# XiSHEN0220/RANSAC-Flow

Hardware: NVIDIA H100
Metric: image-pairs/sec at 480x640, nbIter=1k RANSAC (higher is better)
Workload: dtype f32-grade: fp16 hi/lo split operands and activations (22 significand bits), 3 wgmma MMAs per MAC, fp32 accumulate; fp16-split correlation; fp32/fp64 RANSAC

## Files before the change

include/ransacflow_b200.h:

```cpp
#ifndef RANSACFLOW_B200_H
#define RANSACFLOW_B200_H

#include <stddef.h>
#include <stdint.h>

#ifdef __cplusplus
extern "C" {
#endif

#define RF_MAX_IMGS 16

#define RF_RANSAC_OK 0
#define RF_RANSAC_NONE 1
#define RF_RANSAC_NO_MODEL 2
#define RF_RANSAC_TOO_FEW 3

int rf_version(void);
const char* rf_source_digest(void);
const char* rf_last_error_string(void);
uint64_t rf_launch_count(void);

size_t rf_corr_mutual_nn_workspace(int NA, int NB, int C, int precision);
int rf_corr_mutual_nn_launches(int precision);
int rf_corr_mutual_nn(const float* featA, int NA, const float* featB, int NB, int C,
                      int64_t* idx1_out, int64_t* idx2_out, int* count_out,
                      void* ws, size_t ws_bytes, int precision, void* stream);

size_t rf_corr_mutual_nn_presplit_workspace(int NA, int NB);
int rf_corr_mutual_nn_presplit(const void* A_hi, const void* A_lo, int NA, const void* B_hi, const void* B_lo, int NB, int C,
                               int64_t* idx1_out, int64_t* idx2_out, int* count_out, void* ws, size_t ws_bytes, void* stream);

#define RF_SAMPLES_INDEX 0
#define RF_SAMPLES_MOD 1
#define RF_SAMPLES_PHILOX64 2
size_t rf_ransac_workspace(int nbIter);
int rf_ransac_homography(const float* match1, const float* match2, int M, const int* M_dev,
                         const int64_t* samples, int sample_mode, int nbIter, float tolerance, int chunk,
                         float* H_out, int64_t* nbInlier_out, uint8_t* mask_out, int* status_out,
                         void* ws, size_t ws_bytes, void* stream);
int rf_homography_dlt(const float* X, const float* Y, int N, float* H_out, void* stream);
int rf_prediction(const float* match1, const float* match2, int M, const float* H, int N, float* err_out, void* stream);
int rf_build_matches(const int64_t* idx1, const int64_t* idx2, const int* count_in,
                     const float* W1, const float* H1, const float* W2, const float* H2,
                     const uint8_t* valid16, float* match1_out, float* match2_out,
                     int64_t* idx2_kept_out, int* count_out, int capacity, void* stream);

#define RF_ENGINE_FP32 0
#define RF_ENGINE_TF32 1
#define RF_ENGINE_F16 2
#define RF_ENGINE_F16_OUT32 3
#define RF_ENGINE_SPLIT 4
#define RF_ENGINE_SPLIT_OUT32 5
int rf_conv2d_nhwc(const float* x, int nimg, const int* hw_host, int Cin,
                   const float* w, const float* w_tc, const float* bias, const float* residual,
                   int Cout, int R, int S, int stride, int pad, int relu, int engine,
                   float* y, void* stream);
int rf_conv1x1_dual_split(const void* x1, const void* x2, int nimg, const int* hw1_host, const int* hw2_host, int Cin1, int Cin2,
                          int stride2, const void* w_split, const float* bias, int Cout, int relu, void* y, void* stream);
#define RF_OP_CONV 0
#define RF_OP_MAXPOOL 1
#define RF_OP_BLUR 2
#define RF_OP_IM2COL 3
#define RF_OP_POOLBLUR 4
#define RF_OP_STEM7 5
#define RF_OP_CONV_DUAL 6
#define RF_MAX_SLOTS 32
typedef struct rf_layer {
    int op;
    int src, dst, res;
    int Cin, Cout, k, stride, pad, relu;
    const float* w;
    const float* w_tc;
    const float* bias;
    const void* w_f16;
    int flags;
    int src2, Cin2, stride2;
} rf_layer_t;
#define RF_LAYER_OUT_F32 1
#define RF_LAYER_TF32 2
int rf_run_layers(const rf_layer_t* layers_host, int n, void* const* slots_host, int nimg, const int* hw_host,
                  int engine, void* stream);
int rf_maxpool2d_nhwc(const float* x, int nimg, const int* hw_host, int C, int k, int stride, int pad,
                      float* y, void* stream);
int rf_blur_downsample_nhwc(const float* x, int nimg, const int* hw_host, int C, int stride, float* y, void* stream);
int rf_l2norm_nhwc(const float* x, long long P, int C, const uint8_t* mask, float* y, void* stream);
int rf_l2norm_split_nhwc(const void* x_split, long long P, int C, const uint8_t* mask, float* y, void* y_hi, void* y_lo, void* stream);
int rf_l2norm_f16_nhwc(const void* x_f16, long long P, int C, const uint8_t* mask, float* y, void* stream);
int rf_corr_neigh_nhwc(const float* x, const float* y, int N, int h, int w, int C, int k, int ldo, int round_tf32_out,
                       float* out, void* stream);
int rf_corr_neigh_pair_nhwc(const float* x, const float* y, int N, int h, int w, int C, int k, int ldo, int round_tf32_out,
                            float* out_xy, float* out_yx, void* stream);
int rf_corr_neigh_pair_split(const float* x, const float* y, int N, int h, int w, int C, int k, int ldo, void* out12_split, void* both_split,
                             void* stream);
int rf_softmax_flow(const float* logits, int N, int h, int w, int k, float* flow_nchw, void* stream);
int rf_sigmoid(const float* x, long long n, float* y, void* stream);
int rf_preproc_u8(const uint8_t* img, long long npix, int normalize, float* out_nhwc, void* stream);
int rf_resample_u8(const uint8_t* in, int in_h, int in_w, int channels, int horizontal,
                   const int* bounds, const int* kk, int ksize, int out_size, uint8_t* out, void* stream);
int rf_lanczos_coeffs_host(int in_size, int out_size, int* bounds_host, int* kk_host, int kk_capacity, int* ksize_out);

int rf_warp_grid(const float* H, int N, int h, int w, float* grid_out, void* stream);
int rf_grid_sample(const float* in, int N, int C, int Hin, int Win, const long long* in_s_host,
                   const float* grid, int Hout, int Wout, int align_corners,
                   float* out, const long long* out_s_host, void* stream);
int rf_upsample_bilinear(const float* in, int NC, int h, int w, int H, int W, float* out, void* stream);
int rf_compose_fine(const float* flowDown8, const float* match12, const float* match21, int h8, int w8,
                    const float* coarse, int H, int W, int clamp, int align_corners,
                    float* flow12_out, float* match_out, float* flowUp_out, void* stream);
int rf_compose_fine_ex(const float* flowDown8, const float* match12, const float* match21, int h8, int w8,
                       const float* coarse, int Hc, int Wc, int H, int W, int clamp, int align_corners,
                       float* flow12_out, float* match_out, float* flowUp_out, void* stream);
size_t rf_remove_small_cc_workspace(int H, int W);
int rf_remove_small_cc(float* match, int N, int H, int W, float match_th, double cc_th, void* ws, size_t ws_bytes, void* stream);

size_t rf_fill_nearest_matched_workspace(int H, int W);
int rf_fill_nearest_matched(const float* flow, const uint8_t* matched, int H, int W, float* flow_out, int* index_out,
                            void* ws, size_t ws_bytes, void* stream);

#ifdef __cplusplus
}
#endif
#endif
```

ransac-flow_b200/csrc/common.cuh:

```cuda
#pragma once
#include <cuda_runtime.h>
#include <stdint.h>
#include <stdio.h>
#include <atomic>

#include "../../include/ransacflow_b200.h"

namespace rf {

extern thread_local char g_err[512];
extern std::atomic<uint64_t> g_launches;

inline int fail(const char* what, cudaError_t e, const char* file, int line) {
    snprintf(g_err, sizeof(g_err), "%s: %s (%s:%d)", what, cudaGetErrorString(e), file, line);
    return 1;
}
inline int fail_msg(const char* msg) {
    snprintf(g_err, sizeof(g_err), "%s", msg);
    return 2;
}

#define RF_CUDA(expr)                                                   \
    do {                                                                \
        cudaError_t _e = (expr);                                        \
        if (_e != cudaSuccess) return rf::fail(#expr, _e, __FILE__, __LINE__); \
    } while (0)

#define RF_LAUNCHED()                                                   \
    do {                                                                \
        rf::g_launches.fetch_add(1, std::memory_order_relaxed);         \
        cudaError_t _e = cudaGetLastError();                            \
        if (_e != cudaSuccess) return rf::fail("kernel launch", _e, __FILE__, __LINE__); \
    } while (0)

#define RF_REQUIRE(cond, msg)                                           \
    do {                                                                \
        if (!(cond)) return rf::fail_msg(msg " [" #cond "]");           \
    } while (0)

inline cudaStream_t as_stream(void* s) { return reinterpret_cast<cudaStream_t>(s); }

inline int current_device() {
    int dev = 0;
    cudaGetDevice(&dev);
    return (dev >= 0 && dev < 64) ? dev : 0;
}

inline int num_sms() {
    static int n[64] = {0};
    const int dev = current_device();
    if (n[dev] == 0) {
        cudaDeviceGetAttribute(&n[dev], cudaDevAttrMultiProcessorCount, dev);
        if (n[dev] <= 0) n[dev] = 132;
    }
    return n[dev];
}

struct ImgSet {
    int n;
    int H[RF_MAX_IMGS], W[RF_MAX_IMGS];
    int Ho[RF_MAX_IMGS], Wo[RF_MAX_IMGS];
    long long in_pix[RF_MAX_IMGS + 1];
    long long out_pix[RF_MAX_IMGS + 1];
};

inline int make_imgset(ImgSet& s, int nimg, const int* hw, int k, int stride, int pad) {
    if (nimg < 1 || nimg > RF_MAX_IMGS) return 1;
    s.n = nimg;
    s.in_pix[0] = 0;
    s.out_pix[0] = 0;
    for (int i = 0; i < nimg; ++i) {
        s.H[i] = hw[2 * i];
        s.W[i] = hw[2 * i + 1];
        s.Ho[i] = (s.H[i] + 2 * pad - k) / stride + 1;
        s.Wo[i] = (s.W[i] + 2 * pad - k) / stride + 1;
        if (s.Ho[i] < 1 || s.Wo[i] < 1) return 1;
        s.in_pix[i + 1] = s.in_pix[i] + (long long)s.H[i] * s.W[i];
        s.out_pix[i + 1] = s.out_pix[i] + (long long)s.Ho[i] * s.Wo[i];
    }
    for (int i = nimg; i < RF_MAX_IMGS; ++i) {
        s.H[i] = s.W[i] = s.Ho[i] = s.Wo[i] = 0;
        s.in_pix[i + 1] = s.in_pix[nimg];
        s.out_pix[i + 1] = s.out_pix[nimg];
    }
    return 0;
}

struct ConvParams {
    const float* x;
    const float* w;
    const float* bias;
    const float* residual;
    float* y;
    int Cin, Cout, R, S, stride, pad, relu;
    int round_out;
    long long Mtot;
    int K;
};

__device__ __forceinline__ int find_img(const ImgSet& s, long long p) {
    int i = 0;
#pragma unroll
    for (int j = 1; j < RF_MAX_IMGS; ++j) i += (j < s.n && p >= s.out_pix[j]) ? 1 : 0;
    return i;
}

__device__ __forceinline__ uint32_t f2ord(float f) {
    uint32_t u = __float_as_uint(f);
    return (u & 0x80000000u) ? ~u : (u | 0x80000000u);
}
__device__ __forceinline__ float round_tf32(float x) {
    uint32_t u;
    asm("cvt.rna.tf32.f32 %0, %1;" : "=r"(u) : "f"(x));
    return __uint_as_float(u);
}
__device__ __forceinline__ float ord2f(uint32_t u) {
    return __uint_as_float((u & 0x80000000u) ? (u & 0x7fffffffu) : ~u);
}
__device__ __forceinline__ unsigned long long pack_key(float v, uint32_t idx) {
    return ((unsigned long long)f2ord(v) << 32) | (unsigned long long)(0xFFFFFFFFu - idx);
}
__device__ __forceinline__ uint32_t key_index(unsigned long long k) { return 0xFFFFFFFFu - (uint32_t)(k & 0xFFFFFFFFull); }
__device__ __forceinline__ float key_value(unsigned long long k) { return ord2f((uint32_t)(k >> 32)); }

}
```

ransac-flow_b200/csrc/elementwise.cu:

```cuda
#include <cuda_fp16.h>

#include <type_traits>

#include "common.cuh"

namespace rf {

__global__ void maxpool_kernel(const __grid_constant__ ImgSet set, const float* __restrict__ x, float* __restrict__ y,
                               int C, int k, int stride, int pad) {
    const int c4n = C >> 2;
    long long t = (long long)blockIdx.x * blockDim.x + threadIdx.x;
    long long total = set.out_pix[set.n] * c4n;
    if (t >= total) return;
    long long pm = t / c4n;
    int c4 = (int)(t - pm * c4n);
    int im = find_img(set, pm);
    int local = (int)(pm - set.out_pix[im]);
    int oy = local / set.Wo[im], ox = local - oy * set.Wo[im];
    const int H = set.H[im], W = set.W[im];
    float4 m = make_float4(-INFINITY, -INFINITY, -INFINITY, -INFINITY);
    for (int r = 0; r < k; ++r) {
        int iy = oy * stride - pad + r;
        if (iy < 0 || iy >= H) continue;
        for (int s = 0; s < k; ++s) {
            int ix = ox * stride - pad + s;
            if (ix < 0 || ix >= W) continue;
            float4 v = __ldg(reinterpret_cast<const float4*>(x + (set.in_pix[im] + (long long)iy * W + ix) * C) + c4);
            m.x = fmaxf(m.x, v.x); m.y = fmaxf(m.y, v.y); m.z = fmaxf(m.z, v.z); m.w = fmaxf(m.w, v.w);
        }
    }
    reinterpret_cast<float4*>(y + pm * C)[c4] = m;
}

__global__ void maxpool_f16_kernel(const __grid_constant__ ImgSet set, const __half* __restrict__ x, __half* __restrict__ y,
                                   int C, int k, int stride, int pad) {
    const int c8n = C >> 3;
    long long t = (long long)blockIdx.x * blockDim.x + threadIdx.x;
    long long total = set.out_pix[set.n] * c8n;
    if (t >= total) return;
    long long pm = t / c8n;
    int c8 = (int)(t - pm * c8n);
    int im = find_img(set, pm);
    int local = (int)(pm - set.out_pix[im]);
    int oy = local / set.Wo[im], ox = local - oy * set.Wo[im];
    const int H = set.H[im], W = set.W[im];
    const __half2 ninf = __float2half2_rn(-INFINITY);
    __half2 m[4] = {ninf, ninf, ninf, ninf};
    for (int r = 0; r < k; ++r) {
        int iy = oy * stride - pad + r;
        if (iy < 0 || iy >= H) continue;
        for (int s = 0; s < k; ++s) {
            int ix = ox * stride - pad + s;
            if (ix < 0 || ix >= W) continue;
            const uint4 v = __ldg(reinterpret_cast<const uint4*>(x + (set.in_pix[im] + (long long)iy * W + ix) * C) + c8);
            const __half2* h = reinterpret_cast<const __half2*>(&v);
#pragma unroll
            for (int e = 0; e < 4; ++e) m[e] = __hmax2(m[e], h[e]);
        }
    }
    uint4 o;
    __half2* ho = reinterpret_cast<__half2*>(&o);
#pragma unroll
    for (int e = 0; e < 4; ++e) ho[e] = m[e];
    reinterpret_cast<uint4*>(y + pm * C)[c8] = o;
}

template <int KC, int CC, int KPADC>
__global__ void im2col_kernel(const __grid_constant__ ImgSet set, const float* __restrict__ x, float* __restrict__ y,
                              int C_, int k_, int stride, int pad, int Kpad_, int round_out) {
    const int C = CC ? CC : C_, k = KC ? KC : k_, Kpad = KPADC ? KPADC : Kpad_;
    const int im = blockIdx.y;
    const int q4 = Kpad >> 2;
    const int Wo = set.Wo[im], H = set.H[im], W = set.W[im];
    const unsigned idx = blockIdx.x * blockDim.x + threadIdx.x;
    const unsigned total = (unsigned)(set.Ho[im] * Wo) * (unsigned)q4;
    if (idx >= total) return;
    const unsigned local = idx / (unsigned)q4;
    const int e0 = (int)(idx - local * (unsigned)q4) * 4;
    const int oy = (int)(local / (unsigned)Wo), ox = (int)(local - (unsigned)oy * (unsigned)Wo);
    const int kkc = k * k * C, kc = k * C;
    const float* src = x + set.in_pix[im] * C;
    float v[4];
#pragma unroll
    for (int j = 0; j < 4; ++j) {
        const int e = e0 + j;
        float t = 0.f;
        if (e < kkc) {
            const int r = e / kc, rem = e - r * kc;
            const int iy = oy * stride - pad + r;
            const int ixc = (ox * stride - pad) * C + rem;
            if (iy >= 0 && iy < H && ixc >= 0 && ixc < W * C) t = __ldg(src + (long long)iy * W * C + ixc);
            if (round_out) t = round_tf32(t);
        }
        v[j] = t;
    }
    reinterpret_cast<float4*>(y + (set.out_pix[im] + local) * Kpad)[e0 >> 2] = make_float4(v[0], v[1], v[2], v[3]);
}

__device__ __forceinline__ int reflect1(int i, int n) { return i < 0 ? -i : (i >= n ? 2 * n - 2 - i : i); }

template <typename T> struct Vec16;
template <> struct Vec16<float> {
    typedef float elem;
    static constexpr int N = 4;
    static __device__ __forceinline__ void load(const float* p, long long, float (&v)[4]) {
        const float4 t = __ldg(reinterpret_cast<const float4*>(p));
        v[0] = t.x; v[1] = t.y; v[2] = t.z; v[3] = t.w;
    }
    static __device__ __forceinline__ void store(float* p, long long, const float (&v)[4], int round_out) {
        float4 t = make_float4(v[0], v[1], v[2], v[3]);
        if (round_out) { t.x = round_tf32(t.x); t.y = round_tf32(t.y); t.z = round_tf32(t.z); t.w = round_tf32(t.w); }
        *reinterpret_cast<float4*>(p) = t;
    }
};
template <> struct Vec16<__half> {
    typedef __half elem;
    static constexpr int N = 8;
    static __device__ __forceinline__ void load(const __half* p, long long, float (&v)[8]) {
        const uint4 t = __ldg(reinterpret_cast<const uint4*>(p));
        const __half2* h = reinterpret_cast<const __half2*>(&t);
#pragma unroll
        for (int e = 0; e < 4; ++e) { const float2 f = __half22float2(h[e]); v[2 * e] = f.x; v[2 * e + 1] = f.y; }
    }
    static __device__ __forceinline__ void store(__half* p, long long, const float (&v)[8], int) {
        uint4 t;
        __half2* h = reinterpret_cast<__half2*>(&t);
#pragma unroll
        for (int e = 0; e < 4; ++e) h[e] = __floats2half2_rn(v[2 * e], v[2 * e + 1]);
        *reinterpret_cast<uint4*>(p) = t;
    }
};
struct SplitH {};
__device__ __forceinline__ void split_store8(__half* p, long long plane, const float (&v)[8]) {
    uint4 th, tl;
    __half2* h = reinterpret_cast<__half2*>(&th);
    __half2* l = reinterpret_cast<__half2*>(&tl);
#pragma unroll
    for (int e = 0; e < 4; ++e) {
        const float a = fminf(fmaxf(v[2 * e], -65504.f), 65504.f), b = fminf(fmaxf(v[2 * e + 1], -65504.f), 65504.f);
        h[e] = __floats2half2_rn(a, b);
        const float2 f = __half22float2(h[e]);
        l[e] = __floats2half2_rn((a - f.x) * 2048.f, (b - f.y) * 2048.f);
    }
    *reinterpret_cast<uint4*>(p) = th;
    *reinterpret_cast<uint4*>(p + plane) = tl;
}
__device__ __forceinline__ void split_load8(const __half* p, long long plane, float (&v)[8]) {
    const uint4 th = __ldg(reinterpret_cast<const uint4*>(p)), tl = __ldg(reinterpret_cast<const uint4*>(p + plane));
    const __half2* h = reinterpret_cast<const __half2*>(&th);
    const __half2* l = reinterpret_cast<const __half2*>(&tl);
#pragma unroll
    for (int e = 0; e < 4; ++e) {
        const float2 fh = __half22float2(h[e]), fl = __half22float2(l[e]);
        v[2 * e] = fmaf(fl.x, 0.00048828125f, fh.x);
        v[2 * e + 1] = fmaf(fl.y, 0.00048828125f, fh.y);
    }
}
template <> struct Vec16<SplitH> {
    typedef __half elem;
    static constexpr int N = 8;
    static __device__ __forceinline__ void load(const __half* p, long long plane, float (&v)[8]) { split_load8(p, plane, v); }
    static __device__ __forceinline__ void store(__half* p, long long plane, const float (&v)[8], int) { split_store8(p, plane, v); }
};

template <typename T>
__global__ void blur_kernel(const __grid_constant__ ImgSet set, const typename Vec16<T>::elem* __restrict__ x, typename Vec16<T>::elem* __restrict__ y,
                            int C, int stride, int round_out, long long pin = 0, long long pout = 0) {
    constexpr int VN = Vec16<T>::N;
    const int cvn = C / VN;
    long long t = (long long)blockIdx.x * blockDim.x + threadIdx.x;
    long long total = set.out_pix[set.n] * cvn;
    if (t >= total) return;
    long long pm = t / cvn;
    int cv = (int)(t - pm * cvn);
    int im = find_img(set, pm);
    int local = (int)(pm - set.out_pix[im]);
    int oy = local / set.Wo[im], ox = local - oy * set.Wo[im];
    const int H = set.H[im], W = set.W[im];
    float acc[VN];
#pragma unroll
    for (int e = 0; e < VN; ++e) acc[e] = 0.f;
#pragma unroll
    for (int r = 0; r < 3; ++r) {
        int iy = reflect1(oy * stride - 1 + r, H);
#pragma unroll
        for (int s = 0; s < 3; ++s) {
            int ix = reflect1(ox * stride - 1 + s, W);
            float wgt = ((r == 1) ? 2.f : 1.f) * ((s == 1) ? 2.f : 1.f) * 0.0625f;
            float v[VN];
            Vec16<T>::load(x + (set.in_pix[im] + (long long)iy * W + ix) * C + cv * VN, pin, v);
#pragma unroll
            for (int e = 0; e < VN; ++e) acc[e] = fmaf(wgt, v[e], acc[e]);
        }
    }
    Vec16<T>::store(y + pm * C + cv * VN, pout, acc, round_out);
}

template <typename T>
__global__ void poolblur_kernel(const __grid_constant__ ImgSet set, const typename Vec16<T>::elem* __restrict__ x, typename Vec16<T>::elem* __restrict__ y,
                                int C, int round_out, long long pin = 0, long long pout = 0) {
    constexpr int VN = Vec16<T>::N;
    const int cvn = C / VN;
    long long t = (long long)blockIdx.x * blockDim.x + threadIdx.x;
    long long total = set.out_pix[set.n] * cvn;
    if (t >= total) return;
    long long pm = t / cvn;
    int cv = (int)(t - pm * cvn);
    int im = find_img(set, pm);
    int local = (int)(pm - set.out_pix[im]);
    int oy = local / set.Wo[im], ox = local - oy * set.Wo[im];
    const int H = set.H[im], W = set.W[im];
    const int Hp = H - 1, Wp = W - 1;
    const typename Vec16<T>::elem* base = x + set.in_pix[im] * C + cv * VN;
    float acc[VN];
#pragma unroll
    for (int e = 0; e < VN; ++e) acc[e] = 0.f;
#pragma unroll
    for (int r = 0; r < 3; ++r) {
        const int py = reflect1(oy * 2 - 1 + r, Hp);
#pragma unroll
        for (int s = 0; s < 3; ++s) {
            const int px = reflect1(ox * 2 - 1 + s, Wp);
            const float wgt = ((r == 1) ? 2.f : 1.f) * ((s == 1) ? 2.f : 1.f) * 0.0625f;
            float a[VN], b[VN], c[VN], d[VN];
            Vec16<T>::load(base + ((long long)py * W + px) * C, pin, a);
            Vec16<T>::load(base + ((long long)py * W + px + 1) * C, pin, b);
            Vec16<T>::load(base + ((long long)(py + 1) * W + px) * C, pin, c);
            Vec16<T>::load(base + ((long long)(py + 1) * W + px + 1) * C, pin, d);
#pragma unroll
            for (int e = 0; e < VN; ++e) acc[e] = fmaf(wgt, fmaxf(fmaxf(a[e], b[e]), fmaxf(c[e], d[e])), acc[e]);
        }
    }
    Vec16<T>::store(y + pm * C + cv * VN, pout, acc, round_out);
}

__global__ void maxpool_split_kernel(const __grid_constant__ ImgSet set, const __half* __restrict__ x, __half* __restrict__ y,
                                     int C, int k, int stride, int pad, long long pin, long long pout) {
    const int c8n = C >> 3;
    long long t = (long long)blockIdx.x * blockDim.x + threadIdx.x;
    long long total = set.out_pix[set.n] * c8n;
    if (t >= total) return;
    long long pm = t / c8n;
    int c8 = (int)(t - pm * c8n);
    int im = find_img(set, pm);
    int local = (int)(pm - set.out_pix[im]);
    int oy = local / set.Wo[im], ox = local - oy * set.Wo[im];
    const int H = set.H[im], W = set.W[im];
    float m[8];
#pragma unroll
    for (int e = 0; e < 8; ++e) m[e] = -INFINITY;
    for (int r = 0; r < k; ++r) {
        int iy = oy * stride - pad + r;
        if (iy < 0 || iy >= H) continue;
        for (int s = 0; s < k; ++s) {
            int ix = ox * stride - pad + s;
            if (ix < 0 || ix >= W) continue;
            float v[8];
            split_load8(x + (set.in_pix[im] + (long long)iy * W + ix) * C + c8 * 8, pin, v);
#pragma unroll
            for (int e = 0; e < 8; ++e) m[e] = fmaxf(m[e], v[e]);
        }
    }
    split_store8(y + pm * C + c8 * 8, pout, m);
}

__global__ void l2norm_kernel(const float* __restrict__ x, long long P, int C, const unsigned char* __restrict__ mask, float* __restrict__ y) {
    long long pix = ((long long)blockIdx.x * blockDim.x + threadIdx.x) >> 5;
    int lane = threadIdx.x & 31;
    if (pix >= P) return;
    const float4* src = reinterpret_cast<const float4*>(x + pix * C);
    float4* dst = reinterpret_cast<float4*>(y + pix * C);
    const int c4n = C >> 2;
    if (mask != nullptr && mask[pix] == 0) {
        for (int c = lane; c < c4n; c += 32) dst[c] = make_float4(0, 0, 0, 0);
        return;
    }
    float ss = 0.f;
    for (int c = lane; c < c4n; c += 32) {
        float4 v = __ldg(src + c);
        ss = fmaf(v.x, v.x, ss); ss = fmaf(v.y, v.y, ss); ss = fmaf(v.z, v.z, ss); ss = fmaf(v.w, v.w, ss);
    }
#pragma unroll
    for (int d = 16; d >= 1; d >>= 1) ss += __shfl_xor_sync(0xffffffffu, ss, d);
    float denom = fmaxf(sqrtf(ss), 1e-12f);
    for (int c = lane; c < c4n; c += 32) {
        float4 v = __ldg(src + c);
        dst[c] = make_float4(__fdiv_rn(v.x, denom), __fdiv_rn(v.y, denom), __fdiv_rn(v.z, denom), __fdiv_rn(v.w, denom));
    }
}

__global__ void l2norm_f16_kernel(const __half* __restrict__ x, long long P, int C, const unsigned char* __restrict__ mask, float* __restrict__ y) {
    long long pix = ((long long)blockIdx.x * blockDim.x + threadIdx.x) >> 5;
    int lane = threadIdx.x & 31;
    if (pix >= P) return;
    const uint4* src = reinterpret_cast<const uint4*>(x + pix * C);
    float4* dst = reinterpret_cast<float4*>(y + pix * C);
    const int c8n = C >> 3;
    if (mask != nullptr && mask[pix] == 0) {
        for (int c = lane; c < 2 * c8n; c += 32) dst[c] = make_float4(0, 0, 0, 0);
        return;
    }
    float ss = 0.f;
    for (int c = lane; c < c8n; c += 32) {
        const uint4 v = __ldg(src + c);
        const __half2* h = reinterpret_cast<const __half2*>(&v);
#pragma unroll
        for (int e = 0; e < 4; ++e) { const float2 f = __half22float2(h[e]); ss = fmaf(f.x, f.x, ss); ss = fmaf(f.y, f.y, ss); }
    }
#pragma unroll
    for (int d = 16; d >= 1; d >>= 1) ss += __shfl_xor_sync(0xffffffffu, ss, d);
    float denom = fmaxf(sqrtf(ss), 1e-12f);
    for (int c = lane; c < c8n; c += 32) {
        const uint4 v = __ldg(src + c);
        const __half2* h = reinterpret_cast<const __half2*>(&v);
        const float2 f0 = __half22float2(h[0]), f1 = __half22float2(h[1]), f2 = __half22float2(h[2]), f3 = __half22float2(h[3]);
        dst[2 * c] = make_float4(__fdiv_rn(f0.x, denom), __fdiv_rn(f0.y, denom), __fdiv_rn(f1.x, denom), __fdiv_rn(f1.y, denom));
        dst[2 * c + 1] = make_float4(__fdiv_rn(f2.x, denom), __fdiv_rn(f2.y, denom), __fdiv_rn(f3.x, denom), __fdiv_rn(f3.y, denom));
    }
}

__global__ void l2norm_split_kernel(const __half* __restrict__ x, long long plane, long long P, int C, const unsigned char* __restrict__ mask,
                                    float* __restrict__ y, __half* __restrict__ yhi, __half* __restrict__ ylo) {
    long long pix = ((long long)blockIdx.x * blockDim.x + threadIdx.x) >> 5;
    int lane = threadIdx.x & 31;
    if (pix >= P) return;
    const __half* src = x + pix * C;
    float4* dst = reinterpret_cast<float4*>(y + pix * C);
    const int c8n = C >> 3;
    if (mask != nullptr && mask[pix] == 0) {
        if (y != nullptr)
            for (int c = lane; c < 2 * c8n; c += 32) dst[c] = make_float4(0, 0, 0, 0);
        if (yhi != nullptr)
            for (int c = lane; c < c8n; c += 32) {
                reinterpret_cast<uint4*>(yhi + pix * C)[c] = make_uint4(0, 0, 0, 0);
                reinterpret_cast<uint4*>(ylo + pix * C)[c] = make_uint4(0, 0, 0, 0);
            }
        return;
    }
    float ss = 0.f;
    for (int c = lane; c < c8n; c += 32) {
        float v[8];
        split_load8(src + c * 8, plane, v);
#pragma unroll
        for (int e = 0; e < 8; ++e) ss = fmaf(v[e], v[e], ss);
    }
#pragma unroll
    for (int d = 16; d >= 1; d >>= 1) ss += __shfl_xor_sync(0xffffffffu, ss, d);
    float denom = fmaxf(sqrtf(ss), 1e-12f);
    for (int c = lane; c < c8n; c += 32) {
        float v[8];
        split_load8(src + c * 8, plane, v);
#pragma unroll
        for (int e = 0; e < 8; ++e) v[e] = __fdiv_rn(v[e], denom);
        if (y != nullptr) {
            dst[2 * c] = make_float4(v[0], v[1], v[2], v[3]);
            dst[2 * c + 1] = make_float4(v[4], v[5], v[6], v[7]);
        }
        if (yhi != nullptr) split_store8(yhi + pix * C + c * 8, (ylo - yhi), v);
    }
}

__device__ __forceinline__ void corr_store(float* out, long long idx, float v, int round_out, long long plane) {
    if (round_out == 3) {
        const float a = fminf(fmaxf(v, -65504.f), 65504.f);
        const __half h = __float2half_rn(a);
        reinterpret_cast<__half*>(out)[idx] = h;
        reinterpret_cast<__half*>(out)[idx + plane] = __float2half_rn((a - __half2float(h)) * 2048.f);
    } else if (round_out == 2) {
        reinterpret_cast<__half*>(out)[idx] = __float2half_rn(v);
    } else {
        out[idx] = round_out ? round_tf32(v) : v;
    }
}

__global__ void corr_neigh_kernel(const float* __restrict__ x, const float* __restrict__ y, int N, int h, int w, int C, int k, int ldo, int round_out,
                                  float* __restrict__ out, float* __restrict__ out2) {
    long long pix = ((long long)blockIdx.x * blockDim.x + threadIdx.x) >> 5;
    int lane = threadIdx.x & 31;
    long long P = (long long)N * h * w;
    if (pix >= P) return;
    int n = (int)(pix / ((long long)h * w));
    int rem = (int)(pix - (long long)n * h * w);
    int r = rem / w, c = rem - r * w;
    const int pad = k / 2, c4n = C >> 2;
    const bool split = round_out == 3;
    const long long plane1 = P * ldo, plane2 = 2 * P * ldo;
    const float4* xs = reinterpret_cast<const float4*>(x + pix * C);
    float4 xv[8];
#pragma unroll
    for (int q = 0; q < 8; ++q) xv[q] = (lane + 32 * q < c4n) ? __ldg(xs + lane + 32 * q) : make_float4(0, 0, 0, 0);
    for (int i = 0; i < k; ++i) {
        int yr = r + i - pad;
        for (int j = 0; j < k; ++j) {
            int yc = c + j - pad;
            float acc = 0.f;
            if (yr >= 0 && yr < h && yc >= 0 && yc < w) {
                const float4* ys = reinterpret_cast<const float4*>(y + (((long long)n * h + yr) * w + yc) * C);
#pragma unroll
                for (int q = 0; q < 8; ++q)
                    if (lane + 32 * q < c4n) {
                        float4 v = __ldg(ys + lane + 32 * q);
                        acc = fmaf(xv[q].x, v.x, acc); acc = fmaf(xv[q].y, v.y, acc);
                        acc = fmaf(xv[q].z, v.z, acc); acc = fmaf(xv[q].w, v.w, acc);
                    }
            }
#pragma unroll
            for (int d = 16; d >= 1; d >>= 1) acc += __shfl_xor_sync(0xffffffffu, acc, d);
            if (lane == 0) {
                corr_store(out, pix * ldo + i * k + j, acc, round_out, plane1);
                if (out2 != nullptr) {
                    if (split) corr_store(out2, pix * ldo + i * k + j, acc, 3, plane2);
                    const bool inside = yr >= 0 && yr < h && yc >= 0 && yc < w;
                    const long long q = inside ? (((long long)n * h + yr) * w + yc) : pix;
                    const int e = inside ? (k - 1 - i) * k + (k - 1 - j) : i * k + j;
                    if (split) corr_store(out2, (P + q) * ldo + e, acc, 3, plane2);
                    else corr_store(out2, q * ldo + e, acc, round_out, 0);
                }
            }
        }
    }
    for (int cz = k * k + lane; cz < ldo; cz += 32) {
        corr_store(out, pix * ldo + cz, 0.f, round_out, plane1);
        if (out2 != nullptr) {
            if (split) { corr_store(out2, pix * ldo + cz, 0.f, 3, plane2); corr_store(out2, (P + pix) * ldo + cz, 0.f, 3, plane2); }
            else corr_store(out2, pix * ldo + cz, 0.f, round_out, 0);
        }
    }
}

__global__ void __launch_bounds__(256)
corr_neigh7_kernel(const float* __restrict__ x, const float* __restrict__ y, int N, int h, int w, int C, int ldo, int round_out,
                   float* __restrict__ out, float* __restrict__ out2) {
    constexpr int K = 7, KK = 49, PAD = 3;
    const long long pix = ((long long)blockIdx.x * blockDim.x + threadIdx.x) >> 5;
    const int lane = threadIdx.x & 31;
    const long long P = (long long)N * h * w;
    if (pix >= P) return;
    const int n = (int)(pix / ((long long)h * w));
    const int rem = (int)(pix - (long long)n * h * w);
    const int r = rem / w, c = rem - r * w;
    const int c4n = C >> 2;
    const bool split = round_out == 3;
    const long long plane1 = P * ldo, plane2 = 2 * P * ldo;
    const float4* xs = reinterpret_cast<const float4*>(x + pix * C);
    float4 xv[8];
#pragma unroll
    for (int q = 0; q < 8; ++q) xv[q] = (lane + 32 * q < c4n) ? __ldg(xs + lane + 32 * q) : make_float4(0, 0, 0, 0);
    float a[64];
#pragma unroll
    for (int t = 0; t < 64; ++t) a[t] = 0.f;
#pragma unroll
    for (int i = 0; i < K; ++i) {
        const int yr = r + i - PAD;
#pragma unroll
        for (int j = 0; j < K; ++j) {
            const int yc = c + j - PAD;
            if (yr >= 0 && yr < h && yc >= 0 && yc < w) {
                const float4* ys = reinterpret_cast<const float4*>(y + (((long long)n * h + yr) * w + yc) * C);
                float acc = 0.f;
#pragma unroll
                for (int q = 0; q < 8; ++q)
                    if (lane + 32 * q < c4n) {
                        const float4 v = __ldg(ys + lane + 32 * q);
                        acc = fmaf(xv[q].x, v.x, acc); acc = fmaf(xv[q].y, v.y, acc);
                        acc = fmaf(xv[q].z, v.z, acc); acc = fmaf(xv[q].w, v.w, acc);
                    }
                a[i * K + j] = acc;
            }
        }
    }
#pragma unroll
    for (int s = 16, nv = 32; s >= 1; s >>= 1, nv >>= 1) {
        const bool up = (lane & s) != 0;
#pragma unroll
        for (int v = 0; v < nv; ++v) {
            const float send = up ? a[v] : a[v + nv];
            const float keep = up ? a[v + nv] : a[v];
            a[v] = keep + __shfl_xor_sync(0xffffffffu, send, s);
        }
    }
#pragma unroll
    for (int u = 0; u < 2; ++u) {
        const int t = 2 * lane + u;
        if (t >= ldo) continue;
        const float v = a[u];
        corr_store(out, pix * ldo + t, v, round_out, plane1);
        if (out2 != nullptr) {
            if (split) corr_store(out2, pix * ldo + t, v, 3, plane2);
            if (t < KK) {
                const int i = t / K, j = t - i * K;
                const int yr = r + i - PAD, yc = c + j - PAD;
                const bool inside = yr >= 0 && yr < h && yc >= 0 && yc < w;
                const long long q = inside ? (((long long)n * h + yr) * w + yc) : pix;
                const int e = inside ? (KK - 1 - t) : t;
                if (split) corr_store(out2, (P + q) * ldo + e, v, 3, plane2);
                else corr_store(out2, q * ldo + e, v, round_out, 0);
            } else {
                if (split) corr_store(out2, (P + pix) * ldo + t, 0.f, 3, plane2);
                else corr_store(out2, pix * ldo + t, 0.f, round_out, 0);
            }
        }
    }
    for (int t = 64 + lane; t < ldo; t += 32) {
        corr_store(out, pix * ldo + t, 0.f, round_out, plane1);
        if (out2 != nullptr) {
            if (split) { corr_store(out2, pix * ldo + t, 0.f, 3, plane2); corr_store(out2, (P + pix) * ldo + t, 0.f, 3, plane2); }
            else corr_store(out2, pix * ldo + t, 0.f, round_out, 0);
        }
    }
}

__global__ void softmax_flow_kernel(const float* __restrict__ logits, int N, int h, int w, int k, float* __restrict__ flow) {
    long long pix = (long long)blockIdx.x * blockDim.x + threadIdx.x;
    long long hw = (long long)h * w;
    if (pix >= N * hw) return;
    const int kk = k * k, pad = k / 2;
    const float* l = logits + pix * kk;
    float m = -INFINITY;
    for (int q = 0; q < kk; ++q) m = fmaxf(m, __ldg(l + q));
    float sum = 0.f, sx = 0.f, sy = 0.f;
    for (int q = 0; q < kk; ++q) {
        float e = expf(__ldg(l + q) - m);
        sum += e;
        sx = fmaf(e, (float)(q % k - pad), sx);
        sy = fmaf(e, (float)(q / k - pad), sy);
    }
    int n = (int)(pix / hw);
    long long rem = pix - n * hw;
    flow[(n * 2 + 0) * hw + rem] = (sx / sum) / (float)w * 2.f;
    flow[(n * 2 + 1) * hw + rem] = (sy / sum) / (float)h * 2.f;
}

__global__ void sigmoid_kernel(const float* __restrict__ x, long long n, float* __restrict__ y) {
    long long i = (long long)blockIdx.x * blockDim.x + threadIdx.x;
    if (i < n) y[i] = 1.f / (1.f + expf(-x[i]));
}

__global__ void preproc_kernel(const unsigned char* __restrict__ img, long long n, int normalize, float* __restrict__ out) {
    long long i = (long long)blockIdx.x * blockDim.x + threadIdx.x;
    if (i >= n) return;
    int c = (int)(i % 3);
    float v = __fdiv_rn((float)img[i], 255.f);
    if (normalize) {
        const float mean = (c == 0) ? 0.485f : (c == 1 ? 0.456f : 0.406f);
        const float sd = (c == 0) ? 0.229f : (c == 1 ? 0.224f : 0.225f);
        v = __fdiv_rn(__fsub_rn(v, mean), sd);
    }
    out[i] = v;
}

__device__ __forceinline__ float preproc_one(unsigned int byte, int c, int normalize) {
    float v = __fdiv_rn((float)byte, 255.f);
    if (normalize) {
        const float mean = (c == 0) ? 0.485f : (c == 1 ? 0.456f : 0.406f);
        const float sd = (c == 0) ? 0.229f : (c == 1 ? 0.224f : 0.225f);
        v = __fdiv_rn(__fsub_rn(v, mean), sd);
    }
    return v;
}
__global__ void preproc_vec_kernel(const unsigned int* __restrict__ img, long long ngroups, int normalize, float4* __restrict__ out) {
    long long g = (long long)blockIdx.x * blockDim.x + threadIdx.x;
    if (g >= ngroups) return;
    const unsigned int w0 = __ldg(img + 3 * g), w1 = __ldg(img + 3 * g + 1), w2 = __ldg(img + 3 * g + 2);
    out[3 * g] = make_float4(preproc_one(w0 & 255u, 0, normalize), preproc_one((w0 >> 8) & 255u, 1, normalize),
                             preproc_one((w0 >> 16) & 255u, 2, normalize), preproc_one(w0 >> 24, 0, normalize));
    out[3 * g + 1] = make_float4(preproc_one(w1 & 255u, 1, normalize), preproc_one((w1 >> 8) & 255u, 2, normalize),
                                 preproc_one((w1 >> 16) & 255u, 0, normalize), preproc_one(w1 >> 24, 1, normalize));
    out[3 * g + 2] = make_float4(preproc_one(w2 & 255u, 2, normalize), preproc_one((w2 >> 8) & 255u, 0, normalize),
                                 preproc_one((w2 >> 16) & 255u, 1, normalize), preproc_one(w2 >> 24, 2, normalize));
}

#define RF_PRECISION_BITS 22
__device__ __forceinline__ unsigned char clip8(int ss) {
    int v = ss >> RF_PRECISION_BITS;
    return (unsigned char)(v < 0 ? 0 : (v > 255 ? 255 : v));
}
__global__ void resample_h_kernel(const unsigned char* __restrict__ in, int in_h, int in_w, int ch, const int* __restrict__ bounds,
                                  const int* __restrict__ kk, int ksize, int out_w, unsigned char* __restrict__ out) {
    long long t = (long long)blockIdx.x * blockDim.x + threadIdx.x;
    if (t >= (long long)in_h * out_w) return;
    const int ox = (int)(t % out_w), oy = (int)(t / out_w);
    const int lo = bounds[2 * ox], cnt = bounds[2 * ox + 1];
    const int* k = kk + (long long)ox * ksize;
    const unsigned char* row = in + ((long long)oy * in_w + lo) * ch;
    if (ch == 3) {
        int s0 = 1 << (RF_PRECISION_BITS - 1), s1 = s0, s2 = s0;
        for (int x = 0; x < cnt; ++x) {
            const int kx = __ldg(k + x);
            s0 += (int)row[3 * x] * kx; s1 += (int)row[3 * x + 1] * kx; s2 += (int)row[3 * x + 2] * kx;
        }
        unsigned char* o = out + t * 3;
        o[0] = clip8(s0); o[1] = clip8(s1); o[2] = clip8(s2);
    } else {
        for (int c = 0; c < ch; ++c) {
            int ss = 1 << (RF_PRECISION_BITS - 1);
            for (int x = 0; x < cnt; ++x) ss += (int)row[(long long)x * ch + c] * __ldg(k + x);
            out[t * ch + c] = clip8(ss);
        }
    }
}
__global__ void resample_v_kernel(const unsigned char* __restrict__ in, int in_h, int row_bytes, const int* __restrict__ bounds,
                                  const int* __restrict__ kk, int ksize, int out_h, unsigned char* __restrict__ out) {
    const int q = row_bytes >> 2;
    long long t = (long long)blockIdx.x * blockDim.x + threadIdx.x;
    if (t >= (long long)out_h * q) return;
    const int xq = (int)(t % q), oy = (int)(t / q);
    const int lo = bounds[2 * oy], cnt = bounds[2 * oy + 1];
    const int* k = kk + (long long)oy * ksize;
    const unsigned int* col = reinterpret_cast<const unsigned int*>(in + (long long)lo * row_bytes) + xq;
    int s0 = 1 << (RF_PRECISION_BITS - 1), s1 = s0, s2 = s0, s3 = s0;
    for (int y = 0; y < cnt; ++y) {
        const unsigned int v = __ldg(col + (long long)y * q);
        const int ky = __ldg(k + y);
        s0 += (int)(v & 0xFF) * ky; s1 += (int)((v >> 8) & 0xFF) * ky; s2 += (int)((v >> 16) & 0xFF) * ky; s3 += (int)(v >> 24) * ky;
    }
    reinterpret_cast<unsigned int*>(out)[t] = (unsigned)clip8(s0) | ((unsigned)clip8(s1) << 8) | ((unsigned)clip8(s2) << 16) | ((unsigned)clip8(s3) << 24);
}
__global__ void resample_u8_kernel(const unsigned char* __restrict__ in, int in_h, int in_w, int ch, int horizontal,
                                   const int* __restrict__ bounds, const int* __restrict__ kk, int ksize, int out_size,
                                   unsigned char* __restrict__ out) {
    const int out_h = horizontal ? in_h : out_size, out_w = horizontal ? out_size : in_w;
    long long t = (long long)blockIdx.x * blockDim.x + threadIdx.x;
    long long total = (long long)out_h * out_w * ch;
    if (t >= total) return;
    int c = (int)(t % ch);
    long long pq = t / ch;
    int ox = (int)(pq % out_w), oy = (int)(pq / out_w);
    int o = horizontal ? ox : oy;
    int lo = bounds[2 * o], cnt = bounds[2 * o + 1];
    const int* k = kk + (long long)o * ksize;
    int ss = 1 << (RF_PRECISION_BITS - 1);
    if (horizontal) {
        const unsigned char* row = in + ((long long)oy * in_w) * ch + c;
        for (int x = 0; x < cnt; ++x) ss += (int)row[(long long)(x + lo) * ch] * k[x];
    } else {
        const unsigned char* col = in + (long long)ox * ch + c;
        for (int y = 0; y < cnt; ++y) ss += (int)col[(long long)(y + lo) * in_w * ch] * k[y];
    }
    out[t] = clip8(ss);
}

__device__ __forceinline__ float lin11(int i, int n) {
    if (n == 1) return -1.f;
    float step = 2.f / (float)(n - 1);
    return (i < n / 2) ? (-1.f + step * (float)i) : (1.f - step * (float)(n - 1 - i));
}

__global__ void warp_grid_kernel(const float* __restrict__ Hm, int N, int h, int w, float* __restrict__ grid) {
    long long t = (long long)blockIdx.x * blockDim.x + threadIdx.x;
    long long hw = (long long)h * w;
    if (t >= N * hw) return;
    int n = (int)(t / hw);
    int rem = (int)(t - n * hw);
    int r = rem / w, c = rem - r * w;
    const float* H = Hm + n * 9;
    float x = lin11(c, w), y = lin11(r, h);
    float px = __fadd_rn(__fadd_rn(__fmul_rn(H[0], x), __fmul_rn(H[1], y)), H[2]);
    float py = __fadd_rn(__fadd_rn(__fmul_rn(H[3], x), __fmul_rn(H[4], y)), H[5]);
    float pz = __fadd_rn(__fadd_rn(__fmul_rn(H[6], x), __fmul_rn(H[7], y)), H[8]);
    reinterpret_cast<float2*>(grid)[t] = make_float2(__fdiv_rn(px, pz), __fdiv_rn(py, pz));
}

__device__ __forceinline__ float unnormalize(float coord, int size, int align_corners) {
    return align_corners ? ((coord + 1.f) / 2.f) * (float)(size - 1) : ((coord + 1.f) * (float)size - 1.f) / 2.f;
}

__device__ __forceinline__ float in_int_range(float c) {
    return fabsf(c) < 2147483648.f ? c : -100.f;
}

struct Strides4 { long long n, c, h, w; };

__global__ void grid_sample_kernel(const float* __restrict__ in, int N, int C, int Hin, int Win, Strides4 is,
                                   const float* __restrict__ grid, int Hout, int Wout, int align_corners,
                                   float* __restrict__ out, Strides4 os) {
    long long t = (long long)blockIdx.x * blockDim.x + threadIdx.x;
    long long hw = (long long)Hout * Wout;
    if (t >= N * hw) return;
    int n = (int)(t / hw);
    int rem = (int)(t - n * hw);
    int r = rem / Wout, c = rem - r * Wout;
    float2 g = __ldg(reinterpret_cast<const float2*>(grid) + t);
    float ix = in_int_range(unnormalize(g.x, Win, align_corners)), iy = in_int_range(unnormalize(g.y, Hin, align_corners));
    float fx = floorf(ix), fy = floorf(iy);
    int x0 = (int)fx, y0 = (int)fy, x1 = x0 + 1, y1 = y0 + 1;
    float nw = (fx + 1.f - ix) * (fy + 1.f - iy), ne = (ix - fx) * (fy + 1.f - iy);
    float sw = (fx + 1.f - ix) * (iy - fy), se = (ix - fx) * (iy - fy);
    bool vx0 = x0 >= 0 && x0 < Win, vx1 = x1 >= 0 && x1 < Win, vy0 = y0 >= 0 && y0 < Hin, vy1 = y1 >= 0 && y1 < Hin;
    const float* base = in + n * is.n;
    float* ob = out + n * os.n + r * os.h + c * os.w;
    for (int ch = 0; ch < C; ++ch) {
        const float* p = base + ch * is.c;
        float acc = 0.f;
        if (vy0 && vx0) acc += __ldg(p + y0 * is.h + x0 * is.w) * nw;
        if (vy0 && vx1) acc += __ldg(p + y0 * is.h + x1 * is.w) * ne;
        if (vy1 && vx0) acc += __ldg(p + y1 * is.h + x0 * is.w) * sw;
        if (vy1 && vx1) acc += __ldg(p + y1 * is.h + x1 * is.w) * se;
        ob[ch * os.c] = acc;
    }
}

__device__ __forceinline__ void up_coord(int dst, int in_size, int out_size, int& i0, int& i1, float& l0, float& l1) {
    float scale = (float)in_size / (float)out_size;
    float src = scale * ((float)dst + 0.5f) - 0.5f;
    if (src < 0.f) src = 0.f;
    i0 = (int)src;
    i1 = i0 + ((i0 < in_size - 1) ? 1 : 0);
    l1 = src - (float)i0;
    l0 = 1.f - l1;
}
__device__ __forceinline__ float up_sample(const float* __restrict__ p, int h, int w, int H, int W, int Y, int X) {
    int y0, y1, x0, x1;
    float ly0, ly1, lx0, lx1;
    up_coord(Y, h, H, y0, y1, ly0, ly1);
    up_coord(X, w, W, x0, x1, lx0, lx1);
    return ly0 * (lx0 * __ldg(p + y0 * w + x0) + lx1 * __ldg(p + y0 * w + x1)) +
           ly1 * (lx0 * __ldg(p + y1 * w + x0) + lx1 * __ldg(p + y1 * w + x1));
}

__global__ void upsample_kernel(const float* __restrict__ in, int NC, int h, int w, int H, int W, float* __restrict__ out) {
    long long t = (long long)blockIdx.x * blockDim.x + threadIdx.x;
    long long HW = (long long)H * W;
    if (t >= NC * HW) return;
    int nc = (int)(t / HW);
    int rem = (int)(t - nc * HW);
    int Y = rem / W, X = rem - Y * W;
    out[t] = up_sample(in + (long long)nc * h * w, h, w, H, W, Y, X);
}

__global__ void compose_fine_kernel(const float* __restrict__ flow8, const float* __restrict__ m12, const float* __restrict__ m21,
                                    int h8, int w8, const float* __restrict__ coarse, int Hc, int Wc, int H, int W, int clamp, int align_corners,
                                    float* __restrict__ flow12, float* __restrict__ match, float* __restrict__ flowUp_out) {
    long long t = (long long)blockIdx.x * blockDim.x + threadIdx.x;
    if (t >= (long long)H * W) return;
    int Y = (int)(t / W), X = (int)(t - (long long)Y * W);
    float fx = up_sample(flow8, h8, w8, H, W, Y, X) + lin11(X, W);
    float fy = up_sample(flow8 + h8 * w8, h8, w8, H, W, Y, X) + lin11(Y, H);
    if (clamp) {
        fx = fminf(fmaxf(fx, -1.f), 1.f);
        fy = fminf(fmaxf(fy, -1.f), 1.f);
    }
    if (flowUp_out) reinterpret_cast<float2*>(flowUp_out)[t] = make_float2(fx, fy);
    const float2* cg = reinterpret_cast<const float2*>(coarse);
    float ox = 0.f, oy = 0.f, mm = 0.f;
    {
        float ix = unnormalize(fx, Wc, align_corners), iy = unnormalize(fy, Hc, align_corners);
        float flx = floorf(ix), fly = floorf(iy);
        int x0 = (int)flx, y0 = (int)fly, x1 = x0 + 1, y1 = y0 + 1;
        float nw = (flx + 1.f - ix) * (fly + 1.f - iy), ne = (ix - flx) * (fly + 1.f - iy);
        float sw = (flx + 1.f - ix) * (iy - fly), se = (ix - flx) * (iy - fly);
        bool vx0 = x0 >= 0 && x0 < Wc, vx1 = x1 >= 0 && x1 < Wc, vy0 = y0 >= 0 && y0 < Hc, vy1 = y1 >= 0 && y1 < Hc;
        if (vy0 && vx0) { float2 v = __ldg(cg + (long long)y0 * Wc + x0); ox += v.x * nw; oy += v.y * nw; }
        if (vy0 && vx1) { float2 v = __ldg(cg + (long long)y0 * Wc + x1); ox += v.x * ne; oy += v.y * ne; }
        if (vy1 && vx0) { float2 v = __ldg(cg + (long long)y1 * Wc + x0); ox += v.x * sw; oy += v.y * sw; }
        if (vy1 && vx1) { float2 v = __ldg(cg + (long long)y1 * Wc + x1); ox += v.x * se; oy += v.y * se; }
    }
    if (m21) {
        float ix = unnormalize(fx, W, align_corners), iy = unnormalize(fy, H, align_corners);
        float flx = floorf(ix), fly = floorf(iy);
        int x0 = (int)flx, y0 = (int)fly, x1 = x0 + 1, y1 = y0 + 1;
        float nw = (flx + 1.f - ix) * (fly + 1.f - iy), ne = (ix - flx) * (fly + 1.f - iy);
        float sw = (flx + 1.f - ix) * (iy - fly), se = (ix - flx) * (iy - fly);
        bool vx0 = x0 >= 0 && x0 < W, vx1 = x1 >= 0 && x1 < W, vy0 = y0 >= 0 && y0 < H, vy1 = y1 >= 0 && y1 < H;
        if (vy0 && vx0) mm += up_sample(m21, h8, w8, H, W, y0, x0) * nw;
        if (vy0 && vx1) mm += up_sample(m21, h8, w8, H, W, y0, x1) * ne;
        if (vy1 && vx0) mm += up_sample(m21, h8, w8, H, W, y1, x0) * sw;
        if (vy1 && vx1) mm += up_sample(m21, h8, w8, H, W, y1, x1) * se;
    }
    reinterpret_cast<float2*>(flow12)[t] = make_float2(ox, oy);
    if (match) {
        float m = up_sample(m12, h8, w8, H, W, Y, X);
        if (m21) m *= mm;
        float inside = ((ox >= -1.f && ox <= 1.f) ? 1.f : 0.f) * ((oy >= -1.f && oy <= 1.f) ? 1.f : 0.f);
        match[t] = m * inside;
    }
}

__device__ __forceinline__ int cc_find(const int* L, int i) {
    int p = L[i];
    while (p != i) { i = p; p = L[i]; }
    return i;
}
__device__ __forceinline__ void cc_union(int* L, int a, int b) {
    bool done = false;
    while (!done) {
        a = cc_find(L, a);
        b = cc_find(L, b);
        if (a < b) { int old = atomicMin(&L[b], a); done = (old == b); b = old; }
        else if (b < a) { int old = atomicMin(&L[a], b); done = (old == a); a = old; }
        else done = true;
    }
}
__global__ void cc_init_kernel(const float* __restrict__ match, float th, int n, int* __restrict__ L, int* __restrict__ cnt) {
    int i = blockIdx.x * blockDim.x + threadIdx.x;
    if (i >= n) return;
    L[i] = (match[i] > th) ? i : -1;
    cnt[i] = 0;
}
__global__ void cc_merge_kernel(int* __restrict__ L, int H, int W) {
    int i = blockIdx.x * blockDim.x + threadIdx.x;
    if (i >= H * W || L[i] < 0) return;
    const int y = i / W, x = i - y * W;
    if (x > 0 && L[i - 1] >= 0) cc_union(L, i, i - 1);
    if (y > 0) {
        if (L[i - W] >= 0) cc_union(L, i, i - W);
        if (x > 0 && L[i - W - 1] >= 0) cc_union(L, i, i - W - 1);
        if (x + 1 < W && L[i - W + 1] >= 0) cc_union(L, i, i - W + 1);
    }
}
__global__ void cc_flatten_count_kernel(int* __restrict__ L, int n, int* __restrict__ cnt) {
    int i = blockIdx.x * blockDim.x + threadIdx.x;
    if (i >= n || L[i] < 0) return;
    const int r = cc_find(L, i);
    atomicAdd(&cnt[r], 1);
}
__global__ void cc_filter_kernel(float* __restrict__ match, const int* __restrict__ L, const int* __restrict__ cnt, int n, double cc_th) {
    int i = blockIdx.x * blockDim.x + threadIdx.x;
    if (i >= n || L[i] < 0) return;
    const int r = cc_find(L, i);
    if ((double)cnt[r] / (double)n <= cc_th) match[i] = 0.f;
}

__global__ void edt_cols_kernel(const unsigned char* __restrict__ matched, int H, int W, int* __restrict__ gy) {
    const int x = blockIdx.x * blockDim.x + threadIdx.x;
    if (x >= W) return;
    int last = -1;
    for (int y = 0; y < H; ++y) {
        if (matched[(long long)y * W + x]) last = y;
        gy[(long long)y * W + x] = last;
    }
    last = -1;
    for (int y = H - 1; y >= 0; --y) {
        if (matched[(long long)y * W + x]) last = y;
        const int a = gy[(long long)y * W + x];
        int pick = a;
        if (a < 0) pick = last;
        else if (last >= 0 && (last - y) < (y - a)) pick = last;
        gy[(long long)y * W + x] = pick;
    }
}
__global__ void edt_rows_fill_kernel(const int* __restrict__ gy, int H, int W, int* __restrict__ v, double* __restrict__ z,
                                     const float2* __restrict__ flow, float2* __restrict__ out, int* __restrict__ idx_out) {
    const int y = blockIdx.x * blockDim.x + threadIdx.x;
    if (y >= H) return;
    const int* g = gy + (long long)y * W;
    int* vv = v + (long long)y * W;
    double* zz = z + (long long)y * (W + 1);
    int k = -1;
    for (int q = 0; q < W; ++q) {
        if (g[q] < 0) continue;
        const long long dq = (long long)(y - g[q]) * (y - g[q]);
        double sx = -1e300;
        while (k >= 0) {
            const int p = vv[k];
            const long long dp = (long long)(y - g[p]) * (y - g[p]);
            sx = (double)((dq + (long long)q * q) - (dp + (long long)p * p)) / (double)(2 * (q - p));
            if (sx <= zz[k]) --k; else break;
        }
        if (k < 0) sx = -1e300;
        ++k;
        vv[k] = q;
        zz[k] = sx;
    }
    if (k < 0) {
        for (int x = 0; x < W; ++x) { out[(long long)y * W + x] = flow[(long long)y * W + x]; if (idx_out) { idx_out[2 * ((long long)y * W + x)] = y; idx_out[2 * ((long long)y * W + x) + 1] = x; } }
        return;
    }
    const int kmax = k;
    k = 0;
    for (int x = 0; x < W; ++x) {
        while (k < kmax && zz[k + 1] < (double)x) ++k;
        const int xs = vv[k], ys = g[xs];
        out[(long long)y * W + x] = flow[(long long)ys * W + xs];
        if (idx_out) { idx_out[2 * ((long long)y * W + x)] = ys; idx_out[2 * ((long long)y * W + x) + 1] = xs; }
    }
}

}

using namespace rf;

static inline unsigned blocks_for(long long n, int threads) { return (unsigned)((n + threads - 1) / threads); }

static int launch_corr_neigh(const float* x, const float* y, int N, int h, int w, int C, int k, int ldo, int round_out, float* out,
                             float* out2, void* stream) {
    const long long P = (long long)N * h * w;
    if (P == 0) return 0;
    if (k == 7) corr_neigh7_kernel<<<blocks_for(P * 32, 256), 256, 0, as_stream(stream)>>>(x, y, N, h, w, C, ldo, round_out, out, out2);
    else corr_neigh_kernel<<<blocks_for(P * 32, 256), 256, 0, as_stream(stream)>>>(x, y, N, h, w, C, k, ldo, round_out, out, out2);
    RF_LAUNCHED();
    return 0;
}

extern "C" int rf_maxpool2d_nhwc(const float* x, int nimg, const int* hw_host, int C, int k, int stride, int pad, float* y, void* stream) {
    RF_REQUIRE((C % 4) == 0 && k >= 1 && stride >= 1, "rf_maxpool2d_nhwc: C must be a multiple of 4");
    ImgSet set;
    RF_REQUIRE(make_imgset(set, nimg, hw_host, k, stride, pad) == 0, "rf_maxpool2d_nhwc: bad image set");
    long long total = set.out_pix[nimg] * (C / 4);
    maxpool_kernel<<<blocks_for(total, 256), 256, 0, as_stream(stream)>>>(set, x, y, C, k, stride, pad);
    RF_LAUNCHED();
    return 0;
}

int rf_blur_downsample_impl(const float* x, int nimg, const int* hw_host, int C, int stride, int round_out, float* y, void* stream) {
    RF_REQUIRE((C % 4) == 0 && stride >= 1, "rf_blur_downsample_nhwc: C must be a multiple of 4");
    ImgSet set;
    RF_REQUIRE(make_imgset(set, nimg, hw_host, 3, stride, 1) == 0, "rf_blur_downsample_nhwc: bad image set");
    for (int i = 0; i < nimg; ++i) RF_REQUIRE(set.H[i] >= 2 && set.W[i] >= 2, "rf_blur_downsample_nhwc: reflect padding needs H, W >= 2");
    long long total = set.out_pix[nimg] * (C / 4);
    blur_kernel<float><<<blocks_for(total, 256), 256, 0, as_stream(stream)>>>(set, x, y, C, stride, round_out);
    RF_LAUNCHED();
    return 0;
}

int rf_poolblur_impl(const float* x, int nimg, const int* hw_host, int C, int round_out, float* y, void* stream) {
    RF_REQUIRE((C % 4) == 0, "rf_poolblur: C must be a multiple of 4");
    ImgSet set;
    RF_REQUIRE(make_imgset(set, nimg, hw_host, 4, 2, 1) == 0, "rf_poolblur: bad image set");
    for (int i = 0; i < nimg; ++i) RF_REQUIRE(set.H[i] >= 3 && set.W[i] >= 3, "rf_poolblur: needs H, W >= 3");
    long long total = set.out_pix[nimg] * (C / 4);
    poolblur_kernel<float><<<blocks_for(total, 256), 256, 0, as_stream(stream)>>>(set, x, y, C, round_out);
    RF_LAUNCHED();
    return 0;
}

extern "C" int rf_blur_downsample_nhwc(const float* x, int nimg, const int* hw_host, int C, int stride, float* y, void* stream) {
    return rf_blur_downsample_impl(x, nimg, hw_host, C, stride, 0, y, stream);
}

template <typename T> struct OutElem { typedef T type; };
template <> struct OutElem<SplitH> { typedef __half type; };

template <int K, int C, int KPAD, int STRIDE, int PAD, int TPX, typename OutT = float>
__global__ void __launch_bounds__(256)
im2col_smem_kernel(const __grid_constant__ ImgSet set, const float* __restrict__ x, typename OutElem<OutT>::type* __restrict__ y, int round_out,
                   long long plane = 0) {
    constexpr int INW = ((TPX - 1) * STRIDE + K) * C;
    constexpr int Q4 = KPAD / 4;
    __shared__ float sIn[K][INW + 1];
    const int im = blockIdx.z, oy = blockIdx.y, ox0 = blockIdx.x * TPX;
    const int Wo = set.Wo[im];
    if (oy >= set.Ho[im] || ox0 >= Wo) return;
    const int H = set.H[im], WC = set.W[im] * C;
    const float* src = x + set.in_pix[im] * C;
    const int col0 = (ox0 * STRIDE - PAD) * C;
    constexpr int NLD = (K * INW + 255) / 256;
    float stage[NLD];
#pragma unroll
    for (int i = 0; i < NLD; ++i) {
        const int idx = threadIdx.x + i * 256;
        const int r = idx / INW, j = idx - r * INW;
        const int iy = oy * STRIDE - PAD + r, col = col0 + j;
        stage[i] = (idx < K * INW && iy >= 0 && iy < H && col >= 0 && col < WC) ? __ldg(src + (long long)iy * WC + col) : 0.f;
    }
#pragma unroll
    for (int i = 0; i < NLD; ++i) {
        const int idx = threadIdx.x + i * 256;
        const int r = idx / INW, j = idx - r * INW;
        if (idx < K * INW) sIn[r][j] = round_out ? round_tf32(stage[i]) : stage[i];
    }
    __syncthreads();
    const int npx = min(TPX, Wo - ox0);
    if constexpr (std::is_same<OutT, SplitH>::value) {
        constexpr int Q8 = KPAD / 8;
        __half* dsts = y + (set.out_pix[im] + (long long)oy * Wo + ox0) * KPAD;
        for (int f = threadIdx.x; f < npx * Q8; f += 256) {
            const int px = f / Q8, e0 = (f - px * Q8) * 8;
            float v[8];
#pragma unroll
            for (int j = 0; j < 8; ++j) {
                const int e = e0 + j;
                v[j] = (e < K * K * C) ? sIn[e / (K * C)][px * STRIDE * C + e % (K * C)] : 0.f;
            }
            split_store8(dsts + (long long)f * 8, plane, v);
        }
        return;
    } else if constexpr (sizeof(OutT) == 2) {
        constexpr int Q8 = KPAD / 8;
        uint4* dst8 = reinterpret_cast<uint4*>(y + (set.out_pix[im] + (long long)oy * Wo + ox0) * KPAD);
        for (int f = threadIdx.x; f < npx * Q8; f += 256) {
            const int px = f / Q8, e0 = (f - px * Q8) * 8;
            float v[8];
#pragma unroll
            for (int j = 0; j < 8; ++j) {
                const int e = e0 + j;
                v[j] = (e < K * K * C) ? sIn[e / (K * C)][px * STRIDE * C + e % (K * C)] : 0.f;
            }
            uint4 o;
            __half2* ho = reinterpret_cast<__half2*>(&o);
#pragma unroll
            for (int j = 0; j < 4; ++j) ho[j] = __floats2half2_rn(v[2 * j], v[2 * j + 1]);
            dst8[f] = o;
        }
        return;
    }
    float4* dst = reinterpret_cast<float4*>(y + (set.out_pix[im] + (long long)oy * Wo + ox0) * KPAD);
    for (int f = threadIdx.x; f < npx * Q4; f += 256) {
        const int px = f / Q4, e0 = (f - px * Q4) * 4;
        float v[4];
#pragma unroll
        for (int j = 0; j < 4; ++j) {
            const int e = e0 + j;
            v[j] = (e < K * K * C) ? sIn[e / (K * C)][px * STRIDE * C + e % (K * C)] : 0.f;
        }
        dst[f] = make_float4(v[0], v[1], v[2], v[3]);
    }
}

int rf_im2col_impl(const float* x, int nimg, const int* hw_host, int C, int k, int stride, int pad, int Kpad, int round_out,
                   float* y, void* stream) {
    RF_REQUIRE(Kpad >= k * k * C && C >= 1, "rf_im2col: Kpad too small");
    ImgSet set;
    RF_REQUIRE(make_imgset(set, nimg, hw_host, k, stride, pad) == 0, "rf_im2col: bad image set");
    RF_REQUIRE((Kpad & 3) == 0, "rf_im2col: Kpad must be a multiple of 4");
    long long maxq = 0;
    for (int i = 0; i < nimg; ++i) {
        long long q = (long long)set.Ho[i] * set.Wo[i] * (Kpad / 4);
        RF_REQUIRE(q < (1ll << 31), "rf_im2col: image too large for 32-bit indexing");
        if (q > maxq) maxq = q;
    }
    int maxHo = 0, maxWo = 0;
    for (int i = 0; i < nimg; ++i) { maxHo = set.Ho[i] > maxHo ? set.Ho[i] : maxHo; maxWo = set.Wo[i] > maxWo ? set.Wo[i] : maxWo; }
    if (k == 7 && C == 3 && Kpad == 160 && stride == 2 && pad == 3) {
        im2col_smem_kernel<7, 3, 160, 2, 3, 64><<<dim3((maxWo + 63) / 64, maxHo, nimg), 256, 0, as_stream(stream)>>>(set, x, y, round_out);
        RF_LAUNCHED();
        return 0;
    }
    if (k == 3 && C == 3 && Kpad == 32 && stride == 1 && pad == 1) {
        im2col_smem_kernel<3, 3, 32, 1, 1, 128><<<dim3((maxWo + 127) / 128, maxHo, nimg), 256, 0, as_stream(stream)>>>(set, x, y, round_out);
        RF_LAUNCHED();
        return 0;
    }
    dim3 grid(blocks_for(maxq, 256), nimg);
    if (k == 7 && C == 3 && Kpad == 160) im2col_kernel<7, 3, 160><<<grid, 256, 0, as_stream(stream)>>>(set, x, y, C, k, stride, pad, Kpad, round_out);
    else if (k == 3 && C == 3 && Kpad == 32) im2col_kernel<3, 3, 32><<<grid, 256, 0, as_stream(stream)>>>(set, x, y, C, k, stride, pad, Kpad, round_out);
    else im2col_kernel<0, 0, 0><<<grid, 256, 0, as_stream(stream)>>>(set, x, y, C, k, stride, pad, Kpad, round_out);
    RF_LAUNCHED();
    return 0;
}

int rf_im2col_f16_impl(const float* x, int nimg, const int* hw_host, int C, int k, int stride, int pad, int Kpad, void* y_f16, void* stream) {
    const bool resnet = (k == 7 && C == 3 && Kpad == 192 && stride == 2 && pad == 3);
    const bool fe = (k == 3 && C == 3 && Kpad == 64 && stride == 1 && pad == 1);
    RF_REQUIRE(resnet || fe, "rf_im2col (engine 2): only the ResNet-50 stem (7x7/2, Kpad 192) and the FeatureExtractor stem (3x3/1, Kpad 64)");
    ImgSet set;
    RF_REQUIRE(make_imgset(set, nimg, hw_host, k, stride, pad) == 0, "rf_im2col: bad image set");
    int maxHo = 0, maxWo = 0;
    for (int i = 0; i < nimg; ++i) { maxHo = set.Ho[i] > maxHo ? set.Ho[i] : maxHo; maxWo = set.Wo[i] > maxWo ? set.Wo[i] : maxWo; }
    if (fe) {
        im2col_smem_kernel<3, 3, 64, 1, 1, 128, __half><<<dim3((maxWo + 127) / 128, maxHo, nimg), 256, 0, as_stream(stream)>>>(
            set, x, static_cast<__half*>(y_f16), 0);
        RF_LAUNCHED();
        return 0;
    }
    im2col_smem_kernel<7, 3, 192, 2, 3, 64, __half><<<dim3((maxWo + 63) / 64, maxHo, nimg), 256, 0, as_stream(stream)>>>(
        set, x, static_cast<__half*>(y_f16), 0);
    RF_LAUNCHED();
    return 0;
}

int rf_blur_f16_impl(const void* x_f16, int nimg, const int* hw_host, int C, int stride, void* y_f16, void* stream) {
    RF_REQUIRE((C % 8) == 0 && stride >= 1, "rf_blur (engine 2): C must be a multiple of 8");
    ImgSet set;
    RF_REQUIRE(make_imgset(set, nimg, hw_host, 3, stride, 1) == 0, "rf_blur: bad image set");
    for (int i = 0; i < nimg; ++i) RF_REQUIRE(set.H[i] >= 2 && set.W[i] >= 2, "rf_blur: reflect padding needs H, W >= 2");
    long long total = set.out_pix[nimg] * (C / 8);
    blur_kernel<__half><<<blocks_for(total, 256), 256, 0, as_stream(stream)>>>(set, static_cast<const __half*>(x_f16), static_cast<__half*>(y_f16), C, stride, 0);
    RF_LAUNCHED();
    return 0;
}

int rf_poolblur_f16_impl(const void* x_f16, int nimg, const int* hw_host, int C, void* y_f16, void* stream) {
    RF_REQUIRE((C % 8) == 0, "rf_poolblur (engine 2): C must be a multiple of 8");
    ImgSet set;
    RF_REQUIRE(make_imgset(set, nimg, hw_host, 4, 2, 1) == 0, "rf_poolblur: bad image set");
    for (int i = 0; i < nimg; ++i) RF_REQUIRE(set.H[i] >= 3 && set.W[i] >= 3, "rf_poolblur: needs H, W >= 3");
    long long total = set.out_pix[nimg] * (C / 8);
    poolblur_kernel<__half><<<blocks_for(total, 256), 256, 0, as_stream(stream)>>>(set, static_cast<const __half*>(x_f16), static_cast<__half*>(y_f16), C, 0);
    RF_LAUNCHED();
    return 0;
}

int rf_maxpool_f16_impl(const void* x_f16, int nimg, const int* hw_host, int C, int k, int stride, int pad, void* y_f16, void* stream) {
    RF_REQUIRE((C % 8) == 0 && k >= 1 && stride >= 1, "rf_maxpool (engine 2): C must be a multiple of 8");
    ImgSet set;
    RF_REQUIRE(make_imgset(set, nimg, hw_host, k, stride, pad) == 0, "rf_maxpool: bad image set");
    long long total = set.out_pix[nimg] * (C / 8);
    maxpool_f16_kernel<<<blocks_for(total, 256), 256, 0, as_stream(stream)>>>(set, static_cast<const __half*>(x_f16), static_cast<__half*>(y_f16), C, k, stride, pad);
    RF_LAUNCHED();
    return 0;
}

extern "C" int rf_l2norm_f16_nhwc(const void* x_f16, long long P, int C, const uint8_t* mask, float* y, void* stream) {
    RF_REQUIRE((C % 8) == 0 && P >= 0, "rf_l2norm_f16_nhwc: C must be a multiple of 8");
    RF_REQUIRE(((uintptr_t)x_f16 % 16) == 0 && ((uintptr_t)y % 16) == 0, "rf_l2norm_f16_nhwc: pointers must be 16-byte aligned");
    if (P == 0) return 0;
    l2norm_f16_kernel<<<blocks_for(P * 32, 256), 256, 0, as_stream(stream)>>>(static_cast<const __half*>(x_f16), P, C, mask, y);
    RF_LAUNCHED();
    return 0;
}

int rf_blur_split_impl(const void* x, int nimg, const int* hw_host, int C, int stride, void* y, void* stream) {
    RF_REQUIRE((C % 8) == 0 && stride >= 1, "rf_blur (engine 4): C must be a multiple of 8");
    ImgSet set;
    RF_REQUIRE(make_imgset(set, nimg, hw_host, 3, stride, 1) == 0, "rf_blur: bad image set");
    for (int i = 0; i < nimg; ++i) RF_REQUIRE(set.H[i] >= 2 && set.W[i] >= 2, "rf_blur: reflect padding needs H, W >= 2");
    long long total = set.out_pix[nimg] * (C / 8);
    blur_kernel<SplitH><<<blocks_for(total, 256), 256, 0, as_stream(stream)>>>(set, static_cast<const __half*>(x), static_cast<__half*>(y), C, stride, 0,
                                                                              set.in_pix[nimg] * C, set.out_pix[nimg] * C);
    RF_LAUNCHED();
    return 0;
}

int rf_poolblur_split_impl(const void* x, int nimg, const int* hw_host, int C, void* y, void* stream) {
    RF_REQUIRE((C % 8) == 0, "rf_poolblur (engine 4): C must be a multiple of 8");
    ImgSet set;
    RF_REQUIRE(make_imgset(set, nimg, hw_host, 4, 2, 1) == 0, "rf_poolblur: bad image set");
    for (int i = 0; i < nimg; ++i) RF_REQUIRE(set.H[i] >= 3 && set.W[i] >= 3, "rf_poolblur: needs H, W >= 3");
    long long total = set.out_pix[nimg] * (C / 8);
    poolblur_kernel<SplitH><<<blocks_for(total, 256), 256, 0, as_stream(stream)>>>(set, static_cast<const __half*>(x), static_cast<__half*>(y), C, 0,
                                                                                  set.in_pix[nimg] * C, set.out_pix[nimg] * C);
    RF_LAUNCHED();
    return 0;
}

int rf_maxpool_split_impl(const void* x, int nimg, const int* hw_host, int C, int k, int stride, int pad, void* y, void* stream) {
    RF_REQUIRE((C % 8) == 0 && k >= 1 && stride >= 1, "rf_maxpool (engine 4): C must be a multiple of 8");
    ImgSet set;
    RF_REQUIRE(make_imgset(set, nimg, hw_host, k, stride, pad) == 0, "rf_maxpool: bad image set");
    long long total = set.out_pix[nimg] * (C / 8);
    maxpool_split_kernel<<<blocks_for(total, 256), 256, 0, as_stream(stream)>>>(set, static_cast<const __half*>(x), static_cast<__half*>(y), C, k, stride, pad,
                                                                               set.in_pix[nimg] * C, set.out_pix[nimg] * C);
    RF_LAUNCHED();
    return 0;
}

int rf_im2col_split_impl(const float* x, int nimg, const int* hw_host, int C, int k, int stride, int pad, int Kpad, void* y, void* stream) {
    RF_REQUIRE(k == 3 && C == 3 && Kpad == 64 && stride == 1 && pad == 1, "rf_im2col (engine 4): only the FeatureExtractor stem (3x3/1, Kpad 64)");
    ImgSet set;
    RF_REQUIRE(make_imgset(set, nimg, hw_host, k, stride, pad) == 0, "rf_im2col: bad image set");
    int maxHo = 0, maxWo = 0;
    for (int i = 0; i < nimg; ++i) { maxHo = set.Ho[i] > maxHo ? set.Ho[i] : maxHo; maxWo = set.Wo[i] > maxWo ? set.Wo[i] : maxWo; }
    im2col_smem_kernel<3, 3, 64, 1, 1, 128, SplitH><<<dim3((maxWo + 127) / 128, maxHo, nimg), 256, 0, as_stream(stream)>>>(
        set, x, static_cast<__half*>(y), 0, set.out_pix[nimg] * 64);
    RF_LAUNCHED();
    return 0;
}

extern "C" int rf_l2norm_split_nhwc(const void* x_split, long long P, int C, const uint8_t* mask, float* y, void* y_hi, void* y_lo, void* stream) {
    RF_REQUIRE((C % 8) == 0 && P >= 0, "rf_l2norm_split_nhwc: C must be a multiple of 8");
    RF_REQUIRE(((uintptr_t)x_split % 16) == 0 && ((uintptr_t)y % 16) == 0 && ((uintptr_t)y_hi % 16) == 0 && ((uintptr_t)y_lo % 16) == 0,
               "rf_l2norm_split_nhwc: pointers must be 16-byte aligned");
    RF_REQUIRE((y_hi == nullptr) == (y_lo == nullptr), "rf_l2norm_split_nhwc: y_hi and y_lo go together");
    RF_REQUIRE(y != nullptr || y_hi != nullptr, "rf_l2norm_split_nhwc: no output");
    if (P == 0) return 0;
    l2norm_split_kernel<<<blocks_for(P * 32, 256), 256, 0, as_stream(stream)>>>(static_cast<const __half*>(x_split), P * C, P, C, mask, y,
                                                                               static_cast<__half*>(y_hi), static_cast<__half*>(y_lo));
    RF_LAUNCHED();
    return 0;
}

extern "C" int rf_corr_neigh_pair_split(const float* x, const float* y, int N, int h, int w, int C, int k, int ldo, void* out12_split, void* both_split,
                                        void* stream) {
    RF_REQUIRE((C % 4) == 0 && C <= 1024 && (k % 2) == 1 && ldo >= k * k, "rf_corr_neigh_pair_split: need C % 4 == 0, C <= 1024, odd k, ldo >= k*k");
    RF_REQUIRE(out12_split != nullptr && out12_split != both_split, "rf_corr_neigh_pair_split: outputs");
    return launch_corr_neigh(x, y, N, h, w, C, k, ldo, 3, static_cast<float*>(out12_split), static_cast<float*>(both_split), stream);
}

extern "C" int rf_l2norm_nhwc(const float* x, long long P, int C, const uint8_t* mask, float* y, void* stream) {
    RF_REQUIRE((C % 4) == 0 && P >= 0, "rf_l2norm_nhwc: C must be a multiple of 4");
    if (P == 0) return 0;
    l2norm_kernel<<<blocks_for(P * 32, 256), 256, 0, as_stream(stream)>>>(x, P, C, mask, y);
    RF_LAUNCHED();
    return 0;
}

extern "C" int rf_corr_neigh_nhwc(const float* x, const float* y, int N, int h, int w, int C, int k, int ldo, int round_tf32_out, float* out, void* stream) {
    RF_REQUIRE((C % 4) == 0 && C <= 1024 && (k % 2) == 1 && ldo >= k * k, "rf_corr_neigh_nhwc: need C % 4 == 0, C <= 1024, odd k, ldo >= k*k");
    return launch_corr_neigh(x, y, N, h, w, C, k, ldo, round_tf32_out, out, nullptr, stream);
}

extern "C" int rf_corr_neigh_pair_nhwc(const float* x, const float* y, int N, int h, int w, int C, int k, int ldo, int round_tf32_out,
                                       float* out_xy, float* out_yx, void* stream) {
    RF_REQUIRE((C % 4) == 0 && C <= 1024 && (k % 2) == 1 && ldo >= k * k, "rf_corr_neigh_pair_nhwc: need C % 4 == 0, C <= 1024, odd k, ldo >= k*k");
    RF_REQUIRE(out_xy != nullptr && out_yx != nullptr && out_xy != out_yx, "rf_corr_neigh_pair_nhwc: two distinct outputs");
    return launch_corr_neigh(x, y, N, h, w, C, k, ldo, round_tf32_out, out_xy, out_yx, stream);
}

extern "C" int rf_softmax_flow(const float* logits, int N, int h, int w, int k, float* flow_nchw, void* stream) {
    long long P = (long long)N * h * w;
    if (P == 0) return 0;
    softmax_flow_kernel<<<blocks_for(P, 128), 128, 0, as_stream(stream)>>>(logits, N, h, w, k, flow_nchw);
    RF_LAUNCHED();
    return 0;
}

extern "C" int rf_sigmoid(const float* x, long long n, float* y, void* stream) {
    if (n <= 0) return 0;
    sigmoid_kernel<<<blocks_for(n, 256), 256, 0, as_stream(stream)>>>(x, n, y);
    RF_LAUNCHED();
    return 0;
}

extern "C" int rf_preproc_u8(const uint8_t* img, long long npix, int normalize, float* out_nhwc, void* stream) {
    if (npix <= 0) return 0;
    const long long n = npix * 3;
    if (((uintptr_t)img & 3) == 0 && ((uintptr_t)out_nhwc & 15) == 0 && n >= 12) {
        const long long groups = n / 12, tail = n - groups * 12;
        preproc_vec_kernel<<<blocks_for(groups, 256), 256, 0, as_stream(stream)>>>(reinterpret_cast<const unsigned int*>(img), groups, normalize,
                                                                                   reinterpret_cast<float4*>(out_nhwc));
        RF_LAUNCHED();
        if (tail > 0) {
            preproc_kernel<<<1, 32, 0, as_stream(stream)>>>(img + groups * 12, tail, normalize, out_nhwc + groups * 12);
            RF_LAUNCHED();
        }
        return 0;
    }
    preproc_kernel<<<blocks_for(n, 256), 256, 0, as_stream(stream)>>>(img, n, normalize, out_nhwc);
    RF_LAUNCHED();
    return 0;
}

extern "C" int rf_resample_u8(const uint8_t* in, int in_h, int in_w, int channels, int horizontal,
                              const int* bounds, const int* kk, int ksize, int out_size, uint8_t* out, void* stream) {
    long long total = (long long)(horizontal ? in_h : out_size) * (horizontal ? out_size : in_w) * channels;
    if (total <= 0) return 0;
    if (horizontal) {
        resample_h_kernel<<<blocks_for((long long)in_h * out_size, 256), 256, 0, as_stream(stream)>>>(in, in_h, in_w, channels, bounds, kk, ksize, out_size, out);
        RF_LAUNCHED();
        return 0;
    }
    const long long row_bytes = (long long)in_w * channels;
    if ((row_bytes & 3) == 0 && ((uintptr_t)in & 3) == 0 && ((uintptr_t)out & 3) == 0) {
        resample_v_kernel<<<blocks_for((long long)out_size * (row_bytes >> 2), 256), 256, 0, as_stream(stream)>>>(in, in_h, (int)row_bytes, bounds, kk, ksize, out_size, out);
        RF_LAUNCHED();
        return 0;
    }
    resample_u8_kernel<<<blocks_for(total, 256), 256, 0, as_stream(stream)>>>(in, in_h, in_w, channels, horizontal, bounds, kk, ksize, out_size, out);
    RF_LAUNCHED();
    return 0;
}

static double rf_sinc(double x) {
    if (x == 0.0) return 1.0;
    x = x * 3.14159265358979323846;
    return sin(x) / x;
}
static double rf_lanczos(double x) {
    if (-3.0 <= x && x < 3.0) return rf_sinc(x) * rf_sinc(x / 3);
    return 0.0;
}
extern "C" int rf_lanczos_coeffs_host(int in_size, int out_size, int* bounds_host, int* kk_host, int kk_capacity, int* ksize_out) {
    RF_REQUIRE(in_size > 0 && out_size > 0, "rf_lanczos_coeffs_host: bad sizes");
    double scale, filterscale;
    filterscale = scale = (double)in_size / out_size;
    if (filterscale < 1.0) filterscale = 1.0;
    double support = 3.0 * filterscale;
    int ksize = (int)ceil(support) * 2 + 1;
    *ksize_out = ksize;
    if (kk_host == nullptr) return 0;
    RF_REQUIRE((long long)ksize * out_size <= kk_capacity, "rf_lanczos_coeffs_host: kk buffer too small");
    double* k = new double[ksize];
    for (int xx = 0; xx < out_size; xx++) {
        double center = 0 + (xx + 0.5) * scale;
        double ww = 0.0;
        double ss = 1.0 / filterscale;
        int xmin = (int)(center - support + 0.5);
        if (xmin < 0) xmin = 0;
        int xmax = (int)(center + support + 0.5);
        if (xmax > in_size) xmax = in_size;
        xmax -= xmin;
        int x;
        for (x = 0; x < xmax; x++) {
            double w = rf_lanczos((x + xmin - center + 0.5) * ss);
            k[x] = w;
            ww += w;
        }
        for (x = 0; x < xmax; x++)
            if (ww != 0.0) k[x] /= ww;
        for (; x < ksize; x++) k[x] = 0;
        bounds_host[xx * 2 + 0] = xmin;
        bounds_host[xx * 2 + 1] = xmax;
        for (x = 0; x < ksize; x++) {
            if (k[x] < 0) kk_host[xx * ksize + x] = (int)(-0.5 + k[x] * (1 << RF_PRECISION_BITS));
            else kk_host[xx * ksize + x] = (int)(0.5 + k[x] * (1 << RF_PRECISION_BITS));
        }
    }
    delete[] k;
    return 0;
}

extern "C" int rf_warp_grid(const float* H, int N, int h, int w, float* grid_out, void* stream) {
    long long total = (long long)N * h * w;
    if (total <= 0) return 0;
    warp_grid_kernel<<<blocks_for(total, 256), 256, 0, as_stream(stream)>>>(H, N, h, w, grid_out);
    RF_LAUNCHED();
    return 0;
}

extern "C" int rf_grid_sample(const float* in, int N, int C, int Hin, int Win, const long long* in_s_host,
                              const float* grid, int Hout, int Wout, int align_corners,
                              float* out, const long long* out_s_host, void* stream) {
    long long total = (long long)N * Hout * Wout;
    if (total <= 0) return 0;
    Strides4 is{in_s_host[0], in_s_host[1], in_s_host[2], in_s_host[3]};
    Strides4 os{out_s_host[0], out_s_host[1], out_s_host[2], out_s_host[3]};
    grid_sample_kernel<<<blocks_for(total, 256), 256, 0, as_stream(stream)>>>(in, N, C, Hin, Win, is, grid, Hout, Wout, align_corners, out, os);
    RF_LAUNCHED();
    return 0;
}

extern "C" int rf_upsample_bilinear(const float* in, int NC, int h, int w, int H, int W, float* out, void* stream) {
    long long total = (long long)NC * H * W;
    if (total <= 0) return 0;
    upsample_kernel<<<blocks_for(total, 256), 256, 0, as_stream(stream)>>>(in, NC, h, w, H, W, out);
    RF_LAUNCHED();
    return 0;
}

extern "C" int rf_compose_fine(const float* flowDown8, const float* match12, const float* match21, int h8, int w8,
                               const float* coarse, int H, int W, int clamp, int align_corners,
                               float* flow12_out, float* match_out, float* flowUp_out, void* stream) {
    long long total = (long long)H * W;
    if (total <= 0) return 0;
    RF_REQUIRE(match_out == nullptr || match12 != nullptr, "rf_compose_fine: match_out needs match12");
    compose_fine_kernel<<<blocks_for(total, 256), 256, 0, as_stream(stream)>>>(flowDown8, match12, match21, h8, w8, coarse, H, W, H, W, clamp,
                                                                              align_corners, flow12_out, match_out, flowUp_out);
    RF_LAUNCHED();
    return 0;
}

extern "C" int rf_compose_fine_ex(const float* flowDown8, const float* match12, const float* match21, int h8, int w8,
                                  const float* coarse, int Hc, int Wc, int H, int W, int clamp, int align_corners,
                                  float* flow12_out, float* match_out, float* flowUp_out, void* stream) {
    long long total = (long long)H * W;
    if (total <= 0) return 0;
    RF_REQUIRE(Hc >= 1 && Wc >= 1, "rf_compose_fine_ex: empty coarse grid");
    RF_REQUIRE(match_out == nullptr || match12 != nullptr, "rf_compose_fine_ex: match_out needs match12");
    compose_fine_kernel<<<blocks_for(total, 256), 256, 0, as_stream(stream)>>>(flowDown8, match12, match21, h8, w8, coarse, Hc, Wc, H, W, clamp,
                                                                              align_corners, flow12_out, match_out, flowUp_out);
    RF_LAUNCHED();
    return 0;
}

extern "C" size_t rf_remove_small_cc_workspace(int H, int W) { return 2ull * (size_t)(H > 0 ? H : 0) * (size_t)(W > 0 ? W : 0) * sizeof(int) + 256; }

extern "C" int rf_remove_small_cc(float* match, int N, int H, int W, float match_th, double cc_th, void* ws, size_t ws_bytes, void* stream) {
    if (cc_th == 0.0 || N <= 0 || H <= 0 || W <= 0) return 0;
    RF_REQUIRE((long long)H * W < (1ll << 31), "rf_remove_small_cc: image too large");
    RF_REQUIRE(ws != nullptr && ws_bytes >= rf_remove_small_cc_workspace(H, W), "rf_remove_small_cc: workspace too small");
    const int n = H * W;
    int* L = reinterpret_cast<int*>((reinterpret_cast<uintptr_t>(ws) + 255) & ~(uintptr_t)255);
    int* cnt = L + n;
    cudaStream_t st = as_stream(stream);
    for (int j = 0; j < N; ++j) {
        float* m = match + (long long)j * n;
        cc_init_kernel<<<blocks_for(n, 256), 256, 0, st>>>(m, match_th, n, L, cnt);
        RF_LAUNCHED();
        cc_merge_kernel<<<blocks_for(n, 256), 256, 0, st>>>(L, H, W);
        RF_LAUNCHED();
        cc_flatten_count_kernel<<<blocks_for(n, 256), 256, 0, st>>>(L, n, cnt);
        RF_LAUNCHED();
        cc_filter_kernel<<<blocks_for(n, 256), 256, 0, st>>>(m, L, cnt, n, cc_th);
        RF_LAUNCHED();
    }
    return 0;
}

extern "C" size_t rf_fill_nearest_matched_workspace(int H, int W) {
    const size_t h = H > 0 ? H : 0, w = W > 0 ? W : 0;
    return 2 * h * w * sizeof(int) + h * (w + 1) * sizeof(double) + 512;
}

extern "C" int rf_fill_nearest_matched(const float* flow, const uint8_t* matched, int H, int W, float* flow_out, int* index_out,
                                       void* ws, size_t ws_bytes, void* stream) {
    if (H <= 0 || W <= 0) return 0;
    RF_REQUIRE(flow != flow_out, "rf_fill_nearest_matched: in-place is not supported");
    RF_REQUIRE(ws != nullptr && ws_bytes >= rf_fill_nearest_matched_workspace(H, W), "rf_fill_nearest_matched: workspace too small");
    const size_t n = (size_t)H * W;
    double* z = reinterpret_cast<double*>((reinterpret_cast<uintptr_t>(ws) + 255) & ~(uintptr_t)255);
    int* gy = reinterpret_cast<int*>(z + (size_t)H * (W + 1));
    int* v = gy + n;
    cudaStream_t st = as_stream(stream);
    edt_cols_kernel<<<blocks_for(W, 64), 64, 0, st>>>(matched, H, W, gy);
    RF_LAUNCHED();
    edt_rows_fill_kernel<<<blocks_for(H, 32), 32, 0, st>>>(gy, H, W, v, z, reinterpret_cast<const float2*>(flow),
                                                          reinterpret_cast<float2*>(flow_out), index_out);
    RF_LAUNCHED();
    return 0;
}
```

ransac-flow_b200/csrc/gemm_tc.cu:

```cuda
#include <cuda.h>
#include <cuda_fp16.h>

#include <mutex>
#include <unordered_map>

#include "common.cuh"
#include "tc_common.cuh"

namespace rf {

constexpr int K_TF32 = 0, K_F16 = 1, K_SPLIT = 2, K_TF32X3 = 3;
constexpr int MODE_CONV = 0, MODE_CORR = 1;
constexpr int O_F32 = 0, O_F16 = 1, O_SPLIT = 2;
constexpr int WG_THREADS = 288;

struct alignas(64) WgParams {
    CUtensorMap mapA[RF_MAX_IMGS];
    CUtensorMap mapA2[RF_MAX_IMGS];
    CUtensorMap mapY[RF_MAX_IMGS];
    CUtensorMap mapR[RF_MAX_IMGS];
    CUtensorMap mapB;
    CUtensorMap mapBlo;
    int nimg;
    int tiles, ntiles;
    int tile_start[RF_MAX_IMGS + 1];
    int tiles_x[RF_MAX_IMGS];
    int tw[RF_MAX_IMGS];
    int Ho[RF_MAX_IMGS], Wo[RF_MAX_IMGS];
    long long out_pix[RF_MAX_IMGS + 1];
    int R, S, pad, stride, Cin, Cout, relu, round_out;
    int kc1, stride2;
    long long plane;
    const float* bias;
    const void* residual;
    void* y;
    unsigned long long* rowbest;
    unsigned long long* colbest;
    int NA, NB;
};
static_assert(sizeof(WgParams) <= 32764, "kernel parameter space (CUDA 12.1+ large kernel parameters)");

template <int KIND, int BN, int MODE>
struct WgCfg {
    static constexpr int NPL = (KIND == K_SPLIT || KIND == K_TF32X3) ? 2 : 1;
    static constexpr int A_BYTES = NPL * TC_A_BYTES;
    static constexpr int B_PLANE = BN * 128;
    static constexpr int STAGE_BYTES = A_BYTES + NPL * B_PLANE;
    static constexpr bool ONE_CTA = MODE == MODE_CORR || NPL * BN >= 256;
    static constexpr int BUDGET = ONE_CTA ? 200 * 1024 : 100 * 1024;
    static constexpr int STAGES = BUDGET / STAGE_BYTES > 6 ? 6 : BUDGET / STAGE_BYTES;
    static constexpr int CTAS_PER_SM = ONE_CTA ? 1 : 2;
    static constexpr int SMEM_BYTES = STAGES * STAGE_BYTES + 1024  + 256 ;
    static_assert(STAGES >= 2 && SMEM_BYTES <= 227 * 1024, "shared memory");
};

__device__ __forceinline__ __half2 pack_sat(float a, float b) {
    uint32_t r;
    asm("cvt.rn.satfinite.f16x2.f32 %0, %1, %2;" : "=r"(r) : "f"(b), "f"(a));
    return *reinterpret_cast<__half2*>(&r);
}
__device__ __forceinline__ void split2(float a, float b, __half2& hi, __half2& lo) {
    hi = pack_sat(a, b);
    const float2 f = __half22float2(hi);
    lo = pack_sat((a - f.x) * 2048.f, (b - f.y) * 2048.f);
}

template <int KIND, int BN, int NACC>
__device__ __forceinline__ void mma_block(float (&acc)[NACC][BN / 2], uint32_t sa, uint32_t sb) {
    constexpr bool TF32 = KIND == K_TF32 || KIND == K_TF32X3;
#pragma unroll
    for (int k = 0; k < 4; ++k) {
        const uint64_t ah = wg_desc(sa + 32 * k), bh = wg_desc(sb + 32 * k);
        if constexpr (KIND == K_SPLIT || KIND == K_TF32X3) {
            const uint64_t al = wg_desc(sa + TC_A_BYTES + 32 * k), bl = wg_desc(sb + BN * 128 + 32 * k);
            float (&x)[BN / 2] = acc[NACC - 1];
            wgmma<TF32, BN>(x, al, bh);
            wgmma<TF32, BN>(x, ah, bl);
            wgmma<TF32, BN>(acc[0], ah, bh);
        } else {
            wgmma<TF32, BN>(acc[0], ah, bh);
        }
    }
}

template <int KIND, int BN, int MODE, int OUT>
__global__ void __launch_bounds__(WG_THREADS, WgCfg<KIND, BN, MODE>::CTAS_PER_SM)
wg_kernel(const __grid_constant__ WgParams p) {
    using Cfg = WgCfg<KIND, BN, MODE>;
    constexpr int STAGES = Cfg::STAGES;
    constexpr int BK = (KIND == K_TF32 || KIND == K_TF32X3) ? TC_BK : TC_BK_F16;
    constexpr int NACC = KIND == K_SPLIT ? 2 : 1;
    constexpr bool SLOT = MODE == MODE_CONV && OUT != O_F32;
    constexpr int BOX_BYTES = (OUT == O_SPLIT ? 2 : 1) * 128 * 128;
    static_assert(!SLOT || (BN / 64) * BOX_BYTES <= Cfg::STAGE_BYTES, "the output tile fits one stage");
    extern __shared__ uint8_t smem_raw[];
    uint8_t* smem = smem_raw + ((1024u - (smem_u32(smem_raw) & 1023u)) & 1023u);
    uint64_t* full = reinterpret_cast<uint64_t*>(smem + STAGES * Cfg::STAGE_BYTES);
    uint64_t* empty = full + STAGES;
    const int warp = threadIdx.x >> 5, lane = threadIdx.x & 31;
    const int kc = p.Cin / BK;
    const int KI = p.R * p.S * kc;

    const int t_first = MODE == MODE_CORR ? 0 : (int)blockIdx.x;
    const int t_step = MODE == MODE_CORR ? 1 : (int)gridDim.x;
    const int t_end = MODE == MODE_CORR ? 1 : p.ntiles;
    struct Tile { int img, tw, ox0, oy0, n0; };
    auto decode = [&](int t) {
        const int mtile = MODE == MODE_CORR ? (int)blockIdx.y : t % p.tiles;
        const int ntile = MODE == MODE_CORR ? (int)blockIdx.x : t / p.tiles;
        Tile T;
        T.img = 0;
#pragma unroll
        for (int j = 1; j < RF_MAX_IMGS; ++j) T.img += (j < p.nimg && mtile >= p.tile_start[j]) ? 1 : 0;
        const int tloc = mtile - p.tile_start[T.img];
        T.tw = p.tw[T.img];
        const int tyi = tloc / p.tiles_x[T.img], txi = tloc - tyi * p.tiles_x[T.img];
        T.ox0 = txi * T.tw;
        T.oy0 = tyi * (128 / T.tw);
        T.n0 = ntile * BN;
        return T;
    };
    auto boxes = [&](const Tile& T) { return BN == 64 || T.n0 + 64 >= p.Cout ? 1 : 2; };

    if (threadIdx.x == 0) {
        for (int s = 0; s < STAGES; ++s) { mbar_init(&full[s], 1); mbar_init(&empty[s], 256); }
        fence_barrier_init();
    }
    __syncthreads();

    if (warp == 8) {
        if (lane == 0) {
            tma_prefetch_desc(&p.mapB);
            uint32_t prefetched = 0;
            int st = 0;
            uint32_t ph = 0;
            for (int t = t_first; t < t_end; t += t_step) {
                const Tile T = decode(t);
                if (!((prefetched >> T.img) & 1u)) {
                    prefetched |= 1u << T.img;
                    tma_prefetch_desc(&p.mapA[T.img]);
                    if constexpr (SLOT) {
                        tma_prefetch_desc(&p.mapY[T.img]);
                        if (p.residual) tma_prefetch_desc(&p.mapR[T.img]);
                    }
                }
                for (int it = 0; it < KI; ++it) {
                    mbar_wait(&empty[st], ph ^ 1);
                    uint8_t* sa = smem + st * Cfg::STAGE_BYTES;
                    uint8_t* sb = sa + Cfg::A_BYTES;
                    mbar_expect_tx(&full[st], Cfg::STAGE_BYTES);
                    if constexpr (MODE == MODE_CORR) {
                        const int c0 = it * BK;
                        tma_load_3d(sa, &p.mapA[0], &full[st], c0, T.ox0, 0);
                        tma_load_3d(sa + TC_A_BYTES, &p.mapA2[0], &full[st], c0, T.ox0, 0);
                        tma_load_2d(sb, &p.mapB, &full[st], c0, T.n0);
                        tma_load_2d(sb + Cfg::B_PLANE, &p.mapBlo, &full[st], c0, T.n0);
                    } else {
                        const int tap = it / kc, cc = it - tap * kc;
                        const int r = tap / p.S, s = tap - r * p.S;
                        const int c0 = cc * BK, x = T.ox0 * p.stride + s - p.pad, y = T.oy0 * p.stride + r - p.pad;
                        const int kcol = tap * p.Cin + c0;
                        if constexpr (KIND == K_SPLIT) {
                            if (cc < p.kc1) tma_load_4d(sa, &p.mapA[T.img], &full[st], c0, x, y, 0);
                            else tma_load_4d(sa, &p.mapA2[T.img], &full[st], (cc - p.kc1) * BK, T.ox0 * p.stride2, T.oy0 * p.stride2, 0);
                            tma_load_3d(sb, &p.mapB, &full[st], kcol, T.n0, 0);
                        } else {
                            tma_load_3d(sa, &p.mapA[T.img], &full[st], c0, x, y);
                            tma_load_2d(sb, &p.mapB, &full[st], kcol, T.n0);
                        }
                    }
                    if (++st == STAGES) { st = 0; ph ^= 1; }
                }
                if constexpr (SLOT) {
                    mbar_wait(&empty[st], ph ^ 1);
                    if (p.residual) {
                        const int nb = boxes(T);
                        uint8_t* slot = smem + st * Cfg::STAGE_BYTES;
                        mbar_expect_tx(&full[st], nb * BOX_BYTES);
                        for (int b = 0; b < nb; ++b) {
                            if constexpr (OUT == O_SPLIT) tma_load_4d(slot + b * BOX_BYTES, &p.mapR[T.img], &full[st], T.n0 + 64 * b, T.ox0, T.oy0, 0);
                            else tma_load_3d(slot + b * BOX_BYTES, &p.mapR[T.img], &full[st], T.n0 + 64 * b, T.ox0, T.oy0);
                        }
                    } else {
                        mbar_arrive(&full[st]);
                    }
                    if (++st == STAGES) { st = 0; ph ^= 1; }
                }
            }
        }
        return;
    }

    const int g = warp >> 2;
    const int rbase = 64 * g + 16 * (warp & 3) + (lane >> 2);
    const int cbase = 2 * (lane & 3);
    auto before = [](int s) { return s == 0 ? STAGES - 1 : s - 1; };
    int st = 0;
    uint32_t ph = 0;
    bool stored = false;
    for (int t = t_first; t < t_end; t += t_step) {
        const Tile T = decode(t);
        float acc[NACC][BN / 2];
#pragma unroll
        for (int a = 0; a < NACC; ++a)
#pragma unroll
            for (int i = 0; i < BN / 2; ++i) acc[a][i] = 0.f;
        for (int it = 0; it < KI; ++it) {
            mbar_wait(&full[st], ph);
            const uint32_t sa = smem_u32(smem + st * Cfg::STAGE_BYTES);
            wg_fence();
            mma_block<KIND, BN, NACC>(acc, sa + g * (64 * 128), sa + Cfg::A_BYTES);
            wg_commit();
            wg_wait<1>();
            if (it > 0) {
                mbar_arrive(&empty[before(st)]);
            } else if (SLOT && stored) {
                if (threadIdx.x == 0) bulk_wait_read();
                mbar_arrive(&empty[before(st)]);
            }
            if (++st == STAGES) { st = 0; ph ^= 1; }
        }
        wg_wait<0>();
#pragma unroll
        for (int a = 0; a < NACC; ++a) wg_fence_regs(acc[a]);
        mbar_arrive(&empty[before(st)]);

        auto value = [&](int i) -> float {
            if constexpr (KIND == K_SPLIT) return fmaf(acc[1][i], 0.00048828125f, acc[0][i]);
            else return acc[0][i];
        };

        if constexpr (SLOT) {
            mbar_wait(&full[st], ph);
            uint8_t* slot = smem + st * Cfg::STAGE_BYTES;
#pragma unroll
            for (int h = 0; h < 2; ++h) {
                const int m = rbase + 8 * h;
#pragma unroll
                for (int j = 0; j < BN / 8; ++j) {
                    const int c = 8 * j + cbase, n = T.n0 + c;
                    if (n >= p.Cout) continue;
                    float v0 = value(4 * j + 2 * h), v1 = value(4 * j + 2 * h + 1);
                    if (p.bias) { v0 += __ldg(p.bias + n); v1 += __ldg(p.bias + n + 1); }
                    uint8_t* e = slot + (c >> 6) * BOX_BYTES + m * 128 + ((((c & 63) >> 3) ^ (m & 7)) << 4) + (c & 7) * 2;
                    if (p.residual) {
                        if constexpr (OUT == O_F16) {
                            const float2 r = __half22float2(*reinterpret_cast<const __half2*>(e));
                            v0 += r.x; v1 += r.y;
                        } else {
                            const float2 rh = __half22float2(*reinterpret_cast<const __half2*>(e));
                            const float2 rl = __half22float2(*reinterpret_cast<const __half2*>(e + 128 * 128));
                            v0 += fmaf(rl.x, 0.00048828125f, rh.x); v1 += fmaf(rl.y, 0.00048828125f, rh.y);
                        }
                    }
                    if (p.relu) { v0 = fmaxf(v0, 0.f); v1 = fmaxf(v1, 0.f); }
                    if constexpr (OUT == O_F16) {
                        *reinterpret_cast<__half2*>(e) = pack_sat(v0, v1);
                    } else {
                        __half2 hi, lo;
                        split2(v0, v1, hi, lo);
                        *reinterpret_cast<__half2*>(e) = hi;
                        *reinterpret_cast<__half2*>(e + 128 * 128) = lo;
                    }
                }
            }
            fence_proxy_async();
            asm volatile("bar.sync 1, 256;" ::: "memory");
            if (threadIdx.x == 0) {
                const int nb = boxes(T);
                for (int b = 0; b < nb; ++b) {
                    if constexpr (OUT == O_SPLIT) tma_store_4d(&p.mapY[T.img], slot + b * BOX_BYTES, T.n0 + 64 * b, T.ox0, T.oy0, 0);
                    else tma_store_3d(&p.mapY[T.img], slot + b * BOX_BYTES, T.n0 + 64 * b, T.ox0, T.oy0);
                }
                bulk_commit();
            }
            stored = true;
            if (++st == STAGES) { st = 0; ph ^= 1; }
        } else if constexpr (MODE == MODE_CONV) {
            const int img = T.img, tw = T.tw;
#pragma unroll
            for (int h = 0; h < 2; ++h) {
                const int m = rbase + 8 * h;
                const int py = m / tw, px = m - py * tw;
                const int oy = T.oy0 + py, ox = T.ox0 + px;
                if (oy >= p.Ho[img] || ox >= p.Wo[img]) continue;
                const long long pix = p.out_pix[img] + (long long)oy * p.Wo[img] + ox;
#pragma unroll
                for (int j = 0; j < BN / 8; ++j) {
                    const int n = T.n0 + 8 * j + cbase;
                    if (n >= p.Cout) continue;
                    const bool two = n + 1 < p.Cout;
                    float v0 = value(4 * j + 2 * h), v1 = value(4 * j + 2 * h + 1);
                    if (p.bias) { v0 += __ldg(p.bias + n); if (two) v1 += __ldg(p.bias + n + 1); }
                    const long long o = pix * p.Cout + n;
                    if (p.residual) {
                        const float* r = static_cast<const float*>(p.residual) + o;
                        v0 += __ldg(r); if (two) v1 += __ldg(r + 1);
                    }
                    if (p.relu) { v0 = fmaxf(v0, 0.f); v1 = fmaxf(v1, 0.f); }
                    if (p.round_out) { v0 = round_tf32(v0); v1 = round_tf32(v1); }
                    float* y = static_cast<float*>(p.y) + o;
                    if (two && (p.Cout & 1) == 0) *reinterpret_cast<float2*>(y) = make_float2(v0, v1);
                    else { y[0] = v0; if (two) y[1] = v1; }
                }
            }
        } else {
            const int n0 = T.n0;
            unsigned long long* sCol = reinterpret_cast<unsigned long long*>(smem);
            const int row0 = T.ox0 + rbase, row1 = row0 + 8;
            const bool rv0 = row0 < p.NA, rv1 = row1 < p.NA;
            unsigned long long rb0 = 0ull, rb1 = 0ull;
            asm volatile("bar.sync 1, 256;" ::: "memory");
#pragma unroll
            for (int j = 0; j < BN / 8; ++j) {
#pragma unroll
                for (int e = 0; e < 2; ++e) {
                    const int c = 8 * j + cbase + e, col = n0 + c;
                    const bool cv = col < p.NB;
                    const float s0 = value(4 * j + e), s1 = value(4 * j + 2 + e);
                    unsigned long long ck = 0ull;
                    if (cv) {
                        if (rv0) { const unsigned long long k = pack_key(s0, (uint32_t)col); rb0 = k > rb0 ? k : rb0; ck = pack_key(s0, (uint32_t)row0); }
                        if (rv1) { const unsigned long long k = pack_key(s1, (uint32_t)col); rb1 = k > rb1 ? k : rb1;
                                   const unsigned long long k1 = pack_key(s1, (uint32_t)row1); ck = k1 > ck ? k1 : ck; }
                    }
#pragma unroll
                    for (int off = 4; off < 32; off <<= 1) {
                        const unsigned long long o = __shfl_xor_sync(0xffffffffu, ck, off);
                        ck = o > ck ? o : ck;
                    }
                    if (lane < 4) sCol[warp * BN + c] = ck;
                }
            }
#pragma unroll
            for (int off = 1; off < 4; off <<= 1) {
                const unsigned long long o0 = __shfl_xor_sync(0xffffffffu, rb0, off), o1 = __shfl_xor_sync(0xffffffffu, rb1, off);
                rb0 = o0 > rb0 ? o0 : rb0;
                rb1 = o1 > rb1 ? o1 : rb1;
            }
            if ((lane & 3) == 0) {
                if (rv0 && rb0 != 0ull) atomicMax(p.rowbest + row0, rb0);
                if (rv1 && rb1 != 0ull) atomicMax(p.rowbest + row1, rb1);
            }
            asm volatile("bar.sync 1, 256;" ::: "memory");
            for (int c = threadIdx.x; c < BN; c += 256) {
                if (n0 + c >= p.NB) continue;
                unsigned long long cb = 0ull;
#pragma unroll
                for (int w = 0; w < 8; ++w) { const unsigned long long k = sCol[w * BN + c]; cb = k > cb ? k : cb; }
                if (cb != 0ull) atomicMax(p.colbest + n0 + c, cb);
            }
        }
    }
    if constexpr (SLOT)
        if (threadIdx.x == 0) bulk_wait();
}


constexpr int SS_TW = 16, SS_TH = 8, SS_K = 7, SS_C = 3, SS_KK = 147, SS_KB = 3;
constexpr int SS_IN_W = ((SS_TW - 1) * 2 + SS_K) * SS_C;
constexpr int SS_IN_H = (SS_TH - 1) * 2 + SS_K;
constexpr int SS_IN_LD = 112;
constexpr int SS_THREADS = 256;
constexpr int SS_B_PLANE = 64 * 128;
constexpr int SS_OFF_ALO = SS_KB * TC_A_BYTES;
constexpr int SS_OFF_B = 2 * SS_KB * TC_A_BYTES;
constexpr int SS_OFF_IN = SS_OFF_B + SS_KB * 2 * SS_B_PLANE;
constexpr int SS_OFF_BAR = SS_OFF_IN + SS_IN_H * SS_IN_LD * 4;
constexpr int SS_SMEM = SS_OFF_BAR + 64 + 1024;
constexpr int SS_NLD = (SS_IN_H * SS_IN_W + SS_THREADS - 1) / SS_THREADS;
static_assert(SS_SMEM <= 227 * 1024, "stem shared memory");

struct alignas(64) StemParams {
    CUtensorMap mapB;
    int nimg;
    int tile_start[RF_MAX_IMGS + 1];
    int tiles_x[RF_MAX_IMGS];
    int H[RF_MAX_IMGS], W[RF_MAX_IMGS], Ho[RF_MAX_IMGS], Wo[RF_MAX_IMGS];
    long long in_pix[RF_MAX_IMGS], out_pix[RF_MAX_IMGS];
    long long plane;
    const float* x;
    const float* bias;
    __half* y;
};

__device__ __forceinline__ uint32_t stem_pack_split(float v) {
    __half2 hi, lo;
    split2(v, 0.f, hi, lo);
    return (*reinterpret_cast<uint32_t*>(&hi) & 0xFFFFu) | (*reinterpret_cast<uint32_t*>(&lo) << 16);
}

template <int HALF, int kb>
__device__ __forceinline__ void stem_build_half(const uint32_t* __restrict__ base, uint8_t* sA, int m) {
#pragma unroll
    for (int cc = 0; cc < 4; ++cc) {
        const int c8 = HALF * 4 + cc;
        uint4 oh, ol;
        uint32_t* ph = reinterpret_cast<uint32_t*>(&oh);
        uint32_t* pl = reinterpret_cast<uint32_t*>(&ol);
#pragma unroll
        for (int e = 0; e < 4; ++e) {
            const int k0 = kb * 64 + c8 * 8 + 2 * e, k1 = k0 + 1;
            const uint32_t a = k0 < SS_KK ? base[(k0 / 21) * SS_IN_LD + (k0 % 21)] : 0u;
            const uint32_t b = k1 < SS_KK ? base[(k1 / 21) * SS_IN_LD + (k1 % 21)] : 0u;
            ph[e] = __byte_perm(a, b, 0x5410);
            pl[e] = __byte_perm(a, b, 0x7632);
        }
        uint8_t* dst = sA + kb * TC_A_BYTES + m * 128 + ((c8 ^ (m & 7)) << 4);
        *reinterpret_cast<uint4*>(dst) = oh;
        *reinterpret_cast<uint4*>(dst + SS_OFF_ALO) = ol;
    }
}

template <bool SPLIT>
__global__ void __launch_bounds__(SS_THREADS, 1)
stem7_kernel(const __grid_constant__ StemParams p) {
    constexpr int NPL = SPLIT ? 2 : 1;
    extern __shared__ uint8_t smem_raw[];
    uint8_t* smem = smem_raw + ((1024u - (smem_u32(smem_raw) & 1023u)) & 1023u);
    uint8_t* sA = smem;
    uint8_t* sB = smem + SS_OFF_B;
    uint32_t* sIn = reinterpret_cast<uint32_t*>(smem + SS_OFF_IN);
    uint64_t* bar_b = reinterpret_cast<uint64_t*>(smem + SS_OFF_BAR);
    const int t = threadIdx.x, warp = t >> 5, lane = t & 31;

    int img = 0;
#pragma unroll
    for (int j = 1; j < RF_MAX_IMGS; ++j) img += (j < p.nimg && (int)blockIdx.x >= p.tile_start[j]) ? 1 : 0;
    const int tloc = blockIdx.x - p.tile_start[img];
    const int tyi = tloc / p.tiles_x[img], txi = tloc - tyi * p.tiles_x[img];
    const int ox0 = txi * SS_TW, oy0 = tyi * SS_TH;

    if (t == 0) {
        mbar_init(bar_b, 1);
        fence_barrier_init();
    }
    __syncthreads();
    if (t == 0) {
        mbar_expect_tx(bar_b, SS_KB * NPL * SS_B_PLANE);
#pragma unroll
        for (int kb = 0; kb < SS_KB; ++kb) {
            if constexpr (SPLIT) tma_load_3d(sB + kb * 2 * SS_B_PLANE, &p.mapB, bar_b, kb * 64, 0, 0);
            else tma_load_2d(sB + kb * SS_B_PLANE, &p.mapB, bar_b, kb * 64, 0);
        }
    }
    {
        const int H = p.H[img], WC = p.W[img] * SS_C;
        const float* src = p.x + p.in_pix[img] * SS_C;
        const int iy0 = oy0 * 2 - 3, col0 = (ox0 * 2 - 3) * SS_C;
#pragma unroll
        for (int i = 0; i < SS_NLD; ++i) {
            const int idx = t + i * SS_THREADS;
            const int r = idx / SS_IN_W, j = idx - r * SS_IN_W;
            const int iy = iy0 + r, col = col0 + j;
            if (idx < SS_IN_H * SS_IN_W)
                sIn[r * SS_IN_LD + j] = stem_pack_split((iy >= 0 && iy < H && col >= 0 && col < WC) ? __ldg(src + (long long)iy * WC + col) : 0.f);
        }
    }
    __syncthreads();
    {
        const int m = t & 127, py = m >> 4, px = m & 15;
        const uint32_t* base = sIn + (2 * py) * SS_IN_LD + 6 * px;
        if (t < 128) { stem_build_half<0, 0>(base, sA, m); stem_build_half<0, 1>(base, sA, m); stem_build_half<0, 2>(base, sA, m); }
        else { stem_build_half<1, 0>(base, sA, m); stem_build_half<1, 1>(base, sA, m); stem_build_half<1, 2>(base, sA, m); }
    }
    fence_proxy_async();
    __syncthreads();
    mbar_wait(bar_b, 0);

    const int g = warp >> 2;
    constexpr int NACC = SPLIT ? 2 : 1;
    float acc[NACC][32];
#pragma unroll
    for (int a = 0; a < NACC; ++a)
#pragma unroll
        for (int i = 0; i < 32; ++i) acc[a][i] = 0.f;
    wg_fence();
#pragma unroll
    for (int kb = 0; kb < SS_KB; ++kb) {
        const uint32_t a = smem_u32(sA + kb * TC_A_BYTES + g * (64 * 128)), b = smem_u32(sB + kb * NPL * SS_B_PLANE);
#pragma unroll
        for (int k = 0; k < 4; ++k) {
            const uint64_t ah = wg_desc(a + 32 * k), bh = wg_desc(b + 32 * k);
            if constexpr (SPLIT) {
                wgmma<false, 64>(acc[1], wg_desc(a + SS_OFF_ALO + 32 * k), bh);
                wgmma<false, 64>(acc[1], ah, wg_desc(b + SS_B_PLANE + 32 * k));
            }
            wgmma<false, 64>(acc[0], ah, bh);
        }
    }
    wg_commit();
    wg_wait<0>();
#pragma unroll
    for (int a = 0; a < NACC; ++a) wg_fence_regs(acc[a]);

    const int rbase = 64 * g + 16 * (warp & 3) + (lane >> 2), cbase = 2 * (lane & 3);
#pragma unroll
    for (int h = 0; h < 2; ++h) {
        const int m = rbase + 8 * h;
        const int oy = oy0 + (m >> 4), ox = ox0 + (m & 15);
        if (oy >= p.Ho[img] || ox >= p.Wo[img]) continue;
        __half* y = p.y + (p.out_pix[img] + (long long)oy * p.Wo[img] + ox) * 64;
#pragma unroll
        for (int j = 0; j < 8; ++j) {
            const int n = 8 * j + cbase, i = 4 * j + 2 * h;
            float v0 = SPLIT ? fmaf(acc[NACC - 1][i], 0.00048828125f, acc[0][i]) : acc[0][i];
            float v1 = SPLIT ? fmaf(acc[NACC - 1][i + 1], 0.00048828125f, acc[0][i + 1]) : acc[0][i + 1];
            if (p.bias) { v0 += __ldg(p.bias + n); v1 += __ldg(p.bias + n + 1); }
            v0 = fmaxf(v0, 0.f);
            v1 = fmaxf(v1, 0.f);
            if constexpr (SPLIT) {
                __half2 hi, lo;
                split2(v0, v1, hi, lo);
                *reinterpret_cast<__half2*>(y + n) = hi;
                *reinterpret_cast<__half2*>(y + p.plane + n) = lo;
            } else {
                *reinterpret_cast<__half2*>(y + n) = pack_sat(v0, v1);
            }
        }
    }
}


__global__ void split_tf32_kernel(const float4* __restrict__ x, float4* __restrict__ hi, float4* __restrict__ lo, long long n4) {
    long long i = (long long)blockIdx.x * blockDim.x + threadIdx.x;
    if (i >= n4) return;
    float4 v = __ldg(x + i), h, l;
    h.x = __uint_as_float(__float_as_uint(v.x) & 0xFFFFE000u); l.x = v.x - h.x;
    h.y = __uint_as_float(__float_as_uint(v.y) & 0xFFFFE000u); l.y = v.y - h.y;
    h.z = __uint_as_float(__float_as_uint(v.z) & 0xFFFFE000u); l.z = v.z - h.z;
    h.w = __uint_as_float(__float_as_uint(v.w) & 0xFFFFE000u); l.w = v.w - h.w;
    hi[i] = h;
    lo[i] = l;
}

__global__ void split_f16_all_kernel(const float4* __restrict__ A, const float4* __restrict__ B, uint2* __restrict__ Ahi, uint2* __restrict__ Alo,
                                     uint2* __restrict__ Bhi, uint2* __restrict__ Blo, long long na4, long long nb4,
                                     unsigned long long* __restrict__ keys, long long nkeys) {
    const long long i = (long long)blockIdx.x * blockDim.x + threadIdx.x;
    if (i < nkeys) keys[i] = 0ull;
    if (i >= na4 + nb4) return;
    const bool isA = i < na4;
    const long long k = isA ? i : i - na4;
    const float4 v = __ldg((isA ? A : B) + k);
    const __half2 h0 = __floats2half2_rn(v.x, v.y), h1 = __floats2half2_rn(v.z, v.w);
    const float2 f0 = __half22float2(h0), f1 = __half22float2(h1);
    const __half2 l0 = __floats2half2_rn((v.x - f0.x) * 2048.f, (v.y - f0.y) * 2048.f);
    const __half2 l1 = __floats2half2_rn((v.z - f1.x) * 2048.f, (v.w - f1.y) * 2048.f);
    uint2 ho, lo2;
    ho.x = *reinterpret_cast<const uint32_t*>(&h0); ho.y = *reinterpret_cast<const uint32_t*>(&h1);
    lo2.x = *reinterpret_cast<const uint32_t*>(&l0); lo2.y = *reinterpret_cast<const uint32_t*>(&l1);
    (isA ? Ahi : Bhi)[k] = ho;
    (isA ? Alo : Blo)[k] = lo2;
}

typedef CUresult (*EncodeTiledFn)(CUtensorMap*, CUtensorMapDataType, cuuint32_t, void*, const cuuint64_t*, const cuuint64_t*,
                                  const cuuint32_t*, const cuuint32_t*, CUtensorMapInterleave, CUtensorMapSwizzle,
                                  CUtensorMapL2promotion, CUtensorMapFloatOOBfill);

static EncodeTiledFn get_encode() {
    static EncodeTiledFn fn = nullptr;
    if (!fn) {
        void* ptr = nullptr;
        cudaDriverEntryPointQueryResult q;
        if (cudaGetDriverEntryPoint("cuTensorMapEncodeTiled", &ptr, cudaEnableDefault, &q) == cudaSuccess && q == cudaDriverEntryPointSuccess)
            fn = reinterpret_cast<EncodeTiledFn>(ptr);
    }
    return fn;
}

struct MapKey {
    const void* ptr;
    unsigned long long d0, d1, d2, d3, plane;
    unsigned b0, b1, b2, b3, es, esize;
    bool operator==(const MapKey& o) const {
        return ptr == o.ptr && d0 == o.d0 && d1 == o.d1 && d2 == o.d2 && d3 == o.d3 && plane == o.plane && b0 == o.b0 && b1 == o.b1 && b2 == o.b2 &&
               b3 == o.b3 && es == o.es && esize == o.esize;
    }
};
struct MapKeyHash {
    size_t operator()(const MapKey& k) const {
        size_t h = std::hash<const void*>()(k.ptr);
        auto mix = [&](unsigned long long v) { h ^= std::hash<unsigned long long>()(v) + 0x9e3779b97f4a7c15ull + (h << 6) + (h >> 2); };
        mix(k.d0); mix(k.d1); mix(k.d2); mix(k.d3); mix(k.plane); mix(k.b0); mix(k.b1); mix(k.b2); mix(k.b3); mix(k.es); mix(k.esize);
        return h;
    }
};
static std::mutex g_map_mu;
static std::unordered_map<MapKey, CUtensorMap, MapKeyHash> g_maps;

int get_map4(CUtensorMap* out, const void* ptr, unsigned long long d0, unsigned long long d1, unsigned long long d2, unsigned long long d3,
             unsigned long long plane_bytes, unsigned b0, unsigned b1, unsigned b2, unsigned b3, unsigned es_, unsigned esize) {
    MapKey key{ptr, d0, d1, d2, d3, plane_bytes, b0, b1, b2, b3, es_, esize};
    std::lock_guard<std::mutex> g(g_map_mu);
    auto it = g_maps.find(key);
    if (it != g_maps.end()) { *out = it->second; return 0; }
    EncodeTiledFn enc = get_encode();
    if (!enc) return fail_msg("cuTensorMapEncodeTiled is not available from this driver");
    cuuint64_t dims[4] = {d0, d1, d2, d3};
    cuuint64_t strides[3] = {d0 * (unsigned long long)esize, d0 * d1 * (unsigned long long)esize, plane_bytes};
    cuuint32_t box[4] = {b0, b1 * es_, b2 * es_, b3};
    cuuint32_t es[4] = {1, es_, es_, 1};
    int rank = d3 > 0 ? 4 : (d2 > 0 ? 3 : 2);
    CUresult r = enc(out, esize == 2 ? CU_TENSOR_MAP_DATA_TYPE_FLOAT16 : CU_TENSOR_MAP_DATA_TYPE_FLOAT32, rank, const_cast<void*>(ptr), dims, strides, box, es,
                     CU_TENSOR_MAP_INTERLEAVE_NONE, CU_TENSOR_MAP_SWIZZLE_128B, CU_TENSOR_MAP_L2_PROMOTION_L2_256B,
                     CU_TENSOR_MAP_FLOAT_OOB_FILL_NONE);
    if (r != CUDA_SUCCESS) {
        snprintf(g_err, sizeof(g_err), "cuTensorMapEncodeTiled failed with CUresult %d (dims %llu,%llu,%llu,%llu box %u,%u,%u,%u)", (int)r, d0, d1, d2, d3, b0, b1, b2, b3);
        return 3;
    }
    if (g_maps.size() > 8192) g_maps.clear();
    g_maps[key] = *out;
    return 0;
}

int get_map(CUtensorMap* out, const void* ptr, unsigned long long d0, unsigned long long d1, unsigned long long d2,
            unsigned b0, unsigned b1, unsigned b2, unsigned es_, unsigned esize) {
    return get_map4(out, ptr, d0, d1, d2, 0, 0, b0, b1, b2, 0, es_, esize);
}

int pick_tw(int Ho, int Wo) {
    int best = 16;
    long long best_area = -1;
    const int cands[5] = {16, 32, 8, 64, 128};
    for (int i = 0; i < 5; ++i) {
        int tw = cands[i], th = 128 / tw;
        long long area = (long long)((Wo + tw - 1) / tw) * ((Ho + th - 1) / th);
        if (best_area < 0 || area < best_area) { best_area = area; best = tw; }
    }
    return best;
}

template <int KIND, int BN, int MODE, int OUT>
static int launch_wg(const WgParams& p, dim3 grid, cudaStream_t st) {
    using Cfg = WgCfg<KIND, BN, MODE>;
    static bool attr[64] = {false};
    const int dev = current_device();
    if (!attr[dev]) {
        RF_CUDA(cudaFuncSetAttribute(wg_kernel<KIND, BN, MODE, OUT>, cudaFuncAttributeMaxDynamicSharedMemorySize, Cfg::SMEM_BYTES));
        attr[dev] = true;
    }
    wg_kernel<KIND, BN, MODE, OUT><<<grid, WG_THREADS, Cfg::SMEM_BYTES, st>>>(p);
    RF_LAUNCHED();
    return 0;
}

template <int KIND, int BN, int OUT>
static int launch_conv_bn(const WgParams& p, cudaStream_t st) {
    const int resident = WgCfg<KIND, BN, MODE_CONV>::CTAS_PER_SM * num_sms();
    return launch_wg<KIND, BN, MODE_CONV, OUT>(p, dim3(p.ntiles < resident ? p.ntiles : resident), st);
}
template <int KIND, int OUT>
static int launch_conv(const WgParams& p, int BN, cudaStream_t st) {
    return BN == 128 ? launch_conv_bn<KIND, 128, OUT>(p, st) : launch_conv_bn<KIND, 64, OUT>(p, st);
}

struct SplitDual { const void* x2; const int* hw2; int Cin2, stride2; };

static int conv_impl(const ImgSet& set, const ConvParams& cp, const void* w, cudaStream_t st, int kind, bool out32, const SplitDual* dual) {
    WgParams p;
    memset(&p, 0, sizeof(p));
    const bool split = kind == K_SPLIT;
    const unsigned esz = kind == K_TF32 ? 4u : 2u;
    const unsigned bk = kind == K_TF32 ? TC_BK : TC_BK_F16;
    const int BN = cp.Cout > 64 ? 128 : 64;
    const char* xb = reinterpret_cast<const char*>(cp.x);
    const unsigned long long in_plane = (unsigned long long)set.in_pix[set.n] * cp.Cin * 2ull;
    long long in2_pix[RF_MAX_IMGS + 1] = {0};
    if (dual)
        for (int i = 0; i < set.n; ++i) in2_pix[i + 1] = in2_pix[i] + (long long)dual->hw2[2 * i] * dual->hw2[2 * i + 1];
    const unsigned long long in2_plane = dual ? (unsigned long long)in2_pix[set.n] * dual->Cin2 * 2ull : 0ull;
    p.nimg = set.n;
    const bool tma_out = kind != K_TF32 && !out32;
    const unsigned long long out_plane = (unsigned long long)set.out_pix[set.n] * cp.Cout * 2ull;
    const char* yb = reinterpret_cast<const char*>(cp.y);
    const char* rb = reinterpret_cast<const char*>(cp.residual);
    int tiles = 0;
    for (int i = 0; i < set.n; ++i) {
        const int tw = pick_tw(set.Ho[i], set.Wo[i]), th = 128 / tw;
        p.tw[i] = tw;
        p.tiles_x[i] = (set.Wo[i] + tw - 1) / tw;
        p.tile_start[i] = tiles;
        tiles += p.tiles_x[i] * ((set.Ho[i] + th - 1) / th);
        p.Ho[i] = set.Ho[i]; p.Wo[i] = set.Wo[i];
        p.out_pix[i] = set.out_pix[i];
        int rc = split ? get_map4(&p.mapA[i], xb + set.in_pix[i] * cp.Cin * 2, (unsigned long long)cp.Cin, (unsigned long long)set.W[i],
                                  (unsigned long long)set.H[i], 2, in_plane, bk, (unsigned)tw, (unsigned)th, 2, (unsigned)cp.stride, 2)
                       : get_map(&p.mapA[i], xb + set.in_pix[i] * cp.Cin * esz, (unsigned long long)cp.Cin, (unsigned long long)set.W[i],
                                 (unsigned long long)set.H[i], bk, (unsigned)tw, (unsigned)th, (unsigned)cp.stride, esz);
        if (!rc && dual)
            rc = get_map4(&p.mapA2[i], static_cast<const char*>(dual->x2) + in2_pix[i] * dual->Cin2 * 2, (unsigned long long)dual->Cin2,
                          (unsigned long long)dual->hw2[2 * i + 1], (unsigned long long)dual->hw2[2 * i], 2, in2_plane, bk, (unsigned)tw,
                          (unsigned)th, 2, (unsigned)dual->stride2, 2);
        const long long o = set.out_pix[i] * cp.Cout * 2;
        for (int m = 0; m < (cp.residual ? 2 : 1) && tma_out && !rc; ++m) {
            CUtensorMap* map = m == 0 ? &p.mapY[i] : &p.mapR[i];
            const void* base = (m == 0 ? yb : rb) + o;
            rc = split ? get_map4(map, base, (unsigned long long)cp.Cout, (unsigned long long)set.Wo[i], (unsigned long long)set.Ho[i], 2,
                                  out_plane, 64, (unsigned)tw, (unsigned)th, 2, 1, 2)
                       : get_map(map, base, (unsigned long long)cp.Cout, (unsigned long long)set.Wo[i], (unsigned long long)set.Ho[i],
                                 64, (unsigned)tw, (unsigned)th, 1, 2);
        }
        if (rc) return rc;
    }
    RF_REQUIRE(tiles > 0, "rf_conv2d_nhwc: empty output");
    for (int i = set.n; i <= RF_MAX_IMGS; ++i) p.tile_start[i] = tiles;
    p.out_pix[set.n] = set.out_pix[set.n];
    int rc = split ? get_map(&p.mapB, w, (unsigned long long)cp.K, (unsigned long long)cp.Cout, 2, bk, (unsigned)BN, 2, 1, 2)
                   : get_map(&p.mapB, w, (unsigned long long)cp.K, (unsigned long long)cp.Cout, 0, bk, (unsigned)BN, 0, 1, esz);
    if (rc) return rc;
    p.R = cp.R; p.S = cp.S; p.pad = cp.pad; p.stride = cp.stride; p.Cin = cp.Cin; p.Cout = cp.Cout; p.relu = cp.relu; p.round_out = cp.round_out;
    p.kc1 = cp.Cin / (int)bk;
    p.stride2 = 1;
    if (dual) { p.Cin = cp.Cin + dual->Cin2; p.stride2 = dual->stride2; }
    p.plane = (long long)set.out_pix[set.n] * cp.Cout;
    p.bias = cp.bias; p.residual = cp.residual; p.y = cp.y;
    p.tiles = tiles;
    p.ntiles = tiles * ((cp.Cout + BN - 1) / BN);
    if (kind == K_TF32) return launch_conv<K_TF32, O_F32>(p, BN, st);
    if (kind == K_F16) return out32 ? launch_conv<K_F16, O_F32>(p, BN, st) : launch_conv<K_F16, O_F16>(p, BN, st);
    return out32 ? launch_conv<K_SPLIT, O_F32>(p, BN, st) : launch_conv<K_SPLIT, O_SPLIT>(p, BN, st);
}

template <bool SPLIT>
static int stem_impl(const float* x, int nimg, const int* hw_host, const void* w, const float* bias, void* y, void* stream) {
    RF_REQUIRE(x != nullptr && w != nullptr && y != nullptr, "rf_stem7: null pointer");
    RF_REQUIRE(((uintptr_t)y % 16) == 0 && ((uintptr_t)w % 16) == 0, "rf_stem7: pointers must be 16-byte aligned");
    ImgSet set;
    RF_REQUIRE(make_imgset(set, nimg, hw_host, 7, 2, 3) == 0, "rf_stem7: bad image set");
    StemParams p;
    memset(&p, 0, sizeof(p));
    p.nimg = nimg;
    int tiles = 0;
    for (int i = 0; i < nimg; ++i) {
        p.tiles_x[i] = (set.Wo[i] + SS_TW - 1) / SS_TW;
        p.tile_start[i] = tiles;
        tiles += p.tiles_x[i] * ((set.Ho[i] + SS_TH - 1) / SS_TH);
        p.H[i] = set.H[i]; p.W[i] = set.W[i]; p.Ho[i] = set.Ho[i]; p.Wo[i] = set.Wo[i];
        p.in_pix[i] = set.in_pix[i];
        p.out_pix[i] = set.out_pix[i];
    }
    for (int i = nimg; i <= RF_MAX_IMGS; ++i) p.tile_start[i] = tiles;
    int rc = SPLIT ? get_map(&p.mapB, w, 192ull, 64ull, 2, 64, 64, 2, 1, 2) : get_map(&p.mapB, w, 192ull, 64ull, 0, 64, 64, 0, 1, 2);
    if (rc) return rc;
    p.plane = set.out_pix[nimg] * 64;
    p.x = x; p.bias = bias; p.y = static_cast<__half*>(y);
    static bool attr[64] = {false};
    const int dev = current_device();
    if (!attr[dev]) {
        RF_CUDA(cudaFuncSetAttribute(stem7_kernel<SPLIT>, cudaFuncAttributeMaxDynamicSharedMemorySize, SS_SMEM));
        attr[dev] = true;
    }
    stem7_kernel<SPLIT><<<tiles, SS_THREADS, SS_SMEM, as_stream(stream)>>>(p);
    RF_LAUNCHED();
    return 0;
}

}

using namespace rf;

bool rf_conv2d_tc_supported(const ConvParams& p) {
    return (p.stride == 1 || p.stride == 2) && (p.Cin % TC_BK) == 0 && p.Cout >= 1 && p.R == p.S && (p.R == 1 || p.R == 3);
}
bool rf_conv2d_f16_supported(const ConvParams& p) {
    return (p.stride == 1 || p.stride == 2) && (p.Cin % TC_BK_F16) == 0 && p.Cout >= 8 && (p.Cout % 8) == 0 && p.R == p.S && (p.R == 1 || p.R == 3);
}
bool rf_conv2d_split_supported(const ConvParams& p) {
    return (p.stride == 1 || p.stride == 2) && (p.Cin % TC_BK_F16) == 0 && p.Cout >= 1 && p.R == p.S && (p.R == 1 || p.R == 3);
}

int rf_conv2d_tc(const ImgSet& set, const ConvParams& cp, const void* w_tc, cudaStream_t st, bool f16, bool out32) {
    RF_REQUIRE(w_tc != nullptr, "rf_conv2d_nhwc: tensor-core engines need w_tc ([Cout][R*S*Cin])");
    RF_REQUIRE(f16 ? rf_conv2d_f16_supported(cp) : rf_conv2d_tc_supported(cp),
               "rf_conv2d_nhwc: tensor-core engines need stride 1 or 2, 1x1 or 3x3, Cin % 32 == 0 (fp16: Cin % 64 == 0, Cout % 8 == 0)");
    RF_REQUIRE(!out32 || (f16 && cp.R == 3 && cp.stride == 1 && cp.pad == 1 && cp.residual == nullptr),
               "rf_conv2d_nhwc: engine 3 (fp16 operands, fp32 output) covers 3x3 / stride 1 / pad 1 layers without residual");
    RF_REQUIRE(!f16 || (((uintptr_t)cp.x % 16) == 0 && ((uintptr_t)cp.y % 16) == 0 && ((uintptr_t)cp.residual % 16) == 0),
               "rf_conv2d_nhwc: engine 2 needs 16-byte aligned x / y / residual");
    return conv_impl(set, cp, w_tc, st, f16 ? K_F16 : K_TF32, out32, nullptr);
}

int rf_conv2d_split(const ImgSet& set, const ConvParams& cp, const void* w_split, cudaStream_t st, bool out32) {
    RF_REQUIRE(w_split != nullptr, "rf_conv2d_nhwc: engine 4 needs the split weights ([2][Cout][R*S*Cin] fp16)");
    RF_REQUIRE(rf_conv2d_split_supported(cp), "rf_conv2d_nhwc: engine 4 needs stride 1 or 2, 1x1 or 3x3, Cin % 64 == 0");
    RF_REQUIRE(out32 || (cp.Cout % 8) == 0, "rf_conv2d_nhwc: engine 4 needs Cout % 8 == 0 for split outputs");
    RF_REQUIRE(!out32 || cp.residual == nullptr, "rf_conv2d_nhwc: engine 4 fp32 outputs take no residual");
    RF_REQUIRE(((uintptr_t)cp.x % 16) == 0 && ((uintptr_t)cp.y % 16) == 0 && ((uintptr_t)cp.residual % 16) == 0 && ((uintptr_t)w_split % 16) == 0,
               "rf_conv2d_nhwc: engine 4 needs 16-byte aligned pointers");
    return conv_impl(set, cp, w_split, st, K_SPLIT, out32, nullptr);
}

extern "C" int rf_conv1x1_dual_split(const void* x1, const void* x2, int nimg, const int* hw1_host, const int* hw2_host, int Cin1, int Cin2,
                                     int stride2, const void* w_split, const float* bias, int Cout, int relu, void* y, void* stream) {
    RF_REQUIRE(x1 != nullptr && x2 != nullptr && y != nullptr && hw1_host != nullptr && hw2_host != nullptr && w_split != nullptr,
               "rf_conv1x1_dual_split: null pointer");
    RF_REQUIRE(Cin1 >= 1 && Cin2 >= 1 && Cout >= 1, "rf_conv1x1_dual_split: bad channel counts");
    RF_REQUIRE((Cin1 % TC_BK_F16) == 0 && (Cin2 % TC_BK_F16) == 0 && (Cout % 8) == 0 && (stride2 == 1 || stride2 == 2),
               "rf_conv1x1_dual_split: Cin1 % 64 == 0, Cin2 % 64 == 0, Cout % 8 == 0, stride2 1 or 2");
    RF_REQUIRE(((uintptr_t)x1 % 16) == 0 && ((uintptr_t)x2 % 16) == 0 && ((uintptr_t)y % 16) == 0 && ((uintptr_t)w_split % 16) == 0,
               "rf_conv1x1_dual_split: pointers must be 16-byte aligned");
    ImgSet set;
    RF_REQUIRE(make_imgset(set, nimg, hw1_host, 1, 1, 0) == 0, "rf_conv1x1_dual_split: bad image set");
    for (int i = 0; i < nimg; ++i)
        RF_REQUIRE((hw2_host[2 * i] - 1) / stride2 + 1 == set.Ho[i] && (hw2_host[2 * i + 1] - 1) / stride2 + 1 == set.Wo[i],
                   "rf_conv1x1_dual_split: the second input, sampled with stride2, must have the first input's size");
    ConvParams p;
    p.x = static_cast<const float*>(x1); p.w = nullptr; p.bias = bias; p.residual = nullptr; p.y = static_cast<float*>(y);
    p.Cin = Cin1; p.Cout = Cout; p.R = 1; p.S = 1; p.stride = 1; p.pad = 0; p.relu = relu;
    p.round_out = 0;
    p.Mtot = set.out_pix[nimg];
    p.K = Cin1 + Cin2;
    SplitDual dual{x2, hw2_host, Cin2, stride2};
    return conv_impl(set, p, w_split, as_stream(stream), K_SPLIT, false, &dual);
}

int rf_stem7_f16_impl(const float* x, int nimg, const int* hw_host, const void* w_f16, const float* bias, void* y_f16, void* stream) {
    return stem_impl<false>(x, nimg, hw_host, w_f16, bias, y_f16, stream);
}
int rf_stem7_split_impl(const float* x, int nimg, const int* hw_host, const void* w_split, const float* bias, void* y_split, void* stream) {
    return stem_impl<true>(x, nimg, hw_host, w_split, bias, y_split, stream);
}

size_t rf_corr_tc_workspace(int NA, int NB, int C) { return 2ull * ((size_t)NA + NB) * C * sizeof(float) + 1024; }

int rf_corr_argmax_tc(const float* featA, int NA, const float* featB, int NB, int C,
                      unsigned long long* rowbest, unsigned long long* colbest, void* ws, cudaStream_t st, int precision,
                      const void* const* presplit) {
    const bool f16 = precision == 2;
    RF_REQUIRE(presplit == nullptr || f16, "rf_corr_mutual_nn: pre-split operands go with the fp16-split kernel (precision 2)");
    RF_REQUIRE((C % (f16 ? TC_BK_F16 : TC_BK)) == 0, "rf_corr_mutual_nn: precision 1 needs C % 32 == 0, precision 2 C % 64 == 0");
    uintptr_t base = (reinterpret_cast<uintptr_t>(ws) + 255) & ~(uintptr_t)255;
    const size_t esz = f16 ? 2 : 4;
    char* Ahi = reinterpret_cast<char*>(base);
    char* Alo = Ahi + (size_t)NA * C * esz;
    char* Bhi = Alo + (size_t)NA * C * esz;
    char* Blo = Bhi + (size_t)NB * C * esz;
    long long na4 = (long long)NA * C / 4, nb4 = (long long)NB * C / 4;
    if (presplit != nullptr) {
        Ahi = const_cast<char*>(static_cast<const char*>(presplit[0]));
        Alo = const_cast<char*>(static_cast<const char*>(presplit[1]));
        Bhi = const_cast<char*>(static_cast<const char*>(presplit[2]));
        Blo = const_cast<char*>(static_cast<const char*>(presplit[3]));
        for (int i = 0; i < 4; ++i) RF_REQUIRE(presplit[i] != nullptr && ((uintptr_t)presplit[i] % 16) == 0, "rf_corr_mutual_nn_presplit: planes must be 16-byte aligned");
    } else if (f16) {
        RF_REQUIRE(colbest == rowbest + NA, "rf_corr_mutual_nn: arg-max keys must be contiguous");
        const long long nkeys = (long long)NA + NB, n = na4 + nb4 > nkeys ? na4 + nb4 : nkeys;
        split_f16_all_kernel<<<(unsigned)((n + 255) / 256), 256, 0, st>>>((const float4*)featA, (const float4*)featB, (uint2*)Ahi, (uint2*)Alo,
                                                                            (uint2*)Bhi, (uint2*)Blo, na4, nb4, rowbest, nkeys);
        RF_LAUNCHED();
    } else {
        split_tf32_kernel<<<(unsigned)((na4 + 255) / 256), 256, 0, st>>>((const float4*)featA, (float4*)Ahi, (float4*)Alo, na4);
        RF_LAUNCHED();
        split_tf32_kernel<<<(unsigned)((nb4 + 255) / 256), 256, 0, st>>>((const float4*)featB, (float4*)Bhi, (float4*)Blo, nb4);
        RF_LAUNCHED();
    }
    constexpr int BN = 128;
    const unsigned bk = f16 ? TC_BK_F16 : TC_BK, es = (unsigned)esz;
    WgParams p;
    memset(&p, 0, sizeof(p));
    p.nimg = 1;
    p.tw[0] = 128;
    p.tiles_x[0] = (NA + 127) / 128;
    for (int i = 1; i <= RF_MAX_IMGS; ++i) p.tile_start[i] = p.tiles_x[0];
    p.Ho[0] = 1; p.Wo[0] = NA;
    int rc = get_map(&p.mapA[0], Ahi, (unsigned long long)C, (unsigned long long)NA, 1, bk, 128, 1, 1, es);
    if (!rc) rc = get_map(&p.mapA2[0], Alo, (unsigned long long)C, (unsigned long long)NA, 1, bk, 128, 1, 1, es);
    if (!rc) rc = get_map(&p.mapB, Bhi, (unsigned long long)C, (unsigned long long)NB, 0, bk, BN, 0, 1, es);
    if (!rc) rc = get_map(&p.mapBlo, Blo, (unsigned long long)C, (unsigned long long)NB, 0, bk, BN, 0, 1, es);
    if (rc) return rc;
    p.R = 1; p.S = 1; p.pad = 0; p.stride = 1; p.Cin = C; p.Cout = NB;
    p.rowbest = rowbest; p.colbest = colbest; p.NA = NA; p.NB = NB;
    const dim3 grid((NB + BN - 1) / BN, p.tiles_x[0]);
    RF_REQUIRE(grid.y <= 65535u, "rf_corr_mutual_nn: NA > 8388480");
    if (f16) return launch_wg<K_SPLIT, BN, MODE_CORR, 0>(p, grid, st);
    return launch_wg<K_TF32X3, BN, MODE_CORR, 0>(p, grid, st);
}
```

ransac-flow_b200/csrc/runner.cu:

```cuda
#include "common.cuh"

using namespace rf;

int rf_im2col_impl(const float* x, int nimg, const int* hw_host, int C, int k, int stride, int pad, int Kpad, int round_out,
                   float* y, void* stream);
int rf_poolblur_impl(const float* x, int nimg, const int* hw_host, int C, int round_out, float* y, void* stream);
int rf_im2col_f16_impl(const float* x, int nimg, const int* hw_host, int C, int k, int stride, int pad, int Kpad, void* y_f16, void* stream);
int rf_maxpool_f16_impl(const void* x_f16, int nimg, const int* hw_host, int C, int k, int stride, int pad, void* y_f16, void* stream);
int rf_stem7_f16_impl(const float* x, int nimg, const int* hw_host, const void* w_f16, const float* bias, void* y_f16, void* stream);
int rf_blur_f16_impl(const void* x_f16, int nimg, const int* hw_host, int C, int stride, void* y_f16, void* stream);
int rf_poolblur_f16_impl(const void* x_f16, int nimg, const int* hw_host, int C, void* y_f16, void* stream);
int rf_stem7_split_impl(const float* x, int nimg, const int* hw_host, const void* w_split, const float* bias, void* y_split, void* stream);
int rf_blur_split_impl(const void* x, int nimg, const int* hw_host, int C, int stride, void* y, void* stream);
int rf_poolblur_split_impl(const void* x, int nimg, const int* hw_host, int C, void* y, void* stream);
int rf_maxpool_split_impl(const void* x, int nimg, const int* hw_host, int C, int k, int stride, int pad, void* y, void* stream);
int rf_im2col_split_impl(const float* x, int nimg, const int* hw_host, int C, int k, int stride, int pad, int Kpad, void* y, void* stream);
int rf_blur_downsample_impl(const float* x, int nimg, const int* hw_host, int C, int stride, int round_out, float* y, void* stream);

extern "C" int rf_run_layers(const rf_layer_t* L, int n, void* const* slots, int nimg, const int* hw_host, int engine, void* stream) {
    RF_REQUIRE(L != nullptr && n >= 1 && nimg >= 1 && nimg <= RF_MAX_IMGS, "rf_run_layers: bad arguments");
    static thread_local int hw[RF_MAX_SLOTS][2 * RF_MAX_IMGS];
    bool known[RF_MAX_SLOTS] = {false};
    RF_REQUIRE(L[0].src >= 0 && L[0].src < RF_MAX_SLOTS, "rf_run_layers: bad input slot");
    for (int i = 0; i < 2 * nimg; ++i) hw[L[0].src][i] = hw_host[i];
    known[L[0].src] = true;
    for (int li = 0; li < n; ++li) {
        const rf_layer_t& l = L[li];
        RF_REQUIRE(l.src >= 0 && l.src < RF_MAX_SLOTS && l.dst >= 0 && l.dst < RF_MAX_SLOTS && l.res < RF_MAX_SLOTS, "rf_run_layers: slot index out of range");
        RF_REQUIRE(known[l.src], "rf_run_layers: layer reads a slot nothing has written");
        RF_REQUIRE(l.dst != l.src && l.dst != l.res, "rf_run_layers: in-place layers are not supported");
        const int* shw = hw[l.src];
        const float* x = static_cast<const float*>(slots[l.src]);
        float* y = static_cast<float*>(slots[l.dst]);
        int rc = 0;
        int k = l.k, stride = l.stride, pad = l.pad;
        if (engine == RF_ENGINE_SPLIT) {
            if (l.op == RF_OP_CONV) {
                const float* res = l.res >= 0 ? static_cast<const float*>(slots[l.res]) : nullptr;
                rc = rf_conv2d_nhwc(x, nimg, shw, l.Cin, l.w, static_cast<const float*>(l.w_f16), l.bias, res, l.Cout, k, k, stride, pad, l.relu,
                                    (l.flags & RF_LAYER_OUT_F32) ? RF_ENGINE_SPLIT_OUT32 : RF_ENGINE_SPLIT, y, stream);
            } else if (l.op == RF_OP_CONV_DUAL) {
                RF_REQUIRE(l.src2 >= 0 && l.src2 < RF_MAX_SLOTS && known[l.src2] && l.dst != l.src2 && l.res < 0 && k == 1 && stride == 1 && pad == 0,
                           "rf_run_layers: RF_OP_CONV_DUAL needs a written second input slot, k = 1, stride 1, pad 0, no residual");
                rc = rf_conv1x1_dual_split(x, slots[l.src2], nimg, shw, hw[l.src2], l.Cin, l.Cin2, l.stride2, l.w_f16, l.bias, l.Cout, l.relu, y, stream);
            } else if (l.op == RF_OP_MAXPOOL) {
                rc = rf_maxpool_split_impl(x, nimg, shw, l.Cin, k, stride, pad, y, stream);
            } else if (l.op == RF_OP_BLUR) {
                k = 3; pad = 1;
                rc = rf_blur_split_impl(x, nimg, shw, l.Cin, stride, y, stream);
            } else if (l.op == RF_OP_POOLBLUR) {
                k = 4; stride = 2; pad = 1;
                rc = rf_poolblur_split_impl(x, nimg, shw, l.Cin, y, stream);
            } else if (l.op == RF_OP_STEM7) {
                RF_REQUIRE(l.src == L[0].src && l.Cin == 3 && l.Cout == 64 && k == 7 && stride == 2 && pad == 3 && l.relu,
                           "rf_run_layers: RF_OP_STEM7 is the ResNet-50 stem on the fp32 input slot");
                rc = rf_stem7_split_impl(x, nimg, shw, l.w_f16, l.bias, y, stream);
            } else if (l.op == RF_OP_IM2COL) {
                RF_REQUIRE(l.src == L[0].src, "rf_run_layers (engine 4): im2col reads the fp32 input slot");
                rc = rf_im2col_split_impl(x, nimg, shw, l.Cin, k, stride, pad, l.Cout, y, stream);
            } else {
                return fail_msg("rf_run_layers: unknown op");
            }
        } else if (engine == RF_ENGINE_F16) {
            if (l.op == RF_OP_CONV) {
                const float* res = l.res >= 0 ? static_cast<const float*>(slots[l.res]) : nullptr;
                if (l.flags & RF_LAYER_TF32)
                    rc = rf_conv2d_nhwc(x, nimg, shw, l.Cin, l.w, l.w_tc, l.bias, res, l.Cout, k, k, stride, pad, l.relu, RF_ENGINE_TF32, y, stream);
                else
                    rc = rf_conv2d_nhwc(x, nimg, shw, l.Cin, l.w, static_cast<const float*>(l.w_f16), l.bias, res, l.Cout, k, k, stride, pad, l.relu,
                                        (l.flags & RF_LAYER_OUT_F32) ? RF_ENGINE_F16_OUT32 : RF_ENGINE_F16, y, stream);
            } else if (l.op == RF_OP_MAXPOOL) {
                rc = rf_maxpool_f16_impl(x, nimg, shw, l.Cin, k, stride, pad, y, stream);
            } else if (l.op == RF_OP_BLUR) {
                k = 3; pad = 1;
                rc = rf_blur_f16_impl(x, nimg, shw, l.Cin, stride, y, stream);
            } else if (l.op == RF_OP_POOLBLUR) {
                k = 4; stride = 2; pad = 1;
                rc = rf_poolblur_f16_impl(x, nimg, shw, l.Cin, y, stream);
            } else if (l.op == RF_OP_STEM7) {
                RF_REQUIRE(l.src == L[0].src && l.Cin == 3 && l.Cout == 64 && k == 7 && stride == 2 && pad == 3 && l.relu,
                           "rf_run_layers: RF_OP_STEM7 is the ResNet-50 stem on the fp32 input slot");
                rc = rf_stem7_f16_impl(x, nimg, shw, l.w_f16, l.bias, y, stream);
            } else if (l.op == RF_OP_IM2COL) {
                RF_REQUIRE(l.src == L[0].src, "rf_run_layers (engine 2): im2col reads the fp32 input slot");
                rc = rf_im2col_f16_impl(x, nimg, shw, l.Cin, k, stride, pad, l.Cout, y, stream);
            } else {
                return fail_msg("rf_run_layers: unknown op");
            }
        } else if (l.op == RF_OP_CONV) {
            const float* res = l.res >= 0 ? static_cast<const float*>(slots[l.res]) : nullptr;
            rc = rf_conv2d_nhwc(x, nimg, shw, l.Cin, l.w, l.w_tc, l.bias, res, l.Cout, k, k, stride, pad, l.relu, engine, y, stream);
        } else if (l.op == RF_OP_MAXPOOL) {
            rc = rf_maxpool2d_nhwc(x, nimg, shw, l.Cin, k, stride, pad, y, stream);
        } else if (l.op == RF_OP_BLUR) {
            k = 3; pad = 1;
            rc = rf_blur_downsample_impl(x, nimg, shw, l.Cin, stride, engine == 1 ? 1 : 0, y, stream);
        } else if (l.op == RF_OP_POOLBLUR) {
            k = 4; stride = 2; pad = 1;
            rc = rf_poolblur_impl(x, nimg, shw, l.Cin, engine == 1 ? 1 : 0, y, stream);
        } else if (l.op == RF_OP_IM2COL) {
            rc = rf_im2col_impl(x, nimg, shw, l.Cin, k, stride, pad, l.Cout, engine == 1 ? 1 : 0, y, stream);
        } else {
            return fail_msg("rf_run_layers: unknown op");
        }
        if (rc) return rc;
        for (int i = 0; i < nimg; ++i) {
            hw[l.dst][2 * i] = (shw[2 * i] + 2 * pad - k) / stride + 1;
            hw[l.dst][2 * i + 1] = (shw[2 * i + 1] + 2 * pad - k) / stride + 1;
        }
        known[l.dst] = true;
    }
    return 0;
}
```

ransac-flow_b200/program.py:

```python
import ctypes as C

import torch

from ._lib import check, lib, need_cuda, stream

RF_OP_CONV, RF_OP_MAXPOOL, RF_OP_BLUR, RF_OP_IM2COL, RF_OP_POOLBLUR, RF_OP_STEM7, RF_OP_CONV_DUAL = 0, 1, 2, 3, 4, 5, 6
RF_MAX_SLOTS = 32
RF_LAYER_OUT_F32, RF_LAYER_TF32 = 1, 2


class rf_layer_t(C.Structure):
    _fields_ = [("op", C.c_int), ("src", C.c_int), ("dst", C.c_int), ("res", C.c_int),
                ("Cin", C.c_int), ("Cout", C.c_int), ("k", C.c_int), ("stride", C.c_int), ("pad", C.c_int), ("relu", C.c_int),
                ("w", C.c_void_p), ("w_tc", C.c_void_p), ("bias", C.c_void_p), ("w_f16", C.c_void_p), ("flags", C.c_int),
                ("src2", C.c_int), ("Cin2", C.c_int), ("stride2", C.c_int)]


lib.rf_run_layers.restype = C.c_int
lib.rf_run_layers.argtypes = [C.POINTER(rf_layer_t), C.c_int, C.POINTER(C.c_void_p), C.c_int, C.POINTER(C.c_int), C.c_int, C.c_void_p]


class LayerProgram:

    def __init__(self, cin, device=None):
        self.device = device
        self.ops = []
        self.chan = [cin]
        self._keep = []
        self.flags = {}
        self.dual = {}
        self._compiled = {}

    def conv(self, src, fc, relu, res=None, out_f32=False, tf32=False):
        assert self.chan[src] == fc.cin, (self.chan[src], fc.cin)
        self.flags[len(self.ops)] = (RF_LAYER_OUT_F32 if out_f32 else 0) | (RF_LAYER_TF32 if tf32 else 0)
        self.ops.append((RF_OP_CONV, src, -1 if res is None else res, fc.cin, fc.cout, fc.k, fc.stride, fc.pad, int(relu), fc))
        self._keep.append(fc)
        self.chan.append(fc.cout)
        return len(self.chan) - 1

    def conv_dual(self, src, src2, fc, stride2, relu):
        assert fc.k == 1 and self.chan[src] == fc.cin and self.chan[src2] == fc.cin2, (self.chan[src], self.chan[src2], fc.cin, fc.cin2)
        self.dual[len(self.ops)] = (src2, fc.cin2, stride2)
        self.ops.append((RF_OP_CONV_DUAL, src, -1, fc.cin, fc.cout, 1, 1, 0, int(relu), fc))
        self._keep.append(fc)
        self.chan.append(fc.cout)
        self.split_only = True
        return len(self.chan) - 1

    def maxpool(self, src, k, stride, pad):
        c = self.chan[src]
        self.ops.append((RF_OP_MAXPOOL, src, -1, c, c, k, stride, pad, 0, None))
        self.chan.append(c)
        return len(self.chan) - 1

    def poolblur(self, src):
        c = self.chan[src]
        self.ops.append((RF_OP_POOLBLUR, src, -1, c, c, 4, 2, 1, 0, None))
        self.chan.append(c)
        return len(self.chan) - 1

    def im2col(self, src, k, stride, pad, kpad):
        c = self.chan[src]
        assert kpad >= k * k * c
        self.ops.append((RF_OP_IM2COL, src, -1, c, kpad, k, stride, pad, 0, None))
        self.chan.append(kpad)
        return len(self.chan) - 1

    def stem(self, src, weight, bn, stride, pad, kalign=32):
        from .model import FoldedConv
        cout, cin, k, _ = weight.shape
        kpad = (k * k * cin + kalign - 1) // kalign * kalign
        dev = self.device or weight.device
        w = weight.detach().float().cpu().permute(0, 2, 3, 1).reshape(cout, k * k * cin)
        w = torch.nn.functional.pad(w, (0, kpad - k * k * cin)).reshape(cout, kpad, 1, 1)
        x = self.im2col(src, k, stride, pad, kpad)
        return self.conv(x, FoldedConv(w, bn, 1, pad=0, device=dev), relu=True)

    def stem7_fused(self, src, weight, bn):
        from .model import FoldedConv
        cout, cin, k, _ = weight.shape
        assert (cout, cin, k) == (64, 3, 7) and self.chan[src] == 3
        dev = self.device or weight.device
        w = weight.detach().float().cpu().permute(0, 2, 3, 1).reshape(cout, k * k * cin)
        w = torch.nn.functional.pad(w, (0, 192 - k * k * cin)).reshape(cout, 192, 1, 1)
        fc = FoldedConv(w, bn, 1, pad=0, device=dev)
        self.ops.append((RF_OP_STEM7, src, -1, 3, 64, 7, 2, 3, 1, fc))
        self._keep.append(fc)
        self.chan.append(64)
        self.f16_only = True
        return len(self.chan) - 1

    def blur(self, src, stride):
        c = self.chan[src]
        self.ops.append((RF_OP_BLUR, src, -1, c, c, 3, stride, 1, 0, None))
        self.chan.append(c)
        return len(self.chan) - 1

    def _compile(self, hw, device, f16=False, split=False):
        n_t = len(self.chan)
        last_use = [0] * n_t
        for i, o in enumerate(self.ops):
            last_use[o[1]] = i
            if o[2] >= 0:
                last_use[o[2]] = i
            if i in self.dual:
                last_use[self.dual[i][0]] = i
        last_use[n_t - 1] = len(self.ops)
        hws = [list(hw)]
        for o in self.ops:
            k, s, p = o[5], o[6], o[7]
            hws.append([((h + 2 * p - k) // s + 1, (w + 2 * p - k) // s + 1) for h, w in hws[o[1]]])
        esize = [4] * n_t
        if f16:
            esize[0] = 4 if self.ops[0][0] in (RF_OP_IM2COL, RF_OP_STEM7) else 2
            for i, o in enumerate(self.ops):
                fl = self.flags.get(i, 0)
                esize[i + 1] = 4 if fl else 2
                if fl & RF_LAYER_TF32:
                    assert esize[o[1]] == 4, "a TF32 layer under the fp16 engine needs an fp32 input (out_f32 on its producer)"
                elif o[0] not in (RF_OP_IM2COL, RF_OP_STEM7):
                    assert esize[o[1]] == 2 and (o[2] < 0 or esize[o[2]] == 2), "fp16 layer fed by an fp32 tensor"
        elems = [sum(h * w for h, w in hws[t]) * self.chan[t] * esize[t] for t in range(n_t)]
        slot_of, free, slot_elems = {0: 0}, [], [0]
        layers = (rf_layer_t * len(self.ops))()
        for i, o in enumerate(self.ops):
            t_out = i + 1
            if free:
                fit = [s for s in free if slot_elems[s] >= elems[t_out]]
                s = min(fit, key=lambda q: slot_elems[q]) if fit else max(free, key=lambda q: slot_elems[q])
                free.remove(s)
                slot_elems[s] = max(slot_elems[s], elems[t_out])
            else:
                s = len(slot_elems)
                slot_elems.append(elems[t_out])
            slot_of[t_out] = s
            L = layers[i]
            L.op, L.src, L.dst, L.res = o[0], slot_of[o[1]], s, (slot_of[o[2]] if o[2] >= 0 else -1)
            L.Cin, L.Cout, L.k, L.stride, L.pad, L.relu = o[3], o[4], o[5], o[6], o[7], o[8]
            fc = o[9]
            if fc is not None:
                L.w, L.w_tc = fc.w.data_ptr(), fc.w_tc.data_ptr()
                L.w_f16 = fc.w_f16.data_ptr() if f16 else (fc.w_split.data_ptr() if split else None)
                L.flags = self.flags.get(i, 0) if (f16 or split) else 0
                L.bias = fc.bias.data_ptr() if fc.bias is not None else None
            L.src2 = -1
            if i in self.dual:
                L.src2, L.Cin2, L.stride2 = slot_of[self.dual[i][0]], self.dual[i][1], self.dual[i][2]
            for t in {o[1], o[2], self.dual[i][0] if i in self.dual else -1}:
                if t > 0 and last_use[t] == i:
                    free.append(slot_of[t])
        assert len(slot_elems) <= RF_MAX_SLOTS
        bufs = [None] + [torch.empty(max(16, e), device=device, dtype=torch.uint8) for e in slot_elems[1:]]
        out_slot = slot_of[n_t - 1]
        chw = (C.c_int * (2 * len(hw)))(*[v for p in hw for v in p])
        out_split = split and not (self.flags.get(len(self.ops) - 1, 0) & RF_LAYER_OUT_F32)
        in_split = split and self.ops[0][0] not in (RF_OP_IM2COL, RF_OP_STEM7)
        return dict(layers=layers, bufs=bufs, out_slot=out_slot, out_hw=hws[-1], out_elems=elems[-1], chw=chw, nslots=len(slot_elems),
                    out_dtype=torch.float16 if (esize[-1] == 2 or out_split) else torch.float32, out_split=out_split,
                    in_dtype=torch.float16 if (esize[0] == 2 or in_split) else torch.float32)

    def run(self, x, engine):
        need_cuda(x.data)
        f16, split = int(engine) == 2, int(engine) == 4
        assert f16 or split or not getattr(self, "f16_only", False), "this program uses tensor-core-engine-only layers"
        assert split or not getattr(self, "split_only", False), "this program uses split-engine-only layers (conv_dual)"
        key = (tuple(x.hw), str(x.data.device), int(engine) if (f16 or split) else 0)
        if key not in self._compiled:
            self._compiled[key] = self._compile(x.hw, x.data.device, f16, split)
        c = self._compiled[key]
        self.__dict__.setdefault("_touched", set()).add(key)
        assert x.data.dtype == c["in_dtype"], (x.data.dtype, c["in_dtype"])
        slots = (C.c_void_p * c["nslots"])()
        slots[0] = x.data.data_ptr()
        for i in range(1, c["nslots"]):
            slots[i] = c["bufs"][i].data_ptr()
        check(lib.rf_run_layers(c["layers"], len(self.ops), slots, len(x.hw), c["chw"], int(engine), stream()))
        out = c["bufs"][c["out_slot"]][:c["out_elems"]].view(c["out_dtype"])
        out = out.view(2, -1, self.chan[-1]) if c["out_split"] else out.view(-1, self.chan[-1])
        return out, c["out_hw"]

    def release(self, keep=()):
        for k in [k for k in self._compiled if k not in keep]:
            del self._compiled[k]
```

Measured before the change: 111.7.

## Fuse ResNet stem 7x7 conv with following 3x3 max-pool in a persistent kernel

The stem convolution kernel becomes persistent: it loops over strip units, prefetches the next input window into registers while the current wgmma runs, and optionally max-pools the 32x4 output tile in shared memory before writing. This removes the full-resolution stem activation write/read and the separate maxpool launch. It costs overlapping halo recomputation between strips, extra shared memory for the tile buffers, and a more complex launch that is gridded by SM count.

```diff
diff --git a/include/ransacflow_b200.h b/include/ransacflow_b200.h
--- a/include/ransacflow_b200.h
+++ b/include/ransacflow_b200.h
@@ -78,6 +78,7 @@
 } rf_layer_t;
 #define RF_LAYER_OUT_F32 1
 #define RF_LAYER_TF32 2
+#define RF_LAYER_STEM_POOL 4
 int rf_run_layers(const rf_layer_t* layers_host, int n, void* const* slots_host, int nimg, const int* hw_host,
                   int engine, void* stream);
 int rf_maxpool2d_nhwc(const float* x, int nimg, const int* hw_host, int C, int k, int stride, int pad,
diff --git a/ransac-flow_b200/csrc/common.cuh b/ransac-flow_b200/csrc/common.cuh
--- a/ransac-flow_b200/csrc/common.cuh
+++ b/ransac-flow_b200/csrc/common.cuh
@@ -1,4 +1,5 @@
 #pragma once
+#include <cuda_fp16.h>
 #include <cuda_runtime.h>
 #include <stdint.h>
 #include <stdio.h>
@@ -38,6 +39,20 @@
         if (!(cond)) return rf::fail_msg(msg " [" #cond "]");           \
     } while (0)
 
+__device__ __forceinline__ void split_store8(__half* p, long long plane, const float (&v)[8]) {
+    uint4 th, tl;
+    __half2* h = reinterpret_cast<__half2*>(&th);
+    __half2* l = reinterpret_cast<__half2*>(&tl);
+#pragma unroll
+    for (int e = 0; e < 4; ++e) {
+        const float a = fminf(fmaxf(v[2 * e], -65504.f), 65504.f), b = fminf(fmaxf(v[2 * e + 1], -65504.f), 65504.f);
+        h[e] = __floats2half2_rn(a, b);
+        const float2 f = __half22float2(h[e]);
+        l[e] = __floats2half2_rn((a - f.x) * 2048.f, (b - f.y) * 2048.f);
+    }
+    *reinterpret_cast<uint4*>(p) = th;
+    *reinterpret_cast<uint4*>(p + plane) = tl;
+}
 inline cudaStream_t as_stream(void* s) { return reinterpret_cast<cudaStream_t>(s); }
 
 inline int current_device() {
diff --git a/ransac-flow_b200/csrc/elementwise.cu b/ransac-flow_b200/csrc/elementwise.cu
--- a/ransac-flow_b200/csrc/elementwise.cu
+++ b/ransac-flow_b200/csrc/elementwise.cu
@@ -131,20 +131,6 @@
     }
 };
 struct SplitH {};
-__device__ __forceinline__ void split_store8(__half* p, long long plane, const float (&v)[8]) {
-    uint4 th, tl;
-    __half2* h = reinterpret_cast<__half2*>(&th);
-    __half2* l = reinterpret_cast<__half2*>(&tl);
-#pragma unroll
-    for (int e = 0; e < 4; ++e) {
-        const float a = fminf(fmaxf(v[2 * e], -65504.f), 65504.f), b = fminf(fmaxf(v[2 * e + 1], -65504.f), 65504.f);
-        h[e] = __floats2half2_rn(a, b);
-        const float2 f = __half22float2(h[e]);
-        l[e] = __floats2half2_rn((a - f.x) * 2048.f, (b - f.y) * 2048.f);
-    }
-    *reinterpret_cast<uint4*>(p) = th;
-    *reinterpret_cast<uint4*>(p + plane) = tl;
-}
 __device__ __forceinline__ void split_load8(const __half* p, long long plane, float (&v)[8]) {
     const uint4 th = __ldg(reinterpret_cast<const uint4*>(p)), tl = __ldg(reinterpret_cast<const uint4*>(p + plane));
     const __half2* h = reinterpret_cast<const __half2*>(&th);
diff --git a/ransac-flow_b200/csrc/gemm_tc.cu b/ransac-flow_b200/csrc/gemm_tc.cu
--- a/ransac-flow_b200/csrc/gemm_tc.cu
+++ b/ransac-flow_b200/csrc/gemm_tc.cu
@@ -357,26 +357,32 @@
 }
 
 
-constexpr int SS_TW = 16, SS_TH = 8, SS_K = 7, SS_C = 3, SS_KK = 147, SS_KB = 3;
-constexpr int SS_IN_W = ((SS_TW - 1) * 2 + SS_K) * SS_C;
-constexpr int SS_IN_H = (SS_TH - 1) * 2 + SS_K;
-constexpr int SS_IN_LD = 112;
-constexpr int SS_THREADS = 256;
-constexpr int SS_B_PLANE = 64 * 128;
-constexpr int SS_OFF_ALO = SS_KB * TC_A_BYTES;
-constexpr int SS_OFF_B = 2 * SS_KB * TC_A_BYTES;
-constexpr int SS_OFF_IN = SS_OFF_B + SS_KB * 2 * SS_B_PLANE;
-constexpr int SS_OFF_BAR = SS_OFF_IN + SS_IN_H * SS_IN_LD * 4;
-constexpr int SS_SMEM = SS_OFF_BAR + 64 + 1024;
-constexpr int SS_NLD = (SS_IN_H * SS_IN_W + SS_THREADS - 1) / SS_THREADS;
-static_assert(SS_SMEM <= 227 * 1024, "stem shared memory");
+constexpr int ST_TW = 32, ST_TH = 4, ST_K = 7, ST_C = 3, ST_KK = 147, ST_KB = 3;
+constexpr int ST_PW = (ST_TW - 2) / 2, ST_PH = ST_TH / 2;
+constexpr int ST_IN_W = ((ST_TW - 1) * 2 + ST_K) * ST_C;
+constexpr int ST_IN_H = (ST_TH - 1) * 2 + ST_K;
+constexpr int ST_IN_LD = 208;
+constexpr int ST_THREADS = 256;
+constexpr int ST_B_PLANE = 64 * 128;
+constexpr int ST_OFF_ALO = ST_KB * TC_A_BYTES;
+constexpr int ST_OFF_B = 2 * ST_KB * TC_A_BYTES;
+constexpr int ST_OFF_T = ST_OFF_B + ST_KB * 2 * ST_B_PLANE;
+constexpr int ST_T_BYTES = 128 * 64 * 4;
+constexpr int ST_OFF_IN = ST_OFF_T + 2 * ST_T_BYTES;
+constexpr int ST_OFF_BAR = ST_OFF_IN + ST_IN_H * ST_IN_LD * 4;
+constexpr int ST_SMEM = ST_OFF_BAR + 64 + 1024;
+constexpr int ST_NLD = (ST_IN_H * ST_IN_W + ST_THREADS - 1) / ST_THREADS;
+static_assert(ST_SMEM <= 227 * 1024, "stem shared memory");
+static_assert(ST_PH * ST_PW * 8 <= ST_THREADS, "one thread per (pooled pixel, 8 channels) of a step");
 
 struct alignas(64) StemParams {
     CUtensorMap mapB;
-    int nimg;
-    int tile_start[RF_MAX_IMGS + 1];
-    int tiles_x[RF_MAX_IMGS];
-    int H[RF_MAX_IMGS], W[RF_MAX_IMGS], Ho[RF_MAX_IMGS], Wo[RF_MAX_IMGS];
+    int nimg, pool;
+    int unit_start[RF_MAX_IMGS + 1];
+    int steps[RF_MAX_IMGS];
+    int H[RF_MAX_IMGS], W[RF_MAX_IMGS];
+    int Hs[RF_MAX_IMGS], Ws[RF_MAX_IMGS];
+    int Ho[RF_MAX_IMGS], Wo[RF_MAX_IMGS];
     long long in_pix[RF_MAX_IMGS], out_pix[RF_MAX_IMGS];
     long long plane;
     const float* x;
@@ -390,7 +396,7 @@
     return (*reinterpret_cast<uint32_t*>(&hi) & 0xFFFFu) | (*reinterpret_cast<uint32_t*>(&lo) << 16);
 }
 
-template <int HALF, int kb>
+template <bool SPLIT, int HALF, int kb>
 __device__ __forceinline__ void stem_build_half(const uint32_t* __restrict__ base, uint8_t* sA, int m) {
 #pragma unroll
     for (int cc = 0; cc < 4; ++cc) {
@@ -401,35 +407,91 @@
 #pragma unroll
         for (int e = 0; e < 4; ++e) {
             const int k0 = kb * 64 + c8 * 8 + 2 * e, k1 = k0 + 1;
-            const uint32_t a = k0 < SS_KK ? base[(k0 / 21) * SS_IN_LD + (k0 % 21)] : 0u;
-            const uint32_t b = k1 < SS_KK ? base[(k1 / 21) * SS_IN_LD + (k1 % 21)] : 0u;
+            const uint32_t a = k0 < ST_KK ? base[(k0 / 21) * ST_IN_LD + (k0 % 21)] : 0u;
+            const uint32_t b = k1 < ST_KK ? base[(k1 / 21) * ST_IN_LD + (k1 % 21)] : 0u;
             ph[e] = __byte_perm(a, b, 0x5410);
             pl[e] = __byte_perm(a, b, 0x7632);
         }
         uint8_t* dst = sA + kb * TC_A_BYTES + m * 128 + ((c8 ^ (m & 7)) << 4);
         *reinterpret_cast<uint4*>(dst) = oh;
-        *reinterpret_cast<uint4*>(dst + SS_OFF_ALO) = ol;
-    }
+        if constexpr (SPLIT) *reinterpret_cast<uint4*>(dst + ST_OFF_ALO) = ol;
+    }
+}
+
+template <bool SPLIT, int kb, int NACC>
+__device__ __forceinline__ void stem_kblock(float (&acc)[NACC][32], const uint32_t* base, uint8_t* sA, const uint8_t* sB, int m, int half,
+                                            int g, uint64_t* bar_b, bool first) {
+    constexpr int NPL = SPLIT ? 2 : 1;
+    if (half == 0) stem_build_half<SPLIT, 0, kb>(base, sA, m);
+    else stem_build_half<SPLIT, 1, kb>(base, sA, m);
+    fence_proxy_async();
+    __syncthreads();
+    if (kb == 0 && first) mbar_wait(bar_b, 0);
+    wg_fence();
+    const uint32_t a = smem_u32(sA + kb * TC_A_BYTES + g * (64 * 128)), b = smem_u32(sB + kb * NPL * ST_B_PLANE);
+#pragma unroll
+    for (int k = 0; k < 4; ++k) {
+        const uint64_t ah = wg_desc(a + 32 * k), bh = wg_desc(b + 32 * k);
+        if constexpr (SPLIT) {
+            wgmma<false, 64>(acc[1], wg_desc(a + ST_OFF_ALO + 32 * k), bh);
+            wgmma<false, 64>(acc[1], ah, wg_desc(b + ST_B_PLANE + 32 * k));
+        }
+        wgmma<false, 64>(acc[0], ah, bh);
+    }
+    wg_commit();
 }
 
 template <bool SPLIT>
-__global__ void __launch_bounds__(SS_THREADS, 1)
+__global__ void __launch_bounds__(ST_THREADS, 1)
 stem7_kernel(const __grid_constant__ StemParams p) {
     constexpr int NPL = SPLIT ? 2 : 1;
+    constexpr int NACC = SPLIT ? 2 : 1;
+    constexpr int PIX_BYTES = SPLIT ? 256 : 128;
     extern __shared__ uint8_t smem_raw[];
     uint8_t* smem = smem_raw + ((1024u - (smem_u32(smem_raw) & 1023u)) & 1023u);
     uint8_t* sA = smem;
-    uint8_t* sB = smem + SS_OFF_B;
-    uint32_t* sIn = reinterpret_cast<uint32_t*>(smem + SS_OFF_IN);
-    uint64_t* bar_b = reinterpret_cast<uint64_t*>(smem + SS_OFF_BAR);
-    const int t = threadIdx.x, warp = t >> 5, lane = t & 31;
-
-    int img = 0;
-#pragma unroll
-    for (int j = 1; j < RF_MAX_IMGS; ++j) img += (j < p.nimg && (int)blockIdx.x >= p.tile_start[j]) ? 1 : 0;
-    const int tloc = blockIdx.x - p.tile_start[img];
-    const int tyi = tloc / p.tiles_x[img], txi = tloc - tyi * p.tiles_x[img];
-    const int ox0 = txi * SS_TW, oy0 = tyi * SS_TH;
+    uint8_t* sB = smem + ST_OFF_B;
+    uint8_t* sT = smem + ST_OFF_T;
+    uint32_t* sIn = reinterpret_cast<uint32_t*>(smem + ST_OFF_IN);
+    uint64_t* bar_b = reinterpret_cast<uint64_t*>(smem + ST_OFF_BAR);
+    const int t = threadIdx.x, warp = t >> 5, lane = t & 31, g = warp >> 2;
+    const long long units = p.unit_start[RF_MAX_IMGS];
+    const int u_begin = (int)(units * blockIdx.x / gridDim.x), u_end = (int)(units * (blockIdx.x + 1) / gridDim.x);
+
+    struct Unit { int img, strip, j, r0, c0; };
+    auto decode = [&](int u) {
+        Unit U;
+        U.img = 0;
+#pragma unroll
+        for (int i = 1; i < RF_MAX_IMGS; ++i) U.img += (i < p.nimg && u >= p.unit_start[i]) ? 1 : 0;
+        const int loc = u - p.unit_start[U.img];
+        U.strip = loc / p.steps[U.img];
+        U.j = loc - U.strip * p.steps[U.img];
+        U.r0 = U.j * ST_TH;
+        U.c0 = p.pool ? U.strip * 2 * ST_PW - 1 : U.strip * ST_TW;
+        return U;
+    };
+    float win[ST_NLD];
+    auto load_window = [&](const Unit& U) {
+        const int H = p.H[U.img], WC = p.W[U.img] * ST_C;
+        const float* src = p.x + p.in_pix[U.img] * ST_C;
+        const int iy0 = U.r0 * 2 - 3, col0 = (U.c0 * 2 - 3) * ST_C;
+#pragma unroll
+        for (int i = 0; i < ST_NLD; ++i) {
+            const int idx = t + i * ST_THREADS;
+            const int r = idx / ST_IN_W, jj = idx - r * ST_IN_W;
+            const int iy = iy0 + r, col = col0 + jj;
+            win[i] = (idx < ST_IN_H * ST_IN_W && iy >= 0 && iy < H && col >= 0 && col < WC) ? __ldg(src + (long long)iy * WC + col) : 0.f;
+        }
+    };
+    auto stage_window = [&]() {
+#pragma unroll
+        for (int i = 0; i < ST_NLD; ++i) {
+            const int idx = t + i * ST_THREADS;
+            const int r = idx / ST_IN_W, jj = idx - r * ST_IN_W;
+            if (idx < ST_IN_H * ST_IN_W) sIn[r * ST_IN_LD + jj] = stem_pack_split(win[i]);
+        }
+    };
 
     if (t == 0) {
         mbar_init(bar_b, 1);
@@ -437,90 +499,127 @@
     }
     __syncthreads();
     if (t == 0) {
-        mbar_expect_tx(bar_b, SS_KB * NPL * SS_B_PLANE);
-#pragma unroll
-        for (int kb = 0; kb < SS_KB; ++kb) {
-            if constexpr (SPLIT) tma_load_3d(sB + kb * 2 * SS_B_PLANE, &p.mapB, bar_b, kb * 64, 0, 0);
-            else tma_load_2d(sB + kb * SS_B_PLANE, &p.mapB, bar_b, kb * 64, 0);
-        }
-    }
-    {
-        const int H = p.H[img], WC = p.W[img] * SS_C;
-        const float* src = p.x + p.in_pix[img] * SS_C;
-        const int iy0 = oy0 * 2 - 3, col0 = (ox0 * 2 - 3) * SS_C;
-#pragma unroll
-        for (int i = 0; i < SS_NLD; ++i) {
-            const int idx = t + i * SS_THREADS;
-            const int r = idx / SS_IN_W, j = idx - r * SS_IN_W;
-            const int iy = iy0 + r, col = col0 + j;
-            if (idx < SS_IN_H * SS_IN_W)
-                sIn[r * SS_IN_LD + j] = stem_pack_split((iy >= 0 && iy < H && col >= 0 && col < WC) ? __ldg(src + (long long)iy * WC + col) : 0.f);
-        }
-    }
+        mbar_expect_tx(bar_b, ST_KB * NPL * ST_B_PLANE);
+#pragma unroll
+        for (int kb = 0; kb < ST_KB; ++kb) {
+            if constexpr (SPLIT) tma_load_3d(sB + kb * 2 * ST_B_PLANE, &p.mapB, bar_b, kb * 64, 0, 0);
+            else tma_load_2d(sB + kb * ST_B_PLANE, &p.mapB, bar_b, kb * 64, 0);
+        }
+    }
+    int u = u_begin;
+    Unit U = decode(u);
+    if (p.pool && U.j > 0) U = decode(--u);
+    load_window(U);
+    stage_window();
     __syncthreads();
-    {
-        const int m = t & 127, py = m >> 4, px = m & 15;
-        const uint32_t* base = sIn + (2 * py) * SS_IN_LD + 6 * px;
-        if (t < 128) { stem_build_half<0, 0>(base, sA, m); stem_build_half<0, 1>(base, sA, m); stem_build_half<0, 2>(base, sA, m); }
-        else { stem_build_half<1, 0>(base, sA, m); stem_build_half<1, 1>(base, sA, m); stem_build_half<1, 2>(base, sA, m); }
-    }
-    fence_proxy_async();
-    __syncthreads();
-    mbar_wait(bar_b, 0);
-
-    const int g = warp >> 2;
-    constexpr int NACC = SPLIT ? 2 : 1;
-    float acc[NACC][32];
-#pragma unroll
-    for (int a = 0; a < NACC; ++a)
-#pragma unroll
-        for (int i = 0; i < 32; ++i) acc[a][i] = 0.f;
-    wg_fence();
-#pragma unroll
-    for (int kb = 0; kb < SS_KB; ++kb) {
-        const uint32_t a = smem_u32(sA + kb * TC_A_BYTES + g * (64 * 128)), b = smem_u32(sB + kb * NPL * SS_B_PLANE);
-#pragma unroll
-        for (int k = 0; k < 4; ++k) {
-            const uint64_t ah = wg_desc(a + 32 * k), bh = wg_desc(b + 32 * k);
-            if constexpr (SPLIT) {
-                wgmma<false, 64>(acc[1], wg_desc(a + SS_OFF_ALO + 32 * k), bh);
-                wgmma<false, 64>(acc[1], ah, wg_desc(b + SS_B_PLANE + 32 * k));
-            }
-            wgmma<false, 64>(acc[0], ah, bh);
-        }
-    }
-    wg_commit();
-    wg_wait<0>();
-#pragma unroll
-    for (int a = 0; a < NACC; ++a) wg_fence_regs(acc[a]);
-
+
+    const int m = t & 127, half = t >> 7;
+    const uint32_t* base = sIn + (2 * (m >> 5)) * ST_IN_LD + 6 * (m & 31);
     const int rbase = 64 * g + 16 * (warp & 3) + (lane >> 2), cbase = 2 * (lane & 3);
-#pragma unroll
-    for (int h = 0; h < 2; ++h) {
-        const int m = rbase + 8 * h;
-        const int oy = oy0 + (m >> 4), ox = ox0 + (m & 15);
-        if (oy >= p.Ho[img] || ox >= p.Wo[img]) continue;
-        __half* y = p.y + (p.out_pix[img] + (long long)oy * p.Wo[img] + ox) * 64;
-#pragma unroll
-        for (int j = 0; j < 8; ++j) {
-            const int n = 8 * j + cbase, i = 4 * j + 2 * h;
-            float v0 = SPLIT ? fmaf(acc[NACC - 1][i], 0.00048828125f, acc[0][i]) : acc[0][i];
-            float v1 = SPLIT ? fmaf(acc[NACC - 1][i + 1], 0.00048828125f, acc[0][i + 1]) : acc[0][i + 1];
-            if (p.bias) { v0 += __ldg(p.bias + n); v1 += __ldg(p.bias + n + 1); }
-            v0 = fmaxf(v0, 0.f);
-            v1 = fmaxf(v1, 0.f);
-            if constexpr (SPLIT) {
-                __half2 hi, lo;
-                split2(v0, v1, hi, lo);
-                *reinterpret_cast<__half2*>(y + n) = hi;
-                *reinterpret_cast<__half2*>(y + p.plane + n) = lo;
-            } else {
-                *reinterpret_cast<__half2*>(y + n) = pack_sat(v0, v1);
-            }
-        }
-    }
-}
-
+    int buf = 0;
+    for (bool first = true; u < u_end; ++u, first = false) {
+        float acc[NACC][32];
+#pragma unroll
+        for (int a = 0; a < NACC; ++a)
+#pragma unroll
+            for (int i = 0; i < 32; ++i) acc[a][i] = 0.f;
+        stem_kblock<SPLIT, 0>(acc, base, sA, sB, m, half, g, bar_b, first);
+        stem_kblock<SPLIT, 1>(acc, base, sA, sB, m, half, g, bar_b, first);
+        stem_kblock<SPLIT, 2>(acc, base, sA, sB, m, half, g, bar_b, first);
+        const bool more = u + 1 < u_end;
+        Unit N = U;
+        if (more) {
+            N = decode(u + 1);
+            load_window(N);
+        }
+        wg_wait<0>();
+#pragma unroll
+        for (int a = 0; a < NACC; ++a) wg_fence_regs(acc[a]);
+
+        const int img = U.img;
+        uint8_t* tile = sT + buf * ST_T_BYTES;
+#pragma unroll
+        for (int h = 0; h < 2; ++h) {
+            const int mm = rbase + 8 * h;
+            const int oy = U.r0 + (mm >> 5), ox = U.c0 + (mm & 31);
+            __half* y = p.y + (p.out_pix[img] + (long long)oy * p.Wo[img] + ox) * 64;
+            const bool store = !p.pool && oy < p.Hs[img] && ox < p.Ws[img];
+#pragma unroll
+            for (int j = 0; j < 8; ++j) {
+                const int n = 8 * j + cbase, i = 4 * j + 2 * h;
+                float v0 = SPLIT ? fmaf(acc[NACC - 1][i], 0.00048828125f, acc[0][i]) : acc[0][i];
+                float v1 = SPLIT ? fmaf(acc[NACC - 1][i + 1], 0.00048828125f, acc[0][i + 1]) : acc[0][i + 1];
+                if (p.bias) { v0 += __ldg(p.bias + n); v1 += __ldg(p.bias + n + 1); }
+                v0 = fmaxf(v0, 0.f);
+                v1 = fmaxf(v1, 0.f);
+                if constexpr (SPLIT) {
+                    __half2 hi, lo;
+                    split2(v0, v1, hi, lo);
+                    if (p.pool) {
+                        const float2 fh = __half22float2(hi), fl = __half22float2(lo);
+                        *reinterpret_cast<float2*>(tile + mm * PIX_BYTES + (((n >> 2) ^ (mm & 7)) << 4) + (n & 3) * 4) =
+                            make_float2(fmaf(fl.x, 0.00048828125f, fh.x), fmaf(fl.y, 0.00048828125f, fh.y));
+                    } else if (store) {
+                        *reinterpret_cast<__half2*>(y + n) = hi;
+                        *reinterpret_cast<__half2*>(y + p.plane + n) = lo;
+                    }
+                } else {
+                    if (p.pool) *reinterpret_cast<__half2*>(tile + mm * PIX_BYTES + ((j ^ (mm & 7)) << 4) + cbase * 2) = pack_sat(v0, v1);
+                    else if (store) *reinterpret_cast<__half2*>(y + n) = pack_sat(v0, v1);
+                }
+            }
+        }
+        if (more) stage_window();
+        __syncthreads();
+
+        if (p.pool && u >= u_begin && t < ST_PH * ST_PW * 8) {
+            const int oct = t & 7, q = t >> 3, pr = q / ST_PW, pc = q - pr * ST_PW;
+            const int oy = U.j * ST_PH + pr, ox = U.strip * ST_PW + pc;
+            if (oy < p.Ho[img] && ox < p.Wo[img]) {
+                float mx[8];
+#pragma unroll
+                for (int e = 0; e < 8; ++e) mx[e] = -INFINITY;
+                const __half2 ninf = __float2half2_rn(-INFINITY);
+                __half2 mh[4] = {ninf, ninf, ninf, ninf};
+#pragma unroll
+                for (int r = 0; r < 3; ++r) {
+                    const int tr = 2 * pr - 1 + r;
+                    if (U.r0 + tr < 0 || U.r0 + tr >= p.Hs[img]) continue;
+                    const uint8_t* trow = tr < 0 ? sT + (buf ^ 1) * ST_T_BYTES + 3 * 32 * PIX_BYTES : tile + tr * 32 * PIX_BYTES;
+#pragma unroll
+                    for (int s = 0; s < 3; ++s) {
+                        const int tc = 2 * pc + s;
+                        if (U.c0 + tc < 0 || U.c0 + tc >= p.Ws[img]) continue;
+                        const uint8_t* px = trow + tc * PIX_BYTES;
+                        if constexpr (SPLIT) {
+                            const float4 a = *reinterpret_cast<const float4*>(px + (((2 * oct) ^ (tc & 7)) << 4));
+                            const float4 b = *reinterpret_cast<const float4*>(px + (((2 * oct + 1) ^ (tc & 7)) << 4));
+                            mx[0] = fmaxf(mx[0], a.x); mx[1] = fmaxf(mx[1], a.y); mx[2] = fmaxf(mx[2], a.z); mx[3] = fmaxf(mx[3], a.w);
+                            mx[4] = fmaxf(mx[4], b.x); mx[5] = fmaxf(mx[5], b.y); mx[6] = fmaxf(mx[6], b.z); mx[7] = fmaxf(mx[7], b.w);
+                        } else {
+                            const uint4 v = *reinterpret_cast<const uint4*>(px + ((oct ^ (tc & 7)) << 4));
+                            const __half2* hv = reinterpret_cast<const __half2*>(&v);
+#pragma unroll
+                            for (int e = 0; e < 4; ++e) mh[e] = __hmax2(mh[e], hv[e]);
+                        }
+                    }
+                }
+                __half* y = p.y + (p.out_pix[img] + (long long)oy * p.Wo[img] + ox) * 64 + oct * 8;
+                if constexpr (SPLIT) {
+                    split_store8(y, p.plane, mx);
+                } else {
+                    uint4 o;
+                    __half2* ho = reinterpret_cast<__half2*>(&o);
+#pragma unroll
+                    for (int e = 0; e < 4; ++e) ho[e] = mh[e];
+                    *reinterpret_cast<uint4*>(y) = o;
+                }
+            }
+        }
+        buf ^= 1;
+        U = N;
+    }
+}
 
 __global__ void split_tf32_kernel(const float4* __restrict__ x, float4* __restrict__ hi, float4* __restrict__ lo, long long n4) {
     long long i = (long long)blockIdx.x * blockDim.x + threadIdx.x;
@@ -723,7 +822,7 @@
 }
 
 template <bool SPLIT>
-static int stem_impl(const float* x, int nimg, const int* hw_host, const void* w, const float* bias, void* y, void* stream) {
+static int stem_impl(const float* x, int nimg, const int* hw_host, const void* w, const float* bias, void* y, int pool, void* stream) {
     RF_REQUIRE(x != nullptr && w != nullptr && y != nullptr, "rf_stem7: null pointer");
     RF_REQUIRE(((uintptr_t)y % 16) == 0 && ((uintptr_t)w % 16) == 0, "rf_stem7: pointers must be 16-byte aligned");
     ImgSet set;
@@ -731,27 +830,34 @@
     StemParams p;
     memset(&p, 0, sizeof(p));
     p.nimg = nimg;
-    int tiles = 0;
+    p.pool = pool ? 1 : 0;
+    int units = 0;
+    long long out = 0;
     for (int i = 0; i < nimg; ++i) {
-        p.tiles_x[i] = (set.Wo[i] + SS_TW - 1) / SS_TW;
-        p.tile_start[i] = tiles;
-        tiles += p.tiles_x[i] * ((set.Ho[i] + SS_TH - 1) / SS_TH);
-        p.H[i] = set.H[i]; p.W[i] = set.W[i]; p.Ho[i] = set.Ho[i]; p.Wo[i] = set.Wo[i];
+        const int Hs = set.Ho[i], Ws = set.Wo[i];
+        const int Ho = pool ? (Hs - 1) / 2 + 1 : Hs, Wo = pool ? (Ws - 1) / 2 + 1 : Ws;
+        const int strips = pool ? (Wo + ST_PW - 1) / ST_PW : (Ws + ST_TW - 1) / ST_TW;
+        p.steps[i] = pool ? (Ho + ST_PH - 1) / ST_PH : (Hs + ST_TH - 1) / ST_TH;
+        p.unit_start[i] = units;
+        units += strips * p.steps[i];
+        p.H[i] = set.H[i]; p.W[i] = set.W[i]; p.Hs[i] = Hs; p.Ws[i] = Ws; p.Ho[i] = Ho; p.Wo[i] = Wo;
         p.in_pix[i] = set.in_pix[i];
-        p.out_pix[i] = set.out_pix[i];
-    }
-    for (int i = nimg; i <= RF_MAX_IMGS; ++i) p.tile_start[i] = tiles;
+        p.out_pix[i] = out;
+        out += (long long)Ho * Wo;
+    }
+    for (int i = nimg; i <= RF_MAX_IMGS; ++i) p.unit_start[i] = units;
     int rc = SPLIT ? get_map(&p.mapB, w, 192ull, 64ull, 2, 64, 64, 2, 1, 2) : get_map(&p.mapB, w, 192ull, 64ull, 0, 64, 64, 0, 1, 2);
     if (rc) return rc;
-    p.plane = set.out_pix[nimg] * 64;
+    p.plane = out * 64;
     p.x = x; p.bias = bias; p.y = static_cast<__half*>(y);
     static bool attr[64] = {false};
     const int dev = current_device();
     if (!attr[dev]) {
-        RF_CUDA(cudaFuncSetAttribute(stem7_kernel<SPLIT>, cudaFuncAttributeMaxDynamicSharedMemorySize, SS_SMEM));
+        RF_CUDA(cudaFuncSetAttribute(stem7_kernel<SPLIT>, cudaFuncAttributeMaxDynamicSharedMemorySize, ST_SMEM));
         attr[dev] = true;
     }
-    stem7_kernel<SPLIT><<<tiles, SS_THREADS, SS_SMEM, as_stream(stream)>>>(p);
+    const int grid = units < num_sms() ? units : num_sms();
+    stem7_kernel<SPLIT><<<grid, ST_THREADS, ST_SMEM, as_stream(stream)>>>(p);
     RF_LAUNCHED();
     return 0;
 }
@@ -815,11 +921,11 @@
     return conv_impl(set, p, w_split, as_stream(stream), K_SPLIT, false, &dual);
 }
 
-int rf_stem7_f16_impl(const float* x, int nimg, const int* hw_host, const void* w_f16, const float* bias, void* y_f16, void* stream) {
-    return stem_impl<false>(x, nimg, hw_host, w_f16, bias, y_f16, stream);
-}
-int rf_stem7_split_impl(const float* x, int nimg, const int* hw_host, const void* w_split, const float* bias, void* y_split, void* stream) {
-    return stem_impl<true>(x, nimg, hw_host, w_split, bias, y_split, stream);
+int rf_stem7_f16_impl(const float* x, int nimg, const int* hw_host, const void* w_f16, const float* bias, int pool, void* y_f16, void* stream) {
+    return stem_impl<false>(x, nimg, hw_host, w_f16, bias, y_f16, pool, stream);
+}
+int rf_stem7_split_impl(const float* x, int nimg, const int* hw_host, const void* w_split, const float* bias, int pool, void* y_split, void* stream) {
+    return stem_impl<true>(x, nimg, hw_host, w_split, bias, y_split, pool, stream);
 }
 
 size_t rf_corr_tc_workspace(int NA, int NB, int C) { return 2ull * ((size_t)NA + NB) * C * sizeof(float) + 1024; }
diff --git a/ransac-flow_b200/csrc/runner.cu b/ransac-flow_b200/csrc/runner.cu
--- a/ransac-flow_b200/csrc/runner.cu
+++ b/ransac-flow_b200/csrc/runner.cu
@@ -7,10 +7,10 @@
 int rf_poolblur_impl(const float* x, int nimg, const int* hw_host, int C, int round_out, float* y, void* stream);
 int rf_im2col_f16_impl(const float* x, int nimg, const int* hw_host, int C, int k, int stride, int pad, int Kpad, void* y_f16, void* stream);
 int rf_maxpool_f16_impl(const void* x_f16, int nimg, const int* hw_host, int C, int k, int stride, int pad, void* y_f16, void* stream);
-int rf_stem7_f16_impl(const float* x, int nimg, const int* hw_host, const void* w_f16, const float* bias, void* y_f16, void* stream);
+int rf_stem7_f16_impl(const float* x, int nimg, const int* hw_host, const void* w_f16, const float* bias, int pool, void* y_f16, void* stream);
 int rf_blur_f16_impl(const void* x_f16, int nimg, const int* hw_host, int C, int stride, void* y_f16, void* stream);
 int rf_poolblur_f16_impl(const void* x_f16, int nimg, const int* hw_host, int C, void* y_f16, void* stream);
-int rf_stem7_split_impl(const float* x, int nimg, const int* hw_host, const void* w_split, const float* bias, void* y_split, void* stream);
+int rf_stem7_split_impl(const float* x, int nimg, const int* hw_host, const void* w_split, const float* bias, int pool, void* y_split, void* stream);
 int rf_blur_split_impl(const void* x, int nimg, const int* hw_host, int C, int stride, void* y, void* stream);
 int rf_poolblur_split_impl(const void* x, int nimg, const int* hw_host, int C, void* y, void* stream);
 int rf_maxpool_split_impl(const void* x, int nimg, const int* hw_host, int C, int k, int stride, int pad, void* y, void* stream);
@@ -34,7 +34,27 @@
         float* y = static_cast<float*>(slots[l.dst]);
         int rc = 0;
         int k = l.k, stride = l.stride, pad = l.pad;
-        if (engine == RF_ENGINE_SPLIT) {
+        if (l.op == RF_OP_STEM7) {
+            RF_REQUIRE(engine == RF_ENGINE_SPLIT || engine == RF_ENGINE_F16, "rf_run_layers: RF_OP_STEM7 needs engine 2 or 4");
+            RF_REQUIRE(l.src == L[0].src && l.Cin == 3 && l.Cout == 64 && k == 7 && stride == 2 && pad == 3 && l.relu,
+                       "rf_run_layers: RF_OP_STEM7 is the ResNet-50 stem on the fp32 input slot");
+            const bool pool = (l.flags & RF_LAYER_STEM_POOL) != 0;
+            const rf_layer_t* mp = pool && li + 1 < n ? &L[li + 1] : nullptr;
+            RF_REQUIRE(!pool || (mp != nullptr && mp->op == RF_OP_MAXPOOL && mp->src == l.dst && mp->Cin == 64 && mp->k == 3 && mp->stride == 2 &&
+                                 mp->pad == 1 && mp->dst >= 0 && mp->dst < RF_MAX_SLOTS && mp->dst != l.src),
+                       "rf_run_layers: RF_LAYER_STEM_POOL needs the next layer to be a 3x3 / stride 2 / pad 1 max-pool of the stem's output");
+            void* out = pool ? slots[mp->dst] : y;
+            rc = engine == RF_ENGINE_SPLIT ? rf_stem7_split_impl(x, nimg, shw, l.w_f16, l.bias, pool, out, stream)
+                                           : rf_stem7_f16_impl(x, nimg, shw, l.w_f16, l.bias, pool, out, stream);
+            if (rc) return rc;
+            if (pool) {
+                for (int i = 0; i < nimg; ++i)
+                    for (int d = 0; d < 2; ++d) hw[mp->dst][2 * i + d] = ((shw[2 * i + d] - 1) / 2 + 1 - 1) / 2 + 1;
+                known[mp->dst] = true;
+                ++li;
+                continue;
+            }
+        } else if (engine == RF_ENGINE_SPLIT) {
             if (l.op == RF_OP_CONV) {
                 const float* res = l.res >= 0 ? static_cast<const float*>(slots[l.res]) : nullptr;
                 rc = rf_conv2d_nhwc(x, nimg, shw, l.Cin, l.w, static_cast<const float*>(l.w_f16), l.bias, res, l.Cout, k, k, stride, pad, l.relu,
@@ -51,10 +71,6 @@
             } else if (l.op == RF_OP_POOLBLUR) {
                 k = 4; stride = 2; pad = 1;
                 rc = rf_poolblur_split_impl(x, nimg, shw, l.Cin, y, stream);
-            } else if (l.op == RF_OP_STEM7) {
-                RF_REQUIRE(l.src == L[0].src && l.Cin == 3 && l.Cout == 64 && k == 7 && stride == 2 && pad == 3 && l.relu,
-                           "rf_run_layers: RF_OP_STEM7 is the ResNet-50 stem on the fp32 input slot");
-                rc = rf_stem7_split_impl(x, nimg, shw, l.w_f16, l.bias, y, stream);
             } else if (l.op == RF_OP_IM2COL) {
                 RF_REQUIRE(l.src == L[0].src, "rf_run_layers (engine 4): im2col reads the fp32 input slot");
                 rc = rf_im2col_split_impl(x, nimg, shw, l.Cin, k, stride, pad, l.Cout, y, stream);
@@ -77,10 +93,6 @@
             } else if (l.op == RF_OP_POOLBLUR) {
                 k = 4; stride = 2; pad = 1;
                 rc = rf_poolblur_f16_impl(x, nimg, shw, l.Cin, y, stream);
-            } else if (l.op == RF_OP_STEM7) {
-                RF_REQUIRE(l.src == L[0].src && l.Cin == 3 && l.Cout == 64 && k == 7 && stride == 2 && pad == 3 && l.relu,
-                           "rf_run_layers: RF_OP_STEM7 is the ResNet-50 stem on the fp32 input slot");
-                rc = rf_stem7_f16_impl(x, nimg, shw, l.w_f16, l.bias, y, stream);
             } else if (l.op == RF_OP_IM2COL) {
                 RF_REQUIRE(l.src == L[0].src, "rf_run_layers (engine 2): im2col reads the fp32 input slot");
                 rc = rf_im2col_f16_impl(x, nimg, shw, l.Cin, k, stride, pad, l.Cout, y, stream);
diff --git a/ransac-flow_b200/program.py b/ransac-flow_b200/program.py
--- a/ransac-flow_b200/program.py
+++ b/ransac-flow_b200/program.py
@@ -6,7 +6,7 @@
 
 RF_OP_CONV, RF_OP_MAXPOOL, RF_OP_BLUR, RF_OP_IM2COL, RF_OP_POOLBLUR, RF_OP_STEM7, RF_OP_CONV_DUAL = 0, 1, 2, 3, 4, 5, 6
 RF_MAX_SLOTS = 32
-RF_LAYER_OUT_F32, RF_LAYER_TF32 = 1, 2
+RF_LAYER_OUT_F32, RF_LAYER_TF32, RF_LAYER_STEM_POOL = 1, 2, 4
 
 
 class rf_layer_t(C.Structure):
@@ -122,6 +122,13 @@
                 elif o[0] not in (RF_OP_IM2COL, RF_OP_STEM7):
                     assert esize[o[1]] == 2 and (o[2] < 0 or esize[o[2]] == 2), "fp16 layer fed by an fp32 tensor"
         elems = [sum(h * w for h, w in hws[t]) * self.chan[t] * esize[t] for t in range(n_t)]
+        stem_pool = set()
+        for i, o in enumerate(self.ops[:-1]):
+            q = self.ops[i + 1]
+            if (f16 or split) and o[0] == RF_OP_STEM7 and q[0] == RF_OP_MAXPOOL and q[1] == i + 1 and tuple(q[5:8]) == (3, 2, 1) \
+                    and last_use[i + 1] == i + 1:
+                stem_pool.add(i)
+                elems[i + 1] = 0
         slot_of, free, slot_elems = {0: 0}, [], [0]
         layers = (rf_layer_t * len(self.ops))()
         for i, o in enumerate(self.ops):
@@ -142,7 +149,7 @@
             if fc is not None:
                 L.w, L.w_tc = fc.w.data_ptr(), fc.w_tc.data_ptr()
                 L.w_f16 = fc.w_f16.data_ptr() if f16 else (fc.w_split.data_ptr() if split else None)
-                L.flags = self.flags.get(i, 0) if (f16 or split) else 0
+                L.flags = (self.flags.get(i, 0) | (RF_LAYER_STEM_POOL if i in stem_pool else 0)) if (f16 or split) else 0
                 L.bias = fc.bias.data_ptr() if fc.bias is not None else None
             L.src2 = -1
             if i in self.dual:
```

Result: faster. 115.3 (median of 6 runs) (+3.2%).
